# mila-iqia/diffusion_for_multi_scale_molecular_dynamics

Hardware: AMD Instinct MI355X
Metric: sampled structures/sec (1000-step predictor-corrector SDE sampling) (higher is better)
Workload: dtype f32 (per-edge matrix products as split-f16 hi/lo x3 MFMA terms with f32 accumulation: 22-bit products; state, updates, reductions and every other layer in f32)

## Files before the change

diffusion_for_multi_scale_molecular_dynamics_amd/csrc/mdx_egnn.hip:

```cpp
#include <hip/hip_runtime.h>
#include <stdint.h>

#include "../../include/mdx_hip.h"
#include "mdx_launch.hpp"

using mdx::as_stream;
using mdx::kBlock;
using mdx::kWave;
using mdx::launch_status;

namespace {

__device__ __forceinline__ float silu_fast(float a) { return a / (1.0f + __expf(-a)); }

__global__ __launch_bounds__(kBlock) void egnn_message_input_kernel(const float* __restrict__ proj, const int64_t* __restrict__ edges,
                                                                    const float* __restrict__ radial, const float* __restrict__ bias,
                                                                    const float* __restrict__ w_radial, int64_t n_edges, int H,
                                                                    int silu, float* __restrict__ out)
{
    const int quads = H >> 2;
    const int64_t total = n_edges * quads;
    for (int64_t t = blockIdx.x * (int64_t)blockDim.x + threadIdx.x; t < total; t += (int64_t)gridDim.x * blockDim.x) {
        const int64_t e = t / quads;
        const int q = (int)(t - e * quads);
        const int64_t src = edges[2 * e], dst = edges[2 * e + 1];
        const float r = radial[e];
        const float4 a = reinterpret_cast<const float4*>(proj + src * 2 * H)[q];
        const float4 b = reinterpret_cast<const float4*>(proj + dst * 2 * H + H)[q];
        const float4 bi = reinterpret_cast<const float4*>(bias)[q];
        const float4 wr = reinterpret_cast<const float4*>(w_radial)[q];
        float4 o;
        o.x = (a.x + b.x + bi.x) + r * wr.x;
        o.y = (a.y + b.y + bi.y) + r * wr.y;
        o.z = (a.z + b.z + bi.z) + r * wr.z;
        o.w = (a.w + b.w + bi.w) + r * wr.w;
        if (silu) { o.x = silu_fast(o.x); o.y = silu_fast(o.y); o.z = silu_fast(o.z); o.w = silu_fast(o.w); }
        reinterpret_cast<float4*>(out + e * H)[q] = o;
    }
}

__device__ __forceinline__ void uplift(float kr, float& c, float& s)
{
    const double a = (double)kr;
    c = (float)cos(a);
    s = (float)sin(a);
}

__global__ __launch_bounds__(kBlock) void egnn_node_inputs_kernel(const float* __restrict__ x, const float* __restrict__ k_vectors,
                                                                  int n_k, const float* __restrict__ sigma, int atoms_per_structure,
                                                                  const int64_t* __restrict__ atom_types,
                                                                  const float* __restrict__ w, const float* __restrict__ b,
                                                                  int F, int H, int64_t n_nodes, float* __restrict__ z,
                                                                  float* __restrict__ h, const float* __restrict__ w2,
                                                                  const float* __restrict__ b2, int H2, float* __restrict__ h2,
                                                                  const uint32_t* __restrict__ table_key)
{
    if (mdx::table_is_current(table_key, sigma)) return;
    const int64_t stride = (int64_t)gridDim.x * blockDim.x, t0 = blockIdx.x * (int64_t)blockDim.x + threadIdx.x;
    if (h2) {
        for (int64_t t = t0; t < n_nodes * H2; t += stride) {
            const int64_t i = t / H2;
            const int j = (int)(t - i * H2);
            const float s = sigma[i / atoms_per_structure];
            const int64_t a = atom_types[i];
            float v = b2[j] + s * w2[(int64_t)j * F];
            if (a >= 0 && a + 1 < F) v = v + w2[(int64_t)j * F + 1 + a];
            h2[t] = v;
        }
    }
    for (int64_t t = t0; h && t < n_nodes * H; t += stride) {
        const int64_t i = t / H;
        const int j = (int)(t - i * H);
        const float s = sigma[i / atoms_per_structure];
        const int64_t a = atom_types[i];
        float v = b[j] + s * w[(int64_t)j * F];
        if (a >= 0 && a + 1 < F) v = v + w[(int64_t)j * F + 1 + a];
        h[t] = v;
    }
    for (int64_t t = t0; t < n_nodes * n_k; t += stride) {
        const int64_t i = t / n_k;
        const int k = (int)(t - i * n_k);
        float kr = 0.0f;
        for (int d = 0; d < 3; ++d) kr = kr + (6.2831855f * x[3 * i + d]) * k_vectors[3 * k + d];
        uplift(kr, z[2 * t], z[2 * t + 1]);
    }
}

__device__ __forceinline__ float4 embed_quad(const float* __restrict__ t, int H, int q, float s, int64_t a, int F)
{
    const float4 bias = reinterpret_cast<const float4*>(t)[q];
    const float4 w0 = reinterpret_cast<const float4*>(t + H)[q];
    float4 v;
    v.x = bias.x + s * w0.x;
    v.y = bias.y + s * w0.y;
    v.z = bias.z + s * w0.z;
    v.w = bias.w + s * w0.w;
    if (a >= 0 && a + 1 < F) {
        const float4 wa = reinterpret_cast<const float4*>(t + (2 + a) * H)[q];
        v.x = v.x + wa.x;
        v.y = v.y + wa.y;
        v.z = v.z + wa.z;
        v.w = v.w + wa.w;
    }
    return v;
}

__global__ __launch_bounds__(kBlock) void egnn_node_inputs_rows_kernel(const float* __restrict__ x, const float* __restrict__ k_vectors,
                                                                       int n_k, const float* __restrict__ sigma,
                                                                       int atoms_per_structure,
                                                                       const int64_t* __restrict__ atom_types,
                                                                       const float* __restrict__ w, const float* __restrict__ b,
                                                                       int F, int H, int64_t n_nodes, float* __restrict__ z,
                                                                       float* __restrict__ h, const float* __restrict__ w2,
                                                                       const float* __restrict__ b2, int H2,
                                                                       float* __restrict__ h2,
                                                                       const uint32_t* __restrict__ table_key)
{
    if (mdx::table_is_current(table_key, sigma)) return;
    extern __shared__ float tables[];
    float* t1 = tables;
    float* t2 = tables + (1 + F) * H;
    for (int j = threadIdx.x; h && j < H; j += blockDim.x) {
        t1[j] = b[j];
        for (int f = 0; f < F; ++f) t1[(1 + f) * H + j] = w[(int64_t)j * F + f];
    }
    if (h2)
        for (int j = threadIdx.x; j < H2; j += blockDim.x) {
            t2[j] = b2[j];
            for (int f = 0; f < F; ++f) t2[(1 + f) * H2 + j] = w2[(int64_t)j * F + f];
        }
    __syncthreads();
    const int lane = threadIdx.x % 64;
    const int64_t wave = (blockIdx.x * (int64_t)blockDim.x + threadIdx.x) / 64, n_waves = ((int64_t)gridDim.x * blockDim.x) / 64;
    const int per = n_k <= 64 ? min(4, 64 / n_k) : 1;
    for (int64_t i0 = wave * per; i0 < n_nodes; i0 += n_waves * per) {
        if (n_k <= 64) {
            const int g = lane / n_k, k = lane - g * n_k;
            const int64_t i = i0 + g;
            if (g < per && i < n_nodes) {
                float kr = 0.0f;
                for (int d = 0; d < 3; ++d) kr = kr + (6.2831855f * x[3 * i + d]) * k_vectors[3 * k + d];
                uplift(kr, z[2 * (i * n_k + k)], z[2 * (i * n_k + k) + 1]);
            }
        } else {
            for (int k = lane; k < n_k; k += 64) {
                float kr = 0.0f;
                for (int d = 0; d < 3; ++d) kr = kr + (6.2831855f * x[3 * i0 + d]) * k_vectors[3 * k + d];
                uplift(kr, z[2 * (i0 * n_k + k)], z[2 * (i0 * n_k + k) + 1]);
            }
        }
        if (!h && !h2) continue;
        for (int g = 0; g < per && i0 + g < n_nodes; ++g) {
            const int64_t i = i0 + g;
            const float s = sigma[i / atoms_per_structure];
            const int64_t a = atom_types[i];
            if (h2)
                for (int q = lane; q < (H2 >> 2); q += 64) reinterpret_cast<float4*>(h2 + i * H2)[q] = embed_quad(t2, H2, q, s, a, F);
            if (h)
                for (int q = lane; q < (H >> 2); q += 64) reinterpret_cast<float4*>(h + i * H)[q] = embed_quad(t1, H, q, s, a, F);
        }
    }
}

__global__ __launch_bounds__(kBlock) void egnn_scores_kernel(const float* __restrict__ z, const float* __restrict__ x_hat,
                                                             const float* __restrict__ k_vectors, int n_k, int64_t n_nodes,
                                                             float* __restrict__ scores)
{
    for (int64_t t = blockIdx.x * (int64_t)blockDim.x + threadIdx.x; t < n_nodes * 3; t += (int64_t)gridDim.x * blockDim.x) {
        const int64_t i = t / 3;
        const int alpha = (int)(t - 3 * i);
        const float* zi = z + i * 2 * n_k;
        const float* xi = x_hat + i * 2 * n_k;
        float acc = 0.0f;
        for (int k = 0; k < n_k; ++k) {
            const float kk = k_vectors[3 * k + alpha];
            acc = acc + ((zi[2 * k] * -kk) * xi[2 * k + 1] + (zi[2 * k + 1] * kk) * xi[2 * k]);
        }
        scores[t] = acc;
    }
}

__device__ __forceinline__ float wave_sum(float v)
{
    v += __builtin_bit_cast(float, __builtin_amdgcn_update_dpp(0, __builtin_bit_cast(int, v), 0x111, 0xf, 0xf, false));
    v += __builtin_bit_cast(float, __builtin_amdgcn_update_dpp(0, __builtin_bit_cast(int, v), 0x112, 0xf, 0xf, false));
    v += __builtin_bit_cast(float, __builtin_amdgcn_update_dpp(0, __builtin_bit_cast(int, v), 0x114, 0xf, 0xf, false));
    v += __builtin_bit_cast(float, __builtin_amdgcn_update_dpp(0, __builtin_bit_cast(int, v), 0x118, 0xf, 0xf, false));
    v += __builtin_bit_cast(float, __builtin_amdgcn_update_dpp(0, __builtin_bit_cast(int, v), 0x142, 0xa, 0xf, false));
    v += __builtin_bit_cast(float, __builtin_amdgcn_update_dpp(0, __builtin_bit_cast(int, v), 0x143, 0xc, 0xf, false));
    return __builtin_bit_cast(float, __builtin_amdgcn_readlane(__builtin_bit_cast(int, v), 63));
}

constexpr int kMaxClasses = 8;

__global__ __launch_bounds__(kBlock) void egnn_outputs_kernel(const float* __restrict__ z, const float* __restrict__ x_hat,
                                                              const float* __restrict__ k_vectors, int n_k,
                                                              const float* __restrict__ h, const float* __restrict__ cw,
                                                              const float* __restrict__ cb, int H, int C, int mask_class,
                                                              int64_t n_nodes, float* __restrict__ scores,
                                                              float* __restrict__ logits, float* __restrict__ zero_out,
                                                              int64_t n_zero)
{
    const int64_t tid = blockIdx.x * (int64_t)blockDim.x + threadIdx.x, n_threads = (int64_t)gridDim.x * blockDim.x;
    for (int64_t t = tid; t < n_zero; t += n_threads) zero_out[t] = 0.0f;
    const int lane = threadIdx.x % kWave;
    const int quads = H >> 2;
    constexpr int kNodesPerWave = 4;
    const int64_t n_waves = n_threads / kWave;
    for (int64_t node0 = (tid / kWave) * kNodesPerWave; node0 < n_nodes; node0 += n_waves * kNodesPerWave) {
        float acc = 0.0f;
        const int score_node = (lane - (kWave - 3 * kNodesPerWave)) / 3, alpha = (lane - (kWave - 3 * kNodesPerWave)) % 3;
        const bool scores_lane = lane >= kWave - 3 * kNodesPerWave && node0 + score_node < n_nodes;
        if (scores_lane) {
            const float* zi = z + (node0 + score_node) * 2 * n_k;
            const float* xi = x_hat + (node0 + score_node) * 2 * n_k;
            for (int k = 0; k < n_k; ++k) {
                const float kk = k_vectors[3 * k + alpha];
                acc = acc + ((zi[2 * k] * -kk) * xi[2 * k + 1] + (zi[2 * k + 1] * kk) * xi[2 * k]);
            }
        }
        float part[kNodesPerWave][kMaxClasses];
#pragma unroll
        for (int m = 0; m < kNodesPerWave; ++m)
#pragma unroll
            for (int c = 0; c < kMaxClasses; ++c) part[m][c] = 0.0f;
        for (int q = lane; q < quads; q += kWave) {
            float4 hv[kNodesPerWave];
#pragma unroll
            for (int m = 0; m < kNodesPerWave; ++m)
                hv[m] = node0 + m < n_nodes ? reinterpret_cast<const float4*>(h + (node0 + m) * H)[q] : float4{0.0f, 0.0f, 0.0f, 0.0f};
#pragma unroll
            for (int c = 0; c < kMaxClasses; ++c) {
                if (c < C && c != mask_class) {
                    const float4 wv = reinterpret_cast<const float4*>(cw + (int64_t)c * H)[q];
#pragma unroll
                    for (int m = 0; m < kNodesPerWave; ++m)
                        part[m][c] += (hv[m].x * wv.x + hv[m].y * wv.y) + (hv[m].z * wv.z + hv[m].w * wv.w);
                }
            }
        }
#pragma unroll
        for (int c = 0; c < kMaxClasses; ++c) {
            if (c < C) {
#pragma unroll
                for (int m = 0; m < kNodesPerWave; ++m) {
                    float v = part[m][c];
                    if (c != mask_class) v = wave_sum(v);
                    if (lane == 0 && node0 + m < n_nodes) logits[(node0 + m) * C + c] = (c == mask_class) ? -__builtin_inff() : v + cb[c];
                }
            }
// ... 17 lines not shown
        const int64_t e0 = offsets[node], deg = degree[node];
        float acc = 0.0f;
        auto row_dot = [&](int64_t e) {
            float part = 0.0f;
            for (int q = lane; q < quads; q += kWave) {
                const float4 hv = reinterpret_cast<const float4*>(hidden + e * H)[q];
                const float4 wv = reinterpret_cast<const float4*>(w)[q];
                part += (hv.x * wv.x + hv.y * wv.y) + (hv.z * wv.z + hv.w * wv.w);
            }
            return part;
        };
        auto finish = [&](int64_t e, float part) {
            part = mdx::wave_sum(part);
            if (lane < d) acc += coord_diff[e * d + lane] * part;
        };
        int64_t e = e0;
        for (; e + 4 <= e0 + deg; e += 4) {
            const float p0 = row_dot(e), p1 = row_dot(e + 1), p2 = row_dot(e + 2), p3 = row_dot(e + 3);
            finish(e, p0); finish(e + 1, p1); finish(e + 2, p2); finish(e + 3, p3);
        }
        for (; e < e0 + deg; ++e) finish(e, row_dot(e));
        if (lane < d) trans[node * d + lane] = (mean && deg > 0) ? acc / (float)deg : acc;
    }
}

__global__ __launch_bounds__(kBlock) void segment_rows_kernel(const float* __restrict__ data, const int64_t* __restrict__ offsets,
                                                              const int64_t* __restrict__ degree, int64_t n_nodes, int H, int mean,
                                                              float* __restrict__ out)
{
    const int lane = threadIdx.x % kWave;
    const int64_t wave = (blockIdx.x * (int64_t)blockDim.x + threadIdx.x) / kWave;
    const int64_t n_waves = ((int64_t)gridDim.x * blockDim.x) / kWave;
    const int quads = H >> 2;
    for (int64_t node = wave; node < n_nodes; node += n_waves) {
        const int64_t e0 = offsets[node], deg = degree[node];
        const float count = (mean && deg > 0) ? (float)deg : 1.0f;
        for (int q = lane; q < quads; q += kWave) {
            float4 acc = {0.0f, 0.0f, 0.0f, 0.0f};
#pragma unroll 4
            for (int64_t e = e0; e < e0 + deg; ++e) {
                const float4 v = reinterpret_cast<const float4*>(data + e * H)[q];
                acc.x += v.x; acc.y += v.y; acc.z += v.z; acc.w += v.w;
            }
            if (mean) { acc.x /= count; acc.y /= count; acc.z /= count; acc.w /= count; }
            reinterpret_cast<float4*>(out + node * H)[q] = acc;
        }
    }
}

}

extern "C" {

int mdx_egnn_message_input(const float* node_proj, const int64_t* edges, const float* radial, const float* bias,
                           const float* w_radial, int64_t n_edges, int H, int silu, float* out, mdx_stream_t stream)
{
    if (n_edges < 0 || H < 4 || (H & 3)) return H >= 1 && (H & 3) ? MDX_ERR_UNSUPPORTED : MDX_ERR_INVALID_ARG;
    if (n_edges == 0) return MDX_OK;
    if (!node_proj || !edges || !radial || !bias || !w_radial || !out) return MDX_ERR_INVALID_ARG;
    int64_t blocks = (n_edges * (H >> 2) + kBlock - 1) / kBlock;
    if (blocks > 16384) blocks = 16384;
    hipLaunchKernelGGL(egnn_message_input_kernel, dim3((unsigned)blocks), dim3(kBlock), 0, as_stream(stream),
                       node_proj, edges, radial, bias, w_radial, n_edges, H, silu, out);
    return launch_status();
}

static unsigned node_grid(int64_t n_nodes)
{
    int64_t blocks = (n_nodes * kWave + kBlock - 1) / kBlock;
    if (blocks > 16384) blocks = 16384;
    return (unsigned)(blocks < 1 ? 1 : blocks);
}

int mdx_egnn_node_inputs(const float* x, const float* k_vectors, int n_k, const float* sigma, int atoms_per_structure,
                         const int64_t* atom_types, const float* emb_weight, const float* emb_bias, int n_features, int H,
                         int64_t n_nodes, float* z_out, float* h_out, const float* second_weight, const float* second_bias,
                         int second_width, float* second_out, mdx_stream_t stream)
{
    return mdx_egnn_node_inputs_keyed(x, k_vectors, n_k, sigma, atoms_per_structure, atom_types, emb_weight, emb_bias, n_features,
                                      H, n_nodes, z_out, h_out, second_weight, second_bias, second_width, second_out, nullptr,
                                      stream);
}

int mdx_egnn_node_inputs_keyed(const float* x, const float* k_vectors, int n_k, const float* sigma, int atoms_per_structure,
                               const int64_t* atom_types, const float* emb_weight, const float* emb_bias, int n_features, int H,
                               int64_t n_nodes, float* z_out, float* h_out, const float* second_weight, const float* second_bias,
                               int second_width, float* second_out, const uint32_t* table_key, mdx_stream_t stream)
{
    if (n_nodes < 0 || n_k < 1 || atoms_per_structure < 1 || n_features < 2 || H < 1) return MDX_ERR_INVALID_ARG;
    if (n_nodes == 0) return MDX_OK;
    if (!x || !k_vectors || !sigma || !atom_types || !emb_weight || !emb_bias || !z_out) return MDX_ERR_INVALID_ARG;
    if (second_out && (!second_weight || !second_bias || second_width < 1)) return MDX_ERR_INVALID_ARG;
    const size_t table_bytes = sizeof(float) * (size_t)(1 + n_features) * ((size_t)H + (second_out ? (size_t)second_width : 0));
    if ((H & 3) == 0 && (!second_out || (second_width & 3) == 0) && table_bytes <= 48 * 1024) {
        int64_t blocks = (n_nodes + 15) / 16;
        if (blocks > 2048) blocks = 2048;
        hipLaunchKernelGGL(egnn_node_inputs_rows_kernel, dim3((unsigned)blocks), dim3(kBlock), table_bytes,
                           as_stream(stream), x, k_vectors, n_k, sigma, atoms_per_structure, atom_types,
                           emb_weight, emb_bias, n_features, H, n_nodes, z_out, h_out, second_weight, second_bias, second_width,
                           second_out, table_key);
        return launch_status();
    }
    int64_t blocks = (n_nodes * H + kBlock - 1) / kBlock;
    if (blocks > 16384) blocks = 16384;
    hipLaunchKernelGGL(egnn_node_inputs_kernel, dim3((unsigned)blocks), dim3(kBlock), 0, as_stream(stream), x,
                       k_vectors, n_k, sigma, atoms_per_structure, atom_types, emb_weight, emb_bias, n_features, H, n_nodes,
                       z_out, h_out, second_weight, second_bias, second_width, second_out, table_key);
    return launch_status();
}

int mdx_egnn_scores(const float* z, const float* x_hat, const float* k_vectors, int n_k, int64_t n_nodes, float* scores_out,
                    mdx_stream_t stream)
{
    if (n_nodes < 0 || n_k < 1) return MDX_ERR_INVALID_ARG;
    if (n_nodes == 0) return MDX_OK;
    if (!z || !x_hat || !k_vectors || !scores_out) return MDX_ERR_INVALID_ARG;
    int64_t blocks = (n_nodes * 3 + kBlock - 1) / kBlock;
    if (blocks > 16384) blocks = 16384;
    hipLaunchKernelGGL(egnn_scores_kernel, dim3((unsigned)blocks), dim3(kBlock), 0, as_stream(stream), z, x_hat,
                       k_vectors, n_k, n_nodes, scores_out);
    return launch_status();
}

int mdx_egnn_outputs(const float* z, const float* x_hat, const float* k_vectors, int n_k, const float* h,
                     const float* class_weight, const float* class_bias, int H, int num_classes, int mask_class,
                     int64_t n_nodes, float* scores_out, float* logits_out, float* zero_out, int64_t n_zero,
                     mdx_stream_t stream)
{
    if (n_nodes < 0 || n_k < 1 || H < 4 || num_classes < 1 || n_zero < 0 || mask_class >= num_classes) return MDX_ERR_INVALID_ARG;
    if ((H & 3) || num_classes > kMaxClasses) return MDX_ERR_UNSUPPORTED;
    if (n_zero > 0 && !zero_out) return MDX_ERR_INVALID_ARG;
    if (n_nodes == 0 && n_zero == 0) return MDX_OK;
    if (n_nodes > 0 && (!z || !x_hat || !k_vectors || !h || !class_weight || !class_bias || !scores_out || !logits_out))
        return MDX_ERR_INVALID_ARG;
    hipLaunchKernelGGL(egnn_outputs_kernel, dim3(node_grid((n_nodes + 3) / 4)), dim3(kBlock), 0, as_stream(stream), z,
                       x_hat, k_vectors, n_k, h, class_weight, class_bias, H, num_classes, mask_class, n_nodes, scores_out,
                       logits_out, zero_out, n_zero);
    return launch_status();
}

int mdx_egnn_coord_head(const float* hidden, const float* w_out, const float* coord_diff, const int64_t* offsets,
                        const int64_t* degree, int64_t n_nodes, int H, int spatial_dimension, int mean, float* trans,
                        mdx_stream_t stream)
{
    if (n_nodes < 0 || H < 4 || spatial_dimension < 1) return MDX_ERR_INVALID_ARG;
    if ((H & 3) || spatial_dimension > kWave) return MDX_ERR_UNSUPPORTED;
    if (n_nodes == 0) return MDX_OK;
    if (!hidden || !w_out || !coord_diff || !offsets || !degree || !trans) return MDX_ERR_INVALID_ARG;
    hipLaunchKernelGGL(egnn_coord_head_kernel, dim3(node_grid(n_nodes)), dim3(kBlock), 0, as_stream(stream),
                       hidden, w_out, coord_diff, offsets, degree, n_nodes, H, spatial_dimension, mean, trans);
    return launch_status();
}

int mdx_segment_rows(const float* data, const int64_t* offsets, const int64_t* degree, int64_t n_nodes, int H, int mean,
                     float* out, mdx_stream_t stream)
{
    if (n_nodes < 0 || H < 4) return MDX_ERR_INVALID_ARG;
    if (H & 3) return MDX_ERR_UNSUPPORTED;
    if (n_nodes == 0) return MDX_OK;
    if (!data || !offsets || !degree || !out) return MDX_ERR_INVALID_ARG;
    hipLaunchKernelGGL(segment_rows_kernel, dim3(node_grid(n_nodes)), dim3(kBlock), 0, as_stream(stream),
                       data, offsets, degree, n_nodes, H, mean, out);
    return launch_status();
}

}
```

diffusion_for_multi_scale_molecular_dynamics_amd/csrc/mdx_egnn_table.hip:

```cpp
#include <hip/hip_runtime.h>
#include <stdint.h>

#include "../../include/mdx_hip.h"
#include "mdx_launch.hpp"

using namespace mdx;

namespace {

typedef float f32x4 __attribute__((ext_vector_type(4)));

__device__ __forceinline__ void lagrange_weights(float t, float w[4])
{
    const float tp = t + 1.0f, tm = t - 1.0f, t2 = t - 2.0f;
    w[0] = -(t * tm * t2) / 6.0f;
    w[1] = (tp * tm * t2) / 2.0f;
    w[2] = -(tp * t * t2) / 2.0f;
    w[3] = (tp * t * tm) / 6.0f;
}

__device__ __forceinline__ float interpolate(const float w[4], float v0, float v1, float v2, float v3)
{
    return ((w[0] * v0 + w[1] * v1) + w[2] * v2) + w[3] * v3;
}

__device__ __forceinline__ f32x4 interpolate4(const float w[4], f32x4 v0, f32x4 v1, f32x4 v2, f32x4 v3)
{
    return ((w[0] * v0 + w[1] * v1) + w[2] * v2) + w[3] * v3;
}

__device__ __forceinline__ float squared_distance(const float* ci, const float* __restrict__ cj, int D)
{
    float r2 = 0.0f;
    for (int k = 0; k < D; ++k) {
        const float dlt = ci[k] - cj[k];
        r2 += dlt * dlt;
    }
    return r2;
}

__device__ __forceinline__ float coord_head_value(float s, int flags) { return (flags & MDX_EGNN_COORD_TANH) ? tanhf(s) : s; }
__device__ __forceinline__ float normalize_factor(float r2) { return tanhf(r2) / sqrtf(r2 + 1.0e-16f); }

__device__ __forceinline__ unsigned abs_bits(float v) { return __float_as_uint(v) & 0x7fffffffu; }

constexpr int kCheckRows = 32;
__global__ __launch_bounds__(256) void egnn_table_check_kernel(const float* __restrict__ messages, const float* __restrict__ scalar,
                                                               int H, int n_pairs, int n_even, unsigned* __restrict__ workspace,
                                                               const uint32_t* __restrict__ table_key,
                                                               const float* __restrict__ sigma)
{
    if (table_is_current(table_key, sigma)) return;
    const int p = blockIdx.x, K = 2 * n_even - 1;
    const int j0 = blockIdx.y * kCheckRows, j1 = min(j0 + kCheckRows, n_even - 2);
    float w[4];
    lagrange_weights(0.5f, w);
    for (int c = threadIdx.x; c <= H; c += blockDim.x) {
        auto value = [&](int row) { return c < H ? messages[((int64_t)p * K + row) * H + c] : scalar[(int64_t)p * K + row]; };
        unsigned err = 0, big = 0;
        for (int j = j0; j < j1; ++j) {
            const float v0 = value(j > 0 ? j - 1 : 1), v1 = value(j), v2 = value(j + 1), v3 = value(j + 2);
            const float mid = value(n_even + j);
            err = max(err, abs_bits(interpolate(w, v0, v1, v2, v3) - mid));
            big = max(big, max(max(abs_bits(v1), abs_bits(v2)), max(abs_bits(v3), abs_bits(mid))));
        }
        if (j0 < j1) {
            atomicMax(workspace + (int64_t)p * (H + 1) + c, err);
            atomicMax(workspace + (int64_t)n_pairs * (H + 1) + p, big);
        }
    }
}

__global__ __launch_bounds__(256) void egnn_table_verdict_kernel(unsigned* __restrict__ workspace, int n_pairs, int columns,
                                                                 const float* __restrict__ sigma, int64_t n_sigma, float tolerance,
                                                                 float* __restrict__ worst_out, uint32_t* __restrict__ status,
                                                                 uint32_t* __restrict__ table_key)
{
    __shared__ float worst[256];
    __shared__ int bad[256];
    float mine = 0.0f;
    int fail = 0;
    const bool built = !table_is_current(table_key, sigma);
    const int64_t n_entries = built ? (int64_t)n_pairs * columns : 0;
    for (int64_t i = threadIdx.x; i < n_entries; i += blockDim.x) {
        const float err = __uint_as_float(workspace[i]), big = __uint_as_float(workspace[n_entries + i / columns]);
        if (!(err <= tolerance * big)) fail = 1;
        if (big > 0.0f) mine = fmaxf(mine, err / big);
        else if (err > 0.0f || err != err) mine = INFINITY;
    }
    __syncthreads();
    if (built)
        for (int64_t i = threadIdx.x; i < n_entries + n_pairs; i += blockDim.x) workspace[i] = 0u;
    const int table_fail = fail;
    for (int64_t i = 1 + threadIdx.x; i < n_sigma; i += blockDim.x)
        if (!(sigma[i] == sigma[0])) fail = 1;
    worst[threadIdx.x] = mine;
    bad[threadIdx.x] = fail | (table_fail << 1);
    __syncthreads();
    for (int s = 128; s > 0; s >>= 1) {
        if ((int)threadIdx.x < s) {
            worst[threadIdx.x] = fmaxf(worst[threadIdx.x], worst[threadIdx.x + s]);
            bad[threadIdx.x] |= bad[threadIdx.x + s];
        }
        __syncthreads();
    }
    if (threadIdx.x == 0) {
        if (worst_out && built) worst_out[0] = worst[0];
        if (bad[0] && status) atomicOr(status, MDX_STATUS_EGNN_TABLE);
        if (table_key && built) {
            if (bad[0] & 2) {
                table_key[0] = MDX_EGNN_TABLE_NO_KEY;
            } else {
                table_key[0] = __float_as_uint(sigma[0]);
                table_key[1] = table_key[1] + 1u;
            }
        }
    }
}

__global__ __launch_bounds__(256) void egnn_table_gather_kernel(const float* __restrict__ table, const float* __restrict__ table_scalar,
                                                                int H, int n_classes, int n_even, float inv_spacing,
                                                                const int64_t* __restrict__ atom_types,
                                                                const int64_t* __restrict__ offsets, const int64_t* __restrict__ degree,
                                                                int64_t n_nodes, int mean_messages, float* __restrict__ out,
                                                                const float* __restrict__ left, const float* __restrict__ coord,
                                                                const int64_t* __restrict__ edges, int D, int mean_coords,
                                                                int flags, float* __restrict__ coord_out, uint32_t* __restrict__ status)
{
    const int lane = threadIdx.x % kWave;
    const int64_t wave = (blockIdx.x * (int64_t)blockDim.x + threadIdx.x) / kWave;
    const int64_t n_waves = ((int64_t)gridDim.x * blockDim.x) / kWave;
    const int K = 2 * n_even - 1, quads = H >> 2;
    const bool has_quad = lane < quads;
    bool outside = false;
    for (int64_t node = wave; node < n_nodes; node += n_waves) {
        const int64_t e0 = offsets[node], deg = degree[node], e1 = e0 + deg;
        int64_t a = atom_types[node];
        if (a < 0 || a >= n_classes) { outside = true; a = 0; }
        float part[8] = {0, 0, 0, 0, 0, 0, 0, 0}, ci[8];
#pragma unroll
        for (int k = 0; k < 8; ++k) ci[k] = k < D ? coord[node * D + k] : 0.0f;
        f32x4 acc = {0.0f, 0.0f, 0.0f, 0.0f};
        for (int64_t c0 = e0; c0 < e1; c0 += kWave) {
            const int64_t e = c0 + lane;
            int row = 0, row_left = 0;
            float w[4] = {0, 0, 0, 0};
            if (e < e1) {
                const int64_t dst = edges[2 * e + 1];
                int64_t b = atom_types[dst];
                if (b < 0 || b >= n_classes) { outside = true; b = 0; }
                const float r2 = squared_distance(ci, coord + dst * D, D);
                const float u = sqrtf(r2) * inv_spacing;
                int m = 0;
                float t = 0.0f;
                if (u <= (float)(n_even - 2)) {
                    m = min((int)u, n_even - 3);
                    t = u - (float)m;
                } else {
                    outside = true;
                }
                lagrange_weights(t, w);
                row = (int)(a * n_classes + b) * K + m;
                row_left = m > 0 ? row - 1 : row + 1;
                const float s = coord_head_value(interpolate(w, table_scalar[row_left], table_scalar[row], table_scalar[row + 1],
                                                             table_scalar[row + 2]), flags);
                if (flags & MDX_EGNN_COORD_NORMALIZE) {
                    float diff[8], n2 = 0.0f;
#pragma unroll
                    for (int k = 0; k < 8; ++k) {
                        diff[k] = k < D ? ci[k] - coord[dst * D + k] : 0.0f;
                        if (k < D) n2 += diff[k] * diff[k];
                    }
                    const float f = normalize_factor(n2);
#pragma unroll
                    for (int k = 0; k < 8; ++k)
                        if (k < D) part[k] += (f * diff[k]) * s;
                } else {
#pragma unroll
                    for (int k = 0; k < 8; ++k)
                        if (k < D) part[k] += (ci[k] - coord[dst * D + k]) * s;
                }
            }
            const int n = (int)min<int64_t>(kWave, e1 - c0);
            for (int i = 0; i < n; ++i) {
                const int r = __builtin_amdgcn_readlane(row, i), rl = __builtin_amdgcn_readlane(row_left, i);
                float wi[4];
#pragma unroll
                for (int k = 0; k < 4; ++k)
                    wi[k] = __builtin_bit_cast(float, __builtin_amdgcn_readlane(__builtin_bit_cast(int, w[k]), i));
                if (has_quad) {
                    const f32x4* base = reinterpret_cast<const f32x4*>(table + (int64_t)r * H) + lane;
                    const f32x4 v0 = reinterpret_cast<const f32x4*>(table + (int64_t)rl * H)[lane];
                    acc += interpolate4(wi, v0, base[0], base[quads], base[2 * quads]);
                }
            }
        }
        const float count = (mean_messages && deg > 0) ? (float)deg : 1.0f;
        if (has_quad) {
            if (mean_messages) acc = acc / count;
            if (left) {
                reinterpret_cast<f32x4*>(out + node * 2 * H)[lane] = reinterpret_cast<const f32x4*>(left + node * H)[lane];
                reinterpret_cast<f32x4*>(out + node * 2 * H + H)[lane] = acc;
            } else {
                reinterpret_cast<f32x4*>(out + node * H)[lane] = acc;
            }
        }
#pragma unroll
        for (int k = 0; k < 8; ++k) {
            if (k < D) {
                float v = part[k];
                v += __builtin_bit_cast(float, __builtin_amdgcn_update_dpp(0, __builtin_bit_cast(int, v), 0x111, 0xf, 0xf, false));
                v += __builtin_bit_cast(float, __builtin_amdgcn_update_dpp(0, __builtin_bit_cast(int, v), 0x112, 0xf, 0xf, false));
                v += __builtin_bit_cast(float, __builtin_amdgcn_update_dpp(0, __builtin_bit_cast(int, v), 0x114, 0xf, 0xf, false));
                v += __builtin_bit_cast(float, __builtin_amdgcn_update_dpp(0, __builtin_bit_cast(int, v), 0x118, 0xf, 0xf, false));
                v += __builtin_bit_cast(float, __builtin_amdgcn_update_dpp(0, __builtin_bit_cast(int, v), 0x142, 0xa, 0xf, false));
                v += __builtin_bit_cast(float, __builtin_amdgcn_update_dpp(0, __builtin_bit_cast(int, v), 0x143, 0xc, 0xf, false));
                part[k] = __builtin_bit_cast(float, __builtin_amdgcn_readlane(__builtin_bit_cast(int, v), 63));
            }
        }
        if (lane < D) {
            float total = 0.0f, mine = 0.0f;
#pragma unroll
            for (int k = 0; k < 8; ++k) {
                if (k == lane) { total = part[k]; mine = ci[k]; }
            }
            if (mean_coords && deg > 0) total = total / (float)deg;
            coord_out[node * D + lane] = mine + total;
        }
    }
    if (outside && status) atomicOr(status, MDX_STATUS_EGNN_TABLE);
}

}

extern "C" {

int mdx_egnn_table_check(const float* table, const float* table_scalar, int H, int n_classes, int n_even, const float* sigma,
                         int64_t n_sigma, float tolerance, uint32_t* workspace, float* worst_out, uint32_t* status,
                         mdx_stream_t stream)
{
    return mdx_egnn_table_check_keyed(table, table_scalar, H, n_classes, n_even, sigma, n_sigma, tolerance, workspace, worst_out,
                                      status, nullptr, stream);
}

int mdx_egnn_table_check_keyed(const float* table, const float* table_scalar, int H, int n_classes, int n_even, const float* sigma,
                               int64_t n_sigma, float tolerance, uint32_t* workspace, float* worst_out, uint32_t* status,
                               uint32_t* table_key, mdx_stream_t stream)
{
    if (H < 1 || n_classes < 1 || n_even < 4 || n_sigma < 1 || !(tolerance >= 0.0f)) return MDX_ERR_INVALID_ARG;
    if (!table || !table_scalar || !sigma || !workspace) return MDX_ERR_INVALID_ARG;
    const int n_pairs = n_classes * n_classes;
    const hipStream_t s = as_stream(stream);
    hipLaunchKernelGGL(egnn_table_check_kernel, dim3((unsigned)n_pairs, (unsigned)((n_even - 2 + kCheckRows - 1) / kCheckRows)),
                       dim3(256), 0, s, table, table_scalar, H, n_pairs, n_even, reinterpret_cast<unsigned*>(workspace),
                       table_key, sigma);
    hipLaunchKernelGGL(egnn_table_verdict_kernel, dim3(1), dim3(256), 0, s, reinterpret_cast<unsigned*>(workspace), n_pairs,
                       H + 1, sigma, n_sigma, tolerance, worst_out, status, table_key);
    return launch_status();
}

int mdx_egnn_table_gather(const float* table, const float* table_scalar, int H, int n_classes, int n_even, float inv_spacing,
                          const int64_t* atom_types, const int64_t* offsets, const int64_t* degree, int64_t n_nodes,
                          int mean_messages, const float* left, float* out, const float* coord, int coord_dimension,
                          const int64_t* edges, int mean_coords, int coord_flags, float* coord_out, uint32_t* status,
                          mdx_stream_t stream)
{
    if (n_nodes < 0 || H < 4 || n_classes < 1 || n_even < 4 || coord_dimension < 1 || !(inv_spacing > 0.0f))
        return MDX_ERR_INVALID_ARG;
    if (coord_flags & ~(MDX_EGNN_COORD_NORMALIZE | MDX_EGNN_COORD_TANH)) return MDX_ERR_INVALID_ARG;
    if ((H & 3) || H > 4 * kWave || coord_dimension > 8) return MDX_ERR_UNSUPPORTED;
    if ((int64_t)n_classes * n_classes * (2 * (int64_t)n_even - 1) * H >= ((int64_t)1 << 31)) return MDX_ERR_UNSUPPORTED;
    if (n_nodes == 0) return MDX_OK;
    if (!table || !table_scalar || !atom_types || !offsets || !degree || !out || !coord || !edges || !coord_out)
        return MDX_ERR_INVALID_ARG;
    int64_t blocks = (n_nodes * kWave + 255) / 256;
    if (blocks > 16384) blocks = 16384;
    hipLaunchKernelGGL(egnn_table_gather_kernel, dim3((unsigned)blocks), dim3(256), 0, as_stream(stream),
                       table, table_scalar, H, n_classes, n_even, inv_spacing, atom_types, offsets, degree, n_nodes, mean_messages,
                       out, left, coord, edges, coord_dimension, mean_coords, coord_flags, coord_out, status);
    return launch_status();
}

}
```

diffusion_for_multi_scale_molecular_dynamics_amd/csrc/mdx_hip.hip:

```cpp
#include <hip/hip_runtime.h>
#include <stdint.h>

#include <atomic>
#include <cmath>

#include "../../include/mdx_hip.h"
#include "mdx_launch.hpp"
#include "mdx_math.hpp"

using namespace mdx;

namespace {

struct ScheduleArgs {
    int T, type, C;
    double time_delta, sigma_min, sigma_max, corrector_eps;
    float *time, *sigma, *sigma2, *g, *g2, *eps, *sqrt2eps, *beta, *alpha_bar, *q, *qbar, *qbar_tm1;
};

template <int CSPEC>
__device__ __forceinline__ void qbar_chain(const ScheduleArgs& a, int r)
{
    const int T = a.T, C = CSPEC > 0 ? CSPEC : a.C;
#define MDX_SCHED_CLASSES(c) _Pragma("unroll") for (int c = 0; c < MDX_MAX_CLASSES; ++c) if (c < C)
// ... 529 lines not shown
            }
            if (one) {
                const float cand = (prop != a_t) ? v_best : -__builtin_huge_valf();
                if (cand > best_v || (cand == best_v && n < best_n)) { best_v = cand; best_n = n; best_prop = prop; }
                v.a_out[n] = a_t;
            } else {
                v.a_out[n] = prop;
                if (st.last_predictor_step && prop == M && p.status) atomicOr(p.status, MDX_STATUS_MASK_AT_LAST_STEP);
            }
        } else if (v.a_out && v.a_out != v.a) {
            v.a_out[n] = v.a[n];
        }
        if (p.do_coords) {
            float z0 = 0.0f, z1 = 0.0f, z2 = 0.0f, z3 = 0.0f;
            if (!v.z_coord) {
                const u32x4 r = philox4x32_10(item, st.call8, st.draw, MDX_TAG_COORD, st.k0, st.k1);
                box_muller(r.v[0], r.v[1], z0, z1);
                if (d > 2) box_muller(r.v[2], r.v[3], z2, z3);
            }
            float xin[3], sin_[3], out[3];
#pragma unroll
            for (int k = 0; k < 3; ++k)
                if (k < d) {
                    const int e = n * d + k;
                    const float zk = k == 0 ? z0 : (k == 1 ? z1 : z2);
                    xin[k] = v.x[e];
                    sin_[k] = v.score_x[e];
                    out[k] = v.z_coord ? v.z_coord[e] : zk;
                }
#pragma unroll
            for (int k = 0; k < 3; ++k)
                if (k < d) out[k] = coord_update(xin[k], sin_[k], out[k], sc.w, sc.n, sc.sigma);
#pragma unroll
            for (int k = 0; k < 3; ++k)
                if (k < d) v.x_out[n * d + k] = out[k];
        }
    }
    if (update_types && one) {
        group_argmax<G>(best_v, best_n, best_prop);
        if (lane == 0 && best_n < N) v.a_out[best_n] = best_prop;
    }
    if (p.do_lattice) {
        for (int k = lane; k < p.nl; k += G) {
            if (p.fixed_lattice) {
                if (v.l_out != v.l) v.l_out[k] = v.l[k];
            } else {
                float zz;
                if (v.z_lat) zz = v.z_lat[k];
                else {
                    const u32x4 r = philox4x32_10((uint32_t)v.b, st.call8 | (uint32_t)(k >> 2), st.draw, MDX_TAG_LATTICE,
                                                  st.k0, st.k1);
                    float z0, z1, z2, z3;
                    box_muller(r.v[0], r.v[1], z0, z1);
                    box_muller(r.v[2], r.v[3], z2, z3);
                    const int kk = k & 3;
                    zz = kk == 0 ? z0 : (kk == 1 ? z1 : (kk == 2 ? z2 : z3));
                }
                v.l_out[k] = (v.l[k] + (sc.w * v.score_l[k]) / sc.sigma_n) + sc.n * zz;
            }
        }
    }
}

__device__ __forceinline__ const float* off(const float* p, int64_t o) { return p ? p + o : nullptr; }
__device__ __forceinline__ float* off(float* p, int64_t o) { return p ? p + o : nullptr; }

__device__ __forceinline__ PcView structure_view(const PcArgs& p, int64_t b)
{
    const int N = p.N, C = p.C, d = p.d;
    PcView v;
    const int64_t a0 = b * N;
    v.a = p.a ? p.a + a0 : nullptr;
    v.x = off(p.x, a0 * d); v.l = off(p.l, b * p.nl);
    v.logits = off(p.logits, a0 * C); v.score_x = off(p.score_x, a0 * d); v.score_l = off(p.score_l, b * p.nl);
    v.z_coord = off(p.z_coord, a0 * d); v.gumbel = off(p.gumbel, a0 * C); v.u = off(p.u, a0);
    v.z_lat = off(p.z_lat, b * p.nl);
    v.a_out = p.a_out ? p.a_out + a0 : nullptr;
    v.x_out = off(p.x_out, a0 * d); v.l_out = off(p.l_out, b * p.nl); v.p_out = off(p.p_out, a0 * C);
    v.item0 = a0;
    v.b = b;
    return v;
}

template <int G, int CSPEC>
__global__ __launch_bounds__(kBlock) void pc_step_kernel(PcArgs p_in)
{
    PcArgs p = p_in;
    if constexpr (CSPEC > 0) { p.C = CSPEC; p.d = 3; p.nl = 6; }
    const int lane = threadIdx.x & (G - 1);
    const int64_t groups_per_grid = ((int64_t)gridDim.x * blockDim.x) / G;
    const int64_t group0 = ((int64_t)blockIdx.x * blockDim.x + threadIdx.x) / G;
    const PcStep st = make_step(p);
    for (int64_t b = group0; b < p.B; b += groups_per_grid) {
        const PcView v = structure_view(p, b);
        pc_update_structure<G>(p, st, v, lane, p.update_types);
    }
}

inline int lanes_per_structure(int N)
{
    int G = 1;
    while (G < N && G < kWave) G <<= 1;
    return G;
}

inline dim3 structure_grid(int64_t B, int G)
{
    int64_t blocks = cdiv(B * G, kBlock);
    if (blocks > 4096) blocks = 4096;
    if (blocks < 1) blocks = 1;
    return dim3((unsigned)blocks);
}

#define MDX_SWITCH_G(G, LAUNCH)                                                                              \
    switch (G) {                                                                                             \
        case 1: LAUNCH(1) break;                                                                             \
        case 2: LAUNCH(2) break;                                                                             \
        case 4: LAUNCH(4) break;                                                                             \
        case 8: LAUNCH(8) break;                                                                             \
        case 16: LAUNCH(16) break;                                                                           \
        case 32: LAUNCH(32) break;                                                                           \
        default: LAUNCH(64) break;                                                                           \
    }

int launch_pc(const PcArgs& a, hipStream_t st)
{
    const int G = lanes_per_structure(a.N);
    const dim3 grid = structure_grid(a.B, G), block(kBlock);
    const int cspec = (a.d == 3 && (a.C == 2 || a.C == 3)) ? a.C : 0;
#define MDX_LAUNCH_PC(GG)                                                                                   \
    if (cspec == 2) hipLaunchKernelGGL((pc_step_kernel<GG, 2>), grid, block, 0, st, a);                       \
    else if (cspec == 3) hipLaunchKernelGGL((pc_step_kernel<GG, 3>), grid, block, 0, st, a);                  \
    else hipLaunchKernelGGL((pc_step_kernel<GG, 0>), grid, block, 0, st, a);
    MDX_SWITCH_G(G, MDX_LAUNCH_PC)
#undef MDX_LAUNCH_PC
    return launch_status();
}

template <int G, int O = G / 2>
__device__ __forceinline__ float group_sum(float v)
{
    if constexpr (O > 0) {
        v = group_sum<G, O / 2>(v);
        v = v + partner<O>(v);
    }
    return v;
}

struct AdaptiveStatsArgs {
    const float *score_x, *score_l, *z_coord, *z_lat;
    mdx_rng_t rng;
    int index_i;
    const int32_t* d_index;
    int64_t B;
    int N, d, nl, fixed_lattice;
    float* workspace;
};

template <int G>
__global__ __launch_bounds__(kBlock) void adaptive_stats_kernel(AdaptiveStatsArgs p)
{
    const int lane = threadIdx.x & (G - 1);
    const int64_t groups_per_grid = ((int64_t)gridDim.x * blockDim.x) / G;
    const int64_t group0 = ((int64_t)blockIdx.x * blockDim.x + threadIdx.x) / G;
    const int N = p.N, d = p.d;
    const int index = (p.d_index ? *p.d_index : 0) + p.index_i;
    const uint32_t draw = (uint32_t)index * p.rng.draw_stride + p.rng.draw_offset;
    const uint32_t k0 = (uint32_t)p.rng.seed, k1 = (uint32_t)(p.rng.seed >> 32), call8 = rng_call(p.rng) << 8;
    for (int64_t b = group0; b < p.B; b += groups_per_grid) {
        const int64_t a0 = b * N;
        const float* sx = p.score_x + a0 * d;
        const float* zx = p.z_coord ? p.z_coord + a0 * d : nullptr;
        float ss = 0.0f, zn = 0.0f;
        for (int n = lane; n < N; n += G) {
            float z0 = 0.0f, z1 = 0.0f, z2 = 0.0f, z3 = 0.0f;
            if (!zx) {
                const u32x4 r = philox4x32_10((uint32_t)(a0 + n), call8, draw, MDX_TAG_COORD, k0, k1);
                box_muller(r.v[0], r.v[1], z0, z1);
                if (d > 2) box_muller(r.v[2], r.v[3], z2, z3);
            }
            float zz = 0.0f;
#pragma unroll
            for (int k = 0; k < 3; ++k)
                if (k < d) {
                    const int e = n * d + k;
                    const float s = sx[e];
                    const float zk = zx ? zx[e] : (k == 0 ? z0 : (k == 1 ? z1 : z2));
                    ss = ss + s * s;
                    zz = zz + zk * zk;
                }
            zn = zn + __builtin_sqrtf(zz);
        }
        ss = group_sum<G>(ss);
        zn = group_sum<G>(zn);
        float sl = 0.0f, zl = 0.0f;
        if (!p.fixed_lattice) {
            for (int k = lane; k < p.nl; k += G) {
                float zk;
                if (p.z_lat) zk = p.z_lat[b * p.nl + k];
                else {
                    const u32x4 r = philox4x32_10((uint32_t)b, call8 | (uint32_t)(k >> 2), draw, MDX_TAG_LATTICE, k0, k1);
                    float z0, z1, z2, z3;
                    box_muller(r.v[0], r.v[1], z0, z1);
                    box_muller(r.v[2], r.v[3], z2, z3);
                    const int kk = k & 3;
                    zk = kk == 0 ? z0 : (kk == 1 ? z1 : (kk == 2 ? z2 : z3));
                }
                const float s = p.score_l[b * p.nl + k];
                sl = sl + s * s;
                zl = zl + zk * zk;
            }
            sl = group_sum<G>(sl);
            zl = group_sum<G>(zl);
        }
        if (lane == 0) {
            float* w = p.workspace + b * 4;
// ... 1311 lines not shown
    return coordinates_update(x, s, z, score_weight, gaussian_noise_weight, sigma, nullptr, count, out, stream);
}

int mdx_relative_coordinates_update_dev(const float* x, const float* s, const float* z, const float* weights, int64_t count,
                                        float* out, mdx_stream_t stream)
{
    if (!weights) return MDX_ERR_INVALID_ARG;
    return coordinates_update(x, s, z, 0.0f, 0.0f, 1.0f, weights, count, out, stream);
}

static int lattice_update(const float* l, const float* s, const float* z, float score_weight, float gaussian_noise_weight,
                          float sigma_n, const float* weights_dev, int64_t count, float* out, mdx_stream_t stream)
{
    if (count < 0 || (count > 0 && (!l || !s || !z || !out))) return MDX_ERR_INVALID_ARG;
    if (count == 0) return MDX_OK;
    hipLaunchKernelGGL(lattice_update_kernel, dim3(flat_grid(count)), dim3(kBlock), 0, as_stream(stream), l, s, z,
                       score_weight, gaussian_noise_weight, sigma_n, count, out, weights_dev);
    return launch_status();
}

int mdx_lattice_parameters_update(const float* l, const float* s, const float* z, float score_weight,
                                  float gaussian_noise_weight, float sigma_n, int64_t count, float* out,
                                  mdx_stream_t stream)
{
    return lattice_update(l, s, z, score_weight, gaussian_noise_weight, sigma_n, nullptr, count, out, stream);
}

int mdx_lattice_parameters_update_dev(const float* l, const float* s, const float* z, const float* weights, int64_t count,
                                      float* out, mdx_stream_t stream)
{
    if (!weights) return MDX_ERR_INVALID_ARG;
    return lattice_update(l, s, z, 0.0f, 0.0f, 1.0f, weights, count, out, stream);
}

int mdx_atom_types_update(const float* logits, const int64_t* atom_types, const float* q, const float* q_bar,
                          const float* q_bar_tm1, const float* gumbel, const float* u, int64_t batch,
                          int number_of_atoms, int num_classes, float small_epsilon, int greedy, int one_transition,
                          int64_t* atom_types_out, float* probabilities_out, mdx_stream_t stream)
{
    if (batch < 0 || number_of_atoms < 1) return MDX_ERR_INVALID_ARG;
    if (num_classes < 2) return MDX_ERR_INVALID_ARG;
    if (num_classes > MDX_MAX_CLASSES) return MDX_ERR_UNSUPPORTED;
    if (batch == 0) return MDX_OK;
    if (!logits || !atom_types || !q || !q_bar || !q_bar_tm1 || !gumbel || !atom_types_out || (greedy && !u))
        return MDX_ERR_INVALID_ARG;
    PcArgs a{};
    a.use_tables = 0;
    a.q_explicit = q; a.qbar_explicit = q_bar; a.qbar_tm1_explicit = q_bar_tm1;
    a.greedy = greedy; a.one_transition = one_transition; a.update_types = 1;
    a.small_eps = small_epsilon;
    a.a = atom_types; a.logits = logits; a.gumbel = gumbel; a.u = u;
    a.B = batch; a.N = number_of_atoms; a.C = num_classes; a.d = 3;
    a.a_out = atom_types_out; a.p_out = probabilities_out;
    return launch_pc(a, as_stream(stream));
}

static int pc_common_args(const mdx_schedule_t* sched_host, int mode, int index_i, const int32_t* d_index, const mdx_pc_flags_t* f,
                          const int64_t* atom_types, const float* logits, const float* gumbel, const float* u, mdx_rng_t rng,
                          int64_t batch, int number_of_atoms, int spatial_dimension, int64_t* atom_types_out, uint32_t* status,
                          PcArgs& a)
{
    const int rc = check_index(sched_host, mode, index_i, d_index);
    if (rc != MDX_OK) return rc;
    if (!f || batch < 0 || number_of_atoms < 1 || spatial_dimension < 1 || spatial_dimension > 3) return MDX_ERR_INVALID_ARG;
    const int C = sched_host->num_classes;
    if (C < 2) return MDX_ERR_INVALID_ARG;
    if (C > MDX_MAX_CLASSES) return MDX_ERR_UNSUPPORTED;
    a.sched = to_dev(sched_host);
    a.use_tables = 1;
    a.mode = mode; a.index_i = index_i; a.d_index = d_index;
    a.atoms_pow = pow((double)number_of_atoms, 1.0 / (double)spatial_dimension);
    a.greedy = f->atom_type_greedy_sampling; a.one_transition = f->one_atom_type_transition_per_step;
    a.fixed_lattice = f->use_fixed_lattice_parameters;
    a.small_eps = f->small_epsilon;
    a.a = atom_types; a.logits = logits; a.gumbel = gumbel; a.u = u;
    a.rng = rng;
    a.B = batch; a.N = number_of_atoms; a.d = spatial_dimension; a.C = C;
    a.nl = spatial_dimension * (spatial_dimension + 1) / 2;
    a.a_out = atom_types_out; a.p_out = nullptr;
    a.status = status;
    return MDX_OK;
}

int mdx_pc_step_update(const mdx_schedule_t* sched_host, int mode, int index_i, const int32_t* d_index,
                       const mdx_pc_flags_t* f, const int64_t* atom_types, const float* x, const float* l,
                       const float* logits, const float* score_x, const float* score_l, const float* z_coordinates,
                       const float* gumbel, const float* u, const float* z_lattice, mdx_rng_t rng, int64_t batch,
                       int number_of_atoms, int spatial_dimension, int64_t* atom_types_out, float* x_out, float* l_out,
                       uint32_t* status, mdx_stream_t stream)
{
    PcArgs a{};
    const int rc = pc_common_args(sched_host, mode, index_i, d_index, f, atom_types, logits, gumbel, u, rng, batch, number_of_atoms,
                                  spatial_dimension, atom_types_out, status, a);
    if (rc != MDX_OK || batch == 0) return rc;
    if (!x || !score_x || !x_out || !l || !l_out) return MDX_ERR_INVALID_ARG;
    if (f->update_atom_types && (!atom_types || !atom_types_out)) return MDX_ERR_INVALID_ARG;
    if (f->update_atom_types && !logits && (a.C != 2 || a.p_out)) return MDX_ERR_INVALID_ARG;
    if (!f->use_fixed_lattice_parameters && !score_l) return MDX_ERR_INVALID_ARG;
    if ((int64_t)batch * number_of_atoms > 0xffffffffLL) return MDX_ERR_UNSUPPORTED;
    a.update_types = f->update_atom_types;
    a.do_coords = 1; a.do_lattice = 1;
    a.x = x; a.l = l; a.score_x = score_x; a.score_l = score_l; a.z_coord = z_coordinates; a.z_lat = z_lattice;
    a.x_out = x_out; a.l_out = l_out;
    return launch_pc(a, as_stream(stream));
}

static AdaptiveStepArgs adaptive_step_args(const mdx_schedule_t* sched_host, int index_i, const int32_t* d_index,
                                           int number_of_atoms, int spatial_dimension, int fixed_lattice, float corrector_r,
                                           float small_epsilon, const double* totals, float* weights)
{
    AdaptiveStepArgs s{};
    s.sched = to_dev(sched_host);
    s.index_i = index_i; s.d_index = d_index;
    s.atoms_pow = pow((double)number_of_atoms, 1.0 / (double)spatial_dimension);
    s.corrector_r = corrector_r; s.small_eps = small_epsilon;
    s.fixed_lattice = fixed_lattice;
    s.totals = totals; s.weights = weights;
    return s;
}

int mdx_adaptive_corrector_statistics(const mdx_schedule_t* sched_host, int index_i, const int32_t* d_index,
                                      const float* score_x, const float* score_l, const float* z_coordinates,
                                      const float* z_lattice_for_step_size, mdx_rng_t rng, int64_t batch, int number_of_atoms,
                                      int spatial_dimension, int use_fixed_lattice_parameters, float corrector_r,
                                      float small_epsilon, float* workspace, double* totals, float* weights,
                                      mdx_stream_t stream)
{
    const int rc = check_index(sched_host, MDX_CORRECTOR, index_i, d_index);
    if (rc != MDX_OK) return rc;
    if (batch < 1 || number_of_atoms < 1 || spatial_dimension < 1 || spatial_dimension > 3) return MDX_ERR_INVALID_ARG;
    if (!score_x || !workspace || !totals || (!use_fixed_lattice_parameters && !score_l)) return MDX_ERR_INVALID_ARG;
    if ((int64_t)batch * number_of_atoms > 0xffffffffLL) return MDX_ERR_UNSUPPORTED;
    AdaptiveStatsArgs a{};
    a.score_x = score_x; a.score_l = score_l; a.z_coord = z_coordinates; a.z_lat = z_lattice_for_step_size;
    a.rng = rng;
    a.index_i = index_i; a.d_index = d_index;
    a.B = batch; a.N = number_of_atoms; a.d = spatial_dimension;
    a.nl = spatial_dimension * (spatial_dimension + 1) / 2;
    a.fixed_lattice = use_fixed_lattice_parameters;
    a.workspace = workspace;
    const int rs = launch_adaptive_stats(a, as_stream(stream));
    if (rs != MDX_OK) return rs;
    hipLaunchKernelGGL(adaptive_totals_kernel, dim3(1), dim3(kBlock), 0, as_stream(stream), (const float*)workspace, batch,
                       number_of_atoms, totals,
                       adaptive_step_args(sched_host, index_i, d_index, number_of_atoms, spatial_dimension,
                                          use_fixed_lattice_parameters, corrector_r, small_epsilon, totals, weights));
    return launch_status();
}

int mdx_adaptive_corrector_step_size(const mdx_schedule_t* sched_host, int index_i, const int32_t* d_index,
                                     const double* totals, int number_of_atoms, int spatial_dimension,
                                     int use_fixed_lattice_parameters, float corrector_r, float small_epsilon, float* weights,
                                     mdx_stream_t stream)
{
    const int rc = check_index(sched_host, MDX_CORRECTOR, index_i, d_index);
    if (rc != MDX_OK) return rc;
    if (number_of_atoms < 1 || spatial_dimension < 1 || spatial_dimension > 3 || !totals || !weights) return MDX_ERR_INVALID_ARG;
    hipLaunchKernelGGL(adaptive_step_kernel, dim3(1), dim3(1), 0, as_stream(stream),
                       adaptive_step_args(sched_host, index_i, d_index, number_of_atoms, spatial_dimension,
                                          use_fixed_lattice_parameters, corrector_r, small_epsilon, totals, weights));
    return launch_status();
}

int mdx_adaptive_corrector_update(const mdx_schedule_t* sched_host, int mode, int index_i, const int32_t* d_index,
                                  const mdx_pc_flags_t* f, const int64_t* atom_types, const float* x, const float* l,
                                  const float* logits, const float* score_x, const float* score_l, const float* z_coordinates,
                                  const float* gumbel, const float* u, const float* z_lattice, const float* weights,
                                  mdx_rng_t rng, int64_t batch, int number_of_atoms, int spatial_dimension,
                                  int64_t* atom_types_out, float* x_out, float* l_out, uint32_t* status, mdx_stream_t stream)
{
    PcArgs a{};
    const int rc = pc_common_args(sched_host, mode, index_i, d_index, f, atom_types, logits, gumbel, u, rng, batch, number_of_atoms,
                                  spatial_dimension, atom_types_out, status, a);
    if (rc != MDX_OK || batch == 0) return rc;
    const int types = mode == MDX_PREDICTOR ? 1 : f->update_atom_types;
    if (types && (!atom_types || !logits || !atom_types_out)) return MDX_ERR_INVALID_ARG;
    if (mode == MDX_CORRECTOR) {
        if (!weights || !x || !score_x || !x_out || !l || !l_out) return MDX_ERR_INVALID_ARG;
        if (!f->use_fixed_lattice_parameters && !score_l) return MDX_ERR_INVALID_ARG;
    }
    if ((int64_t)batch * number_of_atoms > 0xffffffffLL) return MDX_ERR_UNSUPPORTED;
    a.update_types = types;
    if (mode == MDX_CORRECTOR) {
        a.x = x; a.l = l; a.score_x = score_x; a.score_l = score_l; a.z_coord = z_coordinates; a.z_lat = z_lattice;
        a.x_out = x_out; a.l_out = l_out;
    }
    return launch_adaptive_update(a, weights, as_stream(stream));
// ... 376 lines not shown
```

diffusion_for_multi_scale_molecular_dynamics_amd/generators/langevin_generator.py:

```python
import contextlib
import dataclasses
import gc
import warnings
import weakref
from typing import Optional

import torch

from .. import kernels
from .._hip import (MDX_CORRECTOR, MDX_PREDICTOR, STATUS_EGNN_F16_RANGE, STATUS_EGNN_TABLE, STATUS_MASK_AT_LAST_STEP,
                    MdxError, PcFlags, Rng)
from ..models.score_networks.score_network import ScoreNetwork
from ..namespace import AXL, CARTESIAN_FORCES, NOISE, NOISY_AXL_COMPOSITION, TIME
from ..noise_schedulers.noise_parameters import NoiseParameters
from ..noise_schedulers.noise_scheduler import NoiseScheduler
from ..utils.sample_trajectory import PinnedStaging, SampleTrajectory
from . import network_hooks as hooks
from .noise_sources import DevicePhiloxNoise, RecordingNoise, ReferenceOrderNoise, one_host_thread, upload
from .predictor_corrector_axl_generator import PredictorCorrectorAXLGenerator, PredictorCorrectorSamplingParameters
from .trajectory_initializer import TrajectoryInitializer


class LangevinGenerator(PredictorCorrectorAXLGenerator):
    def __init__(self, noise_parameters: NoiseParameters, sampling_parameters: PredictorCorrectorSamplingParameters,
                 axl_network: ScoreNetwork, trajectory_initializer: Optional[TrajectoryInitializer] = None):
        sp = sampling_parameters
        super().__init__(number_of_discretization_steps=noise_parameters.total_time_steps,
                         number_of_corrector_steps=sp.number_of_corrector_steps,
                         spatial_dimension=sp.spatial_dimension, num_atom_types=sp.num_atom_types,
                         number_of_atoms=sp.number_of_atoms,
                         use_fixed_lattice_parameters=sp.use_fixed_lattice_parameters,
                         fixed_lattice_parameters=sp.fixed_lattice_parameters,
                         trajectory_initializer=trajectory_initializer)
        self.noise_parameters = noise_parameters
        self.sampling_parameters = sp
        self.number_of_atoms = sp.number_of_atoms
        self.masked_atom_type_index = self.num_classes - 1
        self.axl_network = axl_network
        self.small_epsilon = sp.small_epsilon
        self.one_atom_type_transition_per_step = sp.one_atom_type_transition_per_step
        self.atom_type_greedy_sampling = sp.atom_type_greedy_sampling
        self.atom_type_transition_in_corrector = sp.atom_type_transition_in_corrector
        self.use_fixed_lattice_parameters = sp.use_fixed_lattice_parameters
        self.fixed_lattice_parameters = sp.fixed_lattice_parameters

        self.record = sp.record_samples
        self.record_corrector = sp.record_samples_corrector_steps
        self.record_atom_type_update = sp.record_atom_type_update
        if self.record_corrector or self.record_atom_type_update:
            assert self.record, "Corrector steps or atom_type_update can only be recorded if record_samples is True."

        rng_mode = getattr(sp, "rng_mode", "reference")
        assert rng_mode in ("reference", "device"), f"unknown rng_mode {rng_mode}"
        self.rng_mode = rng_mode
        self.use_hip_graph = bool(getattr(sp, "use_hip_graph", False))
        self.fused_score_network = bool(getattr(sp, "fused_score_network", False))
        self._mlp_pack = None
        self._noise_workspace = kernels.NoiseWorkspace()
        self.fused_sampler_options = 0
        self.fused_predrawn_noise = True
        self._seed = getattr(sp, "seed", None)
        self._call_counter = 0
        self.noise_source = ReferenceOrderNoise() if rng_mode == "reference" else None
        self.f16_range_fallbacks = 0
        self.table_fallbacks = 0
        self.resampling_steps = 0
        self._visit = 0
        self._warned_not_capturable = False

        self._scheduler = None
        self._status = None
        self._call_word = None
        self._buffers = {}
        if self.record:
            self.sample_trajectory_recorder = SampleTrajectory()
            self._staging = PinnedStaging()
            self.sample_trajectory_recorder.record(key="noise_parameters", entry=dataclasses.asdict(noise_parameters))
            self.sample_trajectory_recorder.record(key="sampling_parameters",
                                                   entry={k: v for k, v in dataclasses.asdict(sp).items()})

    @property
    def _device_rng(self) -> bool:
        return getattr(self.noise_source, "device_rng", False)

    @staticmethod
    def _device(device) -> torch.device:
        device = torch.device(device)
        if device.type == "cuda" and device.index is None:
            device = torch.device("cuda", torch.cuda.current_device())
        return device

    def _prepare(self, device: torch.device):
        device = self._device(device)
        if device.type != "cuda":
            raise MdxError(f"LangevinGenerator runs on the GPU hot path only; got device '{device}' "
                           "(there is no CPU fallback -- use the reference implementation on CPU)")
        if self._scheduler is None or self._scheduler.tables.device != device:
            self._scheduler = NoiseScheduler(self.noise_parameters, num_classes=self.num_classes, device=device)
            self.noise, self.langevin_dynamics = self._scheduler.get_all_sampling_parameters()
            self._status = torch.zeros(1, dtype=torch.int32, device=device)
            self._buffers = {}
            if self.record:
                self.sample_trajectory_recorder.record(
                    key="noise", entry=type(self.noise)(*[t.detach().cpu() for t in self.noise]))
        return self._scheduler.tables

    def _time_sigma(self, batch: int, device):
        key = ("ts", batch)
        if key not in self._buffers:
            self._buffers[key] = (torch.empty(batch, 1, dtype=torch.float32, device=device),
                                  torch.empty(batch, 1, dtype=torch.float32, device=device))
        return self._buffers[key]

    def _flags(self, update_atom_types: bool) -> PcFlags:
        return PcFlags(int(self.atom_type_greedy_sampling), int(self.one_atom_type_transition_per_step),
                       int(self.use_fixed_lattice_parameters), int(update_atom_types), float(self.small_epsilon))

    def _draw_stride(self) -> int:
        return (self.number_of_corrector_steps + 1) * (self.resampling_steps + 1)

    def _rng(self, draw_offset: int) -> Rng:
        src = self.noise_source
        seed, call = (src.seed, src.call) if self._device_rng else (0, 0)
        word = self._call_word.data_ptr() if self._device_rng and self._call_word is not None else None
        return Rng(seed, call, self._draw_stride(),
                   self._visit * (self.number_of_corrector_steps + 1) + draw_offset, 0, word)

    def _begin_call(self, device):
        if self.rng_mode == "device":
            seed = self._seed if self._seed is not None else torch.initial_seed()
            rank = torch.distributed.get_rank() if torch.distributed.is_available() and \
                torch.distributed.is_initialized() else 0
            self.noise_source = DevicePhiloxNoise(seed + rank, self._call_counter)
            device = self._device(device)
            if self._call_word is None or self._call_word.device != device:
                self._buffers.pop("graph_loop", None)
                self._call_word = torch.zeros(1, dtype=torch.int32, device=device)
            kernels.index_set(self._call_word, self._call_counter)
            self._call_counter += 1
        if hasattr(self.trajectory_initializer, "noise_source"):
            self.trajectory_initializer.noise_source = self.noise_source

    def _draw_coordinates_gaussian_sample(self, number_of_samples):
        return self.noise_source.randn(number_of_samples, self.number_of_atoms, self.spatial_dimension)

    def _draw_lattice_gaussian_sample(self, number_of_samples):
        return self.noise_source.randn(number_of_samples, self.num_lattice_parameters)

# ... 39 lines not shown
        lat = lattice_parameters
        if z is None:
            z = self._draw_lattice_gaussian_sample(lat.shape[0])
        weights = self._three_scalars(score_weight, gaussian_noise_weight, sigma_n_i, lat)
        return kernels.lattice_parameters_update(lat.contiguous(), sigma_normalized_scores.to(lat).contiguous(),
                                                 z.to(lat).contiguous(), weights=weights)

    _lattice_parameters_update_predictor_step = _lattice_parameters_update
    _lattice_parameters_update_corrector_step = _lattice_parameters_update

    @staticmethod
    def _shared_matrix(m: torch.Tensor, name: str) -> torch.Tensor:
        from ..utils.d3pm_utils import _one_matrix
        one = _one_matrix(m)
        if one is None:
            flat = m.reshape(-1, m.shape[-2], m.shape[-1])
            one = flat[0]
            if not bool((flat == one).all()):
                raise MdxError(f"{name}: the transition matrices differ between samples / atoms; the sampler's atom-type update "
                               "takes ONE time index per call (use utils.d3pm_utils.get_probability_at_previous_time_step for "
                               "per-atom matrices)")
        return one

    def _atom_types_update(self, predicted_logits: torch.Tensor, atom_types_i: torch.LongTensor, q_matrices_i: torch.Tensor,
                           q_bar_matrices_i: torch.Tensor, q_bar_tm1_matrices_i: torch.Tensor,
                           atom_type_greedy_sampling: bool, one_atom_type_transition_per_step: bool) -> torch.LongTensor:
        logits = predicted_logits
        batch = logits.shape[0]
        gumbel = self._draw_gumbel_sample(batch).to(device=logits.device, dtype=torch.float32).contiguous()
        u = None
        if atom_type_greedy_sampling:
            u = self._draw_binary_sample(batch).to(device=logits.device, dtype=torch.float32).contiguous()
        q, q_bar, q_bar_tm1 = [self._shared_matrix(m, name).to(logits).contiguous()
                               for m, name in ((q_matrices_i, "q_matrices_i"), (q_bar_matrices_i, "q_bar_matrices_i"),
                                               (q_bar_tm1_matrices_i, "q_bar_tm1_matrices_i"))]
        a_in = atom_types_i.to(logits.device).contiguous()
        a_out, probs = kernels.atom_types_update(logits.contiguous(), a_in, q, q_bar, q_bar_tm1, gumbel, u, self.small_epsilon,
                                                 atom_type_greedy_sampling, one_atom_type_transition_per_step,
                                                 return_probabilities=True)
        if self.record_atom_type_update:
            if atom_type_greedy_sampling:
                all_masked = (a_in == self.masked_atom_type_index).all(dim=-1)
                gumbel = torch.where(all_masked.view(-1, 1, 1), gumbel, torch.zeros_like(gumbel))
            self.sample_trajectory_recorder.record(key="atom_type_update", entry=dict(
                predicted_logits=logits.detach().cpu(), one_step_transition_probabilities=probs.cpu(),
                gumbel_sample=gumbel.cpu(), a_i=a_in.cpu(), a_im1=a_out.cpu()))
        return a_out

    def _get_coordinates_corrector_step_size(self, index_i: int, sigma_i: torch.Tensor, model_predictions_i: torch.Tensor,
                                             z: torch.Tensor) -> torch.Tensor:
        self._prepare(model_predictions_i.device)
        return self.langevin_dynamics.epsilon[index_i].to(model_predictions_i)

    def _get_lattice_parameters_corrector_step_size(self, index_i: int, sigma_n_i: torch.Tensor,
                                                    model_predictions_i: torch.Tensor, z: torch.Tensor) -> torch.Tensor:
        self._prepare(model_predictions_i.device)
        return self.langevin_dynamics.epsilon[index_i].to(model_predictions_i)

    def _get_model_predictions(self, composition: AXL, time, sigma_noise, cartesian_forces: torch.Tensor) -> AXL:
        if not isinstance(time, torch.Tensor) or time.dim() == 0:
            time = torch.full((composition.X.shape[0], 1), float(time), dtype=torch.float32, device=composition.X.device)
        if not isinstance(sigma_noise, torch.Tensor) or sigma_noise.dim() == 0:
            sigma_noise = torch.full((composition.X.shape[0], 1), float(sigma_noise), dtype=torch.float32, device=composition.X.device)
        batch = {NOISY_AXL_COMPOSITION: composition, TIME: time, NOISE: sigma_noise, CARTESIAN_FORCES: cartesian_forces}
        with hooks.uniform_sigma(self.axl_network):
            return self.axl_network(batch, conditional=False)

    def _lattice_score(self, predictions: AXL, composition: AXL) -> Optional[torch.Tensor]:
        if self.use_fixed_lattice_parameters:
            return None
        if predictions.L.shape != composition.L.shape:
            raise MdxError(f"the score network's lattice output has shape {tuple(predictions.L.shape)}, the lattice parameters "
                           f"{tuple(composition.L.shape)}: this network can only sample with use_fixed_lattice_parameters=True")
        return predictions.L.contiguous()

    def _logits_unread(self, update_types: bool, predictions_unread: bool) -> bool:
        constant_logits = self.num_classes == 2
        return bool(predictions_unread and (not update_types or constant_logits) and not self.record
                    and not self.record_atom_type_update and "_get_model_predictions" not in self.__dict__
                    and type(self)._get_model_predictions is _OWN_GET_MODEL_PREDICTIONS
                    and not hooks.outputs_watched(self.axl_network))

    def _step(self, mode: int, composition: AXL, index_i: int, cartesian_forces: torch.Tensor, draw_offset: int,
              d_index: Optional[torch.Tensor] = None, in_place: bool = False, predictions_unread: bool = False):
        x = composition.X
        device = x.device
        sched = self._prepare(device)
        batch = x.shape[0]
        time_t, sigma_t = self._time_sigma(batch, device)
        kernels.fill_time_sigma(sched, mode, index_i, d_index, time_t, sigma_t)
        update_types = mode == MDX_PREDICTOR or self.atom_type_transition_in_corrector
        unread = self._logits_unread(update_types, predictions_unread)
        with hooks.logits_unread(self.axl_network) if unread else contextlib.nullcontext():
            predictions = self._get_model_predictions(composition, time_t, sigma_t, cartesian_forces)

        z = gumbel = u = z_lattice = None
        if not self._device_rng:
            if mode == MDX_PREDICTOR:
                gumbel = self._draw_gumbel_sample(batch)
                if self.atom_type_greedy_sampling:
                    u = self._draw_binary_sample(batch)
                z = self._draw_coordinates_gaussian_sample(batch)
                z_lattice = self._draw_lattice_gaussian_sample(batch)
            else:
                z = self._draw_coordinates_gaussian_sample(batch)
                self._draw_lattice_gaussian_sample(batch)
                if not self.use_fixed_lattice_parameters:
                    z_lattice = self._draw_lattice_gaussian_sample(batch)
                if update_types:
                    gumbel = self._draw_gumbel_sample(batch)
                    if self.atom_type_greedy_sampling:
                        u = self._draw_binary_sample(batch)
            if self.use_fixed_lattice_parameters:
                z_lattice = None
            z, gumbel, u, z_lattice = [upload(t, device) for t in (z, gumbel, u, z_lattice)]
            if not self.use_fixed_lattice_parameters and z_lattice is None:
                raise MdxError("internal error: lattice noise missing")

        a_in = composition.A
        if update_types:
            a_out = a_in if in_place else torch.empty_like(a_in)
        else:
            a_out = a_in
        x_out = x if in_place else torch.empty_like(x)
        if self.use_fixed_lattice_parameters or in_place:
            l_out = composition.L
        else:
            l_out = torch.empty_like(composition.L)
        logits = predictions.A.contiguous() if update_types and predictions.A is not None else None
        if update_types and logits is None and not unread:
            raise MdxError("the score network returned no atom-type logits for a step that reads them")
        kernels.pc_step_update(sched, mode, index_i, d_index, self._flags(update_types),
                               a_in if update_types else None, x, composition.L, logits,
                               predictions.X.contiguous(),
                               self._lattice_score(predictions, composition),
                               z, gumbel, u, z_lattice, self._rng(draw_offset),
                               a_out if update_types else None, x_out, l_out, self._status)
        if self.record_atom_type_update and update_types:
            self._record_atom_type_update(sched, mode, index_i, logits, a_in, gumbel, u, a_out, batch)
        return AXL(A=a_out, X=x_out, L=l_out), predictions

    def _record_atom_type_update(self, sched, mode, index_i, logits, a_in, gumbel, u, a_out, batch):
        idx = index_i - 1 if (mode == MDX_PREDICTOR or index_i > 0) else 0
        src = self.noise_source
        if gumbel is None:
            from .._hip import TAG_BINARY, TAG_GUMBEL
            draw = index_i * self._draw_stride() + self._visit * (self.number_of_corrector_steps + 1) + \
                (0 if mode == MDX_PREDICTOR else 1)
            n = batch * self.number_of_atoms
            gumbel = kernels.rng_fill(kernels.RNG_GUMBEL, src.seed, src.call, draw, TAG_GUMBEL, n, self.num_classes,
                                      logits.device).view(batch, self.number_of_atoms, self.num_classes)
            u = kernels.rng_fill(kernels.RNG_UNIFORM, src.seed, src.call, draw, TAG_BINARY, n, 1,
                                 logits.device).view(batch, self.number_of_atoms)
        one = self.one_atom_type_transition_per_step and not (mode == MDX_PREDICTOR and idx == 0)
        a_check, probs = kernels.atom_types_update(logits, a_in, sched.q_matrix[idx], sched.q_bar_matrix[idx],
                                                   sched.q_bar_tm1_matrix[idx], gumbel, u, self.small_epsilon,
                                                   self.atom_type_greedy_sampling, one, return_probabilities=True)
        assert torch.equal(a_check, a_out), "stand-alone and fused atom-type updates disagree"
        if self.atom_type_greedy_sampling:
            all_masked = (a_in == self.masked_atom_type_index).all(dim=-1)
            gumbel = torch.where(all_masked.view(-1, 1, 1), gumbel, torch.zeros_like(gumbel))
        self.sample_trajectory_recorder.record(key="atom_type_update", entry=dict(
            predicted_logits=self._staging.to_host(logits), one_step_transition_probabilities=self._staging.to_host(probs),
            gumbel_sample=self._staging.to_host(gumbel), a_i=self._staging.to_host(a_in),
            a_im1=self._staging.to_host(a_out)))

    def predictor_step(self, composition_i: AXL, index_i: int, cartesian_forces: torch.Tensor) -> AXL:
        assert 1 <= index_i <= self.number_of_discretization_steps, \
            "The predictor step can only be invoked for index_i between 1 and the total number of discretization steps."
        composition_im1, predictions = self._step(MDX_PREDICTOR, composition_i, index_i, cartesian_forces, 0)
        if self.record:
            self._record_step("predictor_step", ["composition_i", "composition_im1", "model_predictions_i"],
                              [composition_i, composition_im1, predictions], index_i)
        return composition_im1

    def corrector_step(self, composition_i: AXL, index_i: int, cartesian_forces: torch.Tensor,
                       corrector_number: int = 0) -> AXL:
        assert 0 <= index_i <= self.number_of_discretization_steps - 1, \
            "The corrector step can only be invoked for index_i between 0 and the total number of " \
            "discretization steps minus 1."
        corrected, predictions = self._step(MDX_CORRECTOR, composition_i, index_i, cartesian_forces,
                                            1 + corrector_number)
        if self.record_corrector:
            self._record_step("corrector_step", ["composition_i", "corrected_composition_i", "model_predictions_i"],
                              [composition_i, corrected, predictions], index_i)
        return corrected

    def _record_step(self, key, names, axls, index_i):
        entry = dict(time_step_index=index_i)
        for name, axl in zip(names, axls):
            host = self._staging.to_host
            entry[name] = AXL(A=host(axl.A), X=host(axl.X), L=host(axl.L))
        self.sample_trajectory_recorder.record(key=key, entry=entry)

    def _after_predictor(self, composition: AXL, index_i: int, d_index=None) -> AXL:
        return composition

    def sample_from_noisy_composition(self, starting_noisy_composition: AXL, starting_step_index: int,
                                      ending_step_index: int) -> AXL:
        self._check_index_range(starting_step_index, ending_step_index)
        self._prepare(starting_noisy_composition.X.device)
        if self.noise_source is None:
            self._begin_call(starting_noisy_composition.X.device)
        self._share_noise_source()
        out = self._run_loop(starting_noisy_composition, starting_step_index, ending_step_index)
        self.check_status()
        return out

    def _recover(self, report: int, index_i: int, run):
        self._status.zero_()
        if report & STATUS_EGNN_F16_RANGE:
            self.f16_range_fallbacks += 1
            warnings.warn(f"EGNN edge chain: a value beyond the f16 range at time index {index_i}; this iteration is recomputed "
                          "with edge_chain_precision='f32' on the same draws (the network's setting is restored afterwards)")
        if report & STATUS_EGNN_TABLE:
            self.table_fallbacks += 1
            hooks.table_off(self.axl_network)
            warnings.warn(f"EGNN first layer: the distance table failed its check at time index {index_i}; this iteration is "
                          "recomputed on the per-edge chain, and the network's first_layer_table is now 'off'")
        if not report & STATUS_EGNN_F16_RANGE:
# ... 1 lines not shown
        with hooks.exact_f32(self.axl_network):
            return run()

    def _iteration(self, composition: AXL, i: int, forces: torch.Tensor) -> AXL:
        visits = self._visits_at(i)
        for self._visit in range(visits):
            composition = self.predictor_step(composition, i + 1, forces)
            for m in range(self.number_of_corrector_steps):
                composition = self.corrector_step(composition, i, forces, m)
            if self._visit < visits - 1:
                composition = self._forward_step(composition, i)
        self._visit = 0
        return composition

    def _guarded_iteration(self, composition: AXL, i: int, forces: torch.Tensor) -> AXL:
        if not hooks.reports_watched(self.axl_network):
            return self._iteration(composition, i, forces)
        source, keeps = self.noise_source, not self._device_rng
        if keeps:
            self.noise_source = RecordingNoise(source)
            self._share_noise_source()
        marks = self._recorder_marks() if self.record else None

        def again():
            if marks is not None:
                self._recorder_truncate(marks)
            if keeps:
                self.noise_source = self.noise_source.replay()
                self._share_noise_source()
            return self._iteration(composition, i, forces)

        try:
            out = self._iteration(composition, i, forces)
            report = hooks.take_reports(self.axl_network)
            return self._recover(report, i, again) if report else out
        finally:
            if keeps:
                self.noise_source = source
                self._share_noise_source()

    def _share_noise_source(self):
        if hasattr(self.trajectory_initializer, "noise_source"):
            self.trajectory_initializer.noise_source = self.noise_source

    def _recorder_marks(self):
        data = self.sample_trajectory_recorder._internal_data
        return {key: len(data[key]) for key in ("predictor_step", "corrector_step", "atom_type_update") if key in data}

    def _recorder_truncate(self, marks):
        data = self.sample_trajectory_recorder._internal_data
        for key in ("predictor_step", "corrector_step", "atom_type_update"):
            if key in data:
                del data[key][marks.get(key, 0):]

    def _run_loop(self, starting_noisy_composition: AXL, starting_step_index: int, ending_step_index: int) -> AXL:
        if self.fused_score_network:
            return self._sample_fused(starting_noisy_composition, starting_step_index, ending_step_index)
        if self.use_hip_graph and self._device_rng and not self.record and self._capture_safe(starting_noisy_composition):
            return self._sample_with_graph(starting_noisy_composition, starting_step_index, ending_step_index)
        composition = starting_noisy_composition
        forces = torch.zeros_like(composition.X)
        hooks.clear_reports(self.axl_network)
        for i in range(starting_step_index - 1, max(ending_step_index, 0) - 1, -1):
            composition = self._guarded_iteration(composition, i, forces)
        return composition

    def _capture_safe(self, composition: AXL) -> bool:
        safe = hooks.capture_safe(self.axl_network, *composition.X.shape[:2], composition.X.device)
        if not safe and not self._warned_not_capturable:
            warnings.warn("use_hip_graph=True, but the score network's forward on this batch shape needs a host "
                          "synchronisation: the sampler iteration is launched eagerly")
            self._warned_not_capturable = True
        return safe

    def _visits_at(self, index_i: int) -> int:
        return 1 + self.resampling_steps if index_i > 0 else 1

    def _forward_step(self, composition: AXL, index_i: int, d_index=None) -> AXL:
        raise MdxError("resampling needs the repaint generator")

    def _iteration_on_device_index(self, comp: AXL, forces: torch.Tensor, d_index: torch.Tensor,
                                   visits: Optional[int] = None):
        visits = 1 + self.resampling_steps if visits is None else visits
        for self._visit in range(visits):
            comp, _ = self._step(MDX_PREDICTOR, comp, 1, forces, 0, d_index=d_index, in_place=True, predictions_unread=True)
            comp = self._after_predictor(comp, 0, d_index=d_index)
            for m in range(self.number_of_corrector_steps):
                comp, _ = self._step(MDX_CORRECTOR, comp, 0, forces, 1 + m, d_index=d_index, in_place=True,
                                     predictions_unread=True)
            if self._visit < visits - 1:
                comp = self._forward_step(comp, 0, d_index=d_index)
        self._visit = 0
        kernels.index_add(d_index, -1)
        return comp

    def fused_pack(self, device):
        from ..models.score_networks.mlp_score_network import MLPScoreNetwork
        if not isinstance(self.axl_network, MLPScoreNetwork):
            raise MdxError("fused_score_network=True needs an MLPScoreNetwork; other networks use the per-step kernels")
        if not self._device_rng or self.record or type(self)._after_predictor is not LangevinGenerator._after_predictor:
            raise MdxError("fused_score_network=True needs rng_mode='device', no recording and no repaint constraint")
        if self._mlp_pack is None or self._mlp_pack.device != torch.device(device):
            self._mlp_pack = kernels.MlpPack(self.axl_network, device)
        return self._mlp_pack

    def _sample_fused(self, start: AXL, starting_step_index: int, ending_step_index: int) -> AXL:
        device = start.X.device
        sched = self._prepare(device)
        pack = self.fused_pack(device)
        comp = AXL(A=start.A.clone(), X=start.X.clone(), L=start.L.clone())
        kernels.mlp_pc_sample(sched, pack, self._flags(True), self.number_of_corrector_steps,
                              self.atom_type_transition_in_corrector, starting_step_index,
                              starting_step_index - max(ending_step_index, 0), self._rng(0), comp.A, comp.X, comp.L,
                              self._status, workspace=self._noise_workspace if self.fused_predrawn_noise else None,
                              options=self.fused_sampler_options)
        return comp

    def _graph_key(self, start: AXL):
        settings = (self.number_of_corrector_steps, self.resampling_steps, self.atom_type_greedy_sampling,
                    self.one_atom_type_transition_per_step, self.atom_type_transition_in_corrector,
                    self.use_fixed_lattice_parameters, self.small_epsilon, self.num_classes)
        words = tuple(None if w is None else w.data_ptr() for w in (self._call_word, self._status))
        net = self.axl_network
        return (tuple(start.X.shape), tuple(start.L.shape), str(start.X.device), hooks.capture_key(net), settings, words,
                kernels.parameter_stamp(*net.parameters()))

    def _sample_with_graph(self, start: AXL, starting_step_index: int, ending_step_index: int) -> AXL:
        key = self._graph_key(start)
        kept = self._buffers.get("graph_loop")
        if kept is not None and kept.key == key:
            loop = kept
            loop.reset(start, starting_step_index)
        else:
            loop = IterationLoop(self, start, starting_step_index, use_graph=True)
            loop.key = key
            self._buffers["graph_loop"] = loop
        loop.advance(starting_step_index - max(ending_step_index, 0))
        comp = loop.composition
        return AXL(A=comp.A.clone(), X=comp.X.clone(), L=comp.L.clone())

    def check_status(self):
        if self._status is None:
            return
        word = int(self._status.item())
        self._status.zero_()
        net_status = hooks.status_word(self.axl_network)
        if net_status is not None:
            from ..utils.neighbors import _raise_if_cutoff_too_large
            held = net_status.clone()
            net_status.zero_()
            _raise_if_cutoff_too_large(held)
        if word & STATUS_MASK_AT_LAST_STEP:
            raise AssertionError("There remains MASKED atoms at the last time step: review code, there must be a "
                                 "bug or invalid input.")

    def sample(self, number_of_samples: int, device: torch.device) -> AXL:
        device = self._device(device)
        self._prepare(device)
        self._begin_call(device)
        composition = super().sample(number_of_samples, device)
        if self.rng_mode == "device":
            self.noise_source = None
        return composition


_OWN_GET_MODEL_PREDICTIONS = LangevinGenerator._get_model_predictions


class IterationLoop:

    def __init__(self, generator: LangevinGenerator, start: AXL, starting_step_index: int, use_graph: bool):
        gen = generator
        self.generator = weakref.proxy(generator)
        device = start.X.device
        gen._prepare(device)
        assert gen._device_rng, "the device-resident loop needs rng_mode='device'"
        self.composition = AXL(A=start.A.clone(), X=start.X.clone(), L=start.L.clone())
        self.forces = torch.zeros_like(self.composition.X)
        self.d_index = torch.zeros(1, dtype=torch.int32, device=device)
        self.remaining = starting_step_index
        self.graph = None
        self.key = None
        self._watch = None
        if use_graph:
            comp = self.composition
            saved = AXL(A=comp.A.clone(), X=comp.X.clone(), L=comp.L.clone())
            side = torch.cuda.Stream(device=device)
            side.wait_stream(torch.cuda.current_stream(device))
            with torch.cuda.stream(side):
                kernels.index_set(self.d_index, starting_step_index - 1)
                for _ in range(2):
                    gen._iteration_on_device_index(comp, self.forces, self.d_index)
            torch.cuda.current_stream(device).wait_stream(side)
            comp.A.copy_(saved.A)
            comp.X.copy_(saved.X)
            comp.L.copy_(saved.L)
            gen._status.zero_()
            hooks.clear_reports(gen.axl_network)
            self.graph = torch.cuda.CUDAGraph()
            previous = gen._buffers.pop("graph_loop", None)
            if previous is not None:
                previous.graph = None
            del previous
            gc.collect()
# ... 85 lines not shown
```

diffusion_for_multi_scale_molecular_dynamics_amd/kernels.py:

```python
import ctypes as C
import inspect
from collections import namedtuple
from dataclasses import dataclass
from functools import lru_cache
from typing import Optional

import torch

from . import _hip
from ._hip import Mlp, PcFlags, Rng, Schedule, call, lib

F32, F64, I64, I32 = torch.float32, torch.float64, torch.int64, torch.int32


@dataclass
class DeviceSchedule:

    total_time_steps: int
    num_classes: int
    sigma_min: float
    time: torch.Tensor
    sigma: torch.Tensor
    sigma_squared: torch.Tensor
    g: torch.Tensor
# ... 6 lines not shown
    q_bar_matrix: torch.Tensor
    q_bar_tm1_matrix: torch.Tensor

    def __post_init__(self):
        self.c_struct = Schedule(self.total_time_steps, self.num_classes, float(self.sigma_min),
                                 self.time.data_ptr(), self.sigma.data_ptr(), self.g.data_ptr(),
                                 self.g_squared.data_ptr(), self.epsilon.data_ptr(), self.q_matrix.data_ptr(),
                                 self.q_bar_matrix.data_ptr(), self.q_bar_tm1_matrix.data_ptr())

    @property
    def device(self):
        return self.time.device


def noise_schedule_build(total_time_steps: int, schedule_type: str, time_delta: float, sigma_min: float,
                         sigma_max: float, corrector_step_epsilon: float, num_classes: int,
                         device: torch.device) -> DeviceSchedule:
    device = torch.device(device)
    if device.type != "cuda":
        raise _hip.MdxError(f"schedule tables are built on the GPU; got device {device}")
    T, Cn = int(total_time_steps), int(num_classes)
    st = {"exponential": 0, "linear": 1}[schedule_type]
    with torch.cuda.device(device):
        vec = [torch.empty(T, dtype=F32, device=device) for _ in range(9)]
        mats = [torch.empty(T, Cn, Cn, dtype=F32, device=device) for _ in range(3)]
        call("mdx_noise_schedule_build", T, st, float(time_delta), float(sigma_min), float(sigma_max),
             float(corrector_step_epsilon), Cn, *vec, *mats)
    time, sigma, sigma2, g, g2, eps, s2e, beta, ab = vec
    q, qb, qbm = mats
    return DeviceSchedule(T, Cn, float(sigma_min), time, sigma, sigma2, g, g2, eps, s2e, beta, ab, q, qb, qbm)


def index_set(d_index: torch.Tensor, value: int):
    call("mdx_index_set", d_index, int(value))


def index_add(d_index: torch.Tensor, delta: int):
    call("mdx_index_add", d_index, int(delta))


def fill_time_sigma(sched: DeviceSchedule, mode: int, index_i: int, d_index: Optional[torch.Tensor],
                    time_out: torch.Tensor, sigma_out: torch.Tensor):
    batch = time_out.numel()
    assert sigma_out.numel() == batch
    call("mdx_fill_time_sigma", C.byref(sched.c_struct), mode, int(index_i), d_index, time_out, sigma_out, batch)


def relative_coordinates_update(x, s, z, score_weight=None, gaussian_noise_weight=None, sigma=None, out=None, weights=None):
    assert x.shape == s.shape == z.shape
    out = torch.empty_like(x) if out is None else out
    if weights is not None:
        assert weights.numel() == 3
        call("mdx_relative_coordinates_update_dev", x, s, z, weights, x.numel(), out)
        return out
    call("mdx_relative_coordinates_update", x, s, z, float(score_weight), float(gaussian_noise_weight), float(sigma), x.numel(), out)
    return out


def lattice_parameters_update(l, s, z, score_weight=None, gaussian_noise_weight=None, sigma_n=None, out=None, weights=None):
    assert l.shape == s.shape == z.shape
    out = torch.empty_like(l) if out is None else out
    if weights is not None:
        assert weights.numel() == 3
        call("mdx_lattice_parameters_update_dev", l, s, z, weights, l.numel(), out)
        return out
    call("mdx_lattice_parameters_update", l, s, z, float(score_weight), float(gaussian_noise_weight), float(sigma_n), l.numel(), out)
    return out


def atom_types_update(logits, atom_types, q, q_bar, q_bar_tm1, gumbel, u, small_epsilon: float, greedy: bool,
                      one_transition: bool, return_probabilities: bool = False):
    B, N, Cn = logits.shape
    assert atom_types.shape == (B, N) and gumbel.shape == (B, N, Cn)
    assert q.shape == q_bar.shape == q_bar_tm1.shape == (Cn, Cn)
    out = torch.empty_like(atom_types)
    p_out = torch.empty_like(logits) if return_probabilities else None
    call("mdx_atom_types_update", logits, atom_types, q, q_bar, q_bar_tm1, gumbel, u, B, N, Cn, float(small_epsilon),
         int(bool(greedy)), int(bool(one_transition)), out, p_out)
    return (out, p_out) if return_probabilities else out


def pc_step_update(sched: DeviceSchedule, mode: int, index_i: int, d_index: Optional[torch.Tensor], flags: PcFlags,
                   atom_types, x, l, logits, score_x, score_l, z_coordinates, gumbel, u, z_lattice, rng: Rng,
                   atom_types_out, x_out, l_out, status: Optional[torch.Tensor]):
    B, N, d = x.shape
    call("mdx_pc_step_update", C.byref(sched.c_struct), int(mode), int(index_i), d_index, C.byref(flags), atom_types, x, l,
         logits, score_x, score_l, z_coordinates, gumbel, u, z_lattice, rng, B, N, d, atom_types_out, x_out, l_out, status)


def adaptive_corrector_statistics(sched: DeviceSchedule, index_i: int, d_index: Optional[torch.Tensor], score_x, score_l,
                                  z_coordinates, z_lattice_for_step_size, rng: Rng, use_fixed_lattice_parameters: bool,
                                  corrector_r: float, small_epsilon: float, workspace, totals, weights=None):
    B, N, d = score_x.shape
    assert workspace.numel() == 4 * B and totals.numel() == 8 and (weights is None or weights.numel() == 6)
    call("mdx_adaptive_corrector_statistics", C.byref(sched.c_struct), int(index_i), d_index, score_x, score_l, z_coordinates,
         z_lattice_for_step_size, rng, B, N, d, int(bool(use_fixed_lattice_parameters)), float(corrector_r),
         float(small_epsilon), workspace, totals, weights)


def adaptive_corrector_step_size(sched: DeviceSchedule, index_i: int, d_index: Optional[torch.Tensor], totals,
                                 number_of_atoms: int, spatial_dimension: int, use_fixed_lattice_parameters: bool,
                                 corrector_r: float, small_epsilon: float, weights):
    assert totals.numel() == 8 and weights.numel() == 6
    call("mdx_adaptive_corrector_step_size", C.byref(sched.c_struct), int(index_i), d_index, totals, int(number_of_atoms),
         int(spatial_dimension), int(bool(use_fixed_lattice_parameters)), float(corrector_r), float(small_epsilon), weights)


def adaptive_corrector_update(sched: DeviceSchedule, mode: int, index_i: int, d_index: Optional[torch.Tensor], flags: PcFlags,
                              atom_types, x, l, logits, score_x, score_l, z_coordinates, gumbel, u, z_lattice, weights,
                              rng: Rng, atom_types_out, x_out, l_out, status: Optional[torch.Tensor]):
    B, N, d = x.shape
    call("mdx_adaptive_corrector_update", C.byref(sched.c_struct), int(mode), int(index_i), d_index, C.byref(flags), atom_types,
         x, l, logits, score_x, score_l, z_coordinates, gumbel, u, z_lattice, weights, rng, B, N, d, atom_types_out, x_out, l_out,
         status)


def noise_relative_coordinates(x0, z, sigma, out=None):
    assert x0.shape == z.shape
    out = torch.empty_like(x0) if out is None else out
    if isinstance(sigma, torch.Tensor):
        assert sigma.shape == x0.shape, "sigmas array is expected to be of the same shape as the real_relative_coordinates array"
        call("mdx_noise_relative_coordinates_sigmas", x0, z, sigma, x0.numel(), out)
        return out
    call("mdx_noise_relative_coordinates", x0, z, float(sigma), x0.numel(), out)
    return out


def noise_lattice_parameters(l0, z, sigmas_n):
    assert l0.shape == z.shape == sigmas_n.shape
    out = torch.empty_like(l0)
    call("mdx_noise_lattice_parameters", l0, z, sigmas_n, l0.numel(), out)
    return out


def noise_atom_types(a0, q_bar, u):
    Cn = u.shape[-1]
    assert u.shape[:-1] == a0.shape
    out = torch.empty_like(a0)
    if q_bar.dim() > 2:
        assert q_bar.shape == tuple(a0.shape) + (Cn, Cn), "q_bar array first dimensions should match real_atom_types array"
        call("mdx_noise_atom_types_per_atom", a0, q_bar, u, a0.numel(), Cn, out)
        return out
    assert q_bar.shape == (Cn, Cn)
    call("mdx_noise_atom_types", a0, q_bar, u, a0.numel(), Cn, out)
    return out


def repaint_constrained_rows(sched: DeviceSchedule, index_i: int, d_index, constrained_x, constrained_a,
                             constrained_indices, z, u, rng: Rng, x_inout, a_inout):
    B, N, d = x_inout.shape
    K = constrained_x.shape[0]
    call("mdx_repaint_constrained_rows", C.byref(sched.c_struct), int(index_i), d_index, constrained_x, constrained_a,
         constrained_indices, K, z, u, rng, B, N, d, x_inout, a_inout)


def forward_diffusion_step(sched: DeviceSchedule, index_i: int, d_index, z, u, rng: Rng, x_inout, a_inout):
    B, N, d = x_inout.shape
    call("mdx_forward_diffusion_step", C.byref(sched.c_struct), int(index_i), d_index, z, u, rng, B, N, d, x_inout, a_inout)


def repaint_rows_per_sample(sched: DeviceSchedule, index_i: int, d_index, constrained_x, constrained_a, constrained_indices,
                            counts, sample_environment, z, u, rng: Rng, x_inout, a_inout):
    B, N, d = x_inout.shape
    E, K = constrained_a.shape
    assert constrained_x.shape == (E, K, d) and constrained_indices.shape == (E, K) and counts.shape == (E,)
    assert sample_environment.shape == (B,) and a_inout.shape == (B, N)
    call("mdx_repaint_rows_per_sample", C.byref(sched.c_struct), int(index_i), d_index, constrained_x, constrained_a,
         constrained_indices, counts, E, K, sample_environment, z, u, rng, B, N, d, x_inout, a_inout)
# ... 1258 lines not shown
        assert W == pack.hidden and agg.shape == node_in.shape
        call("mdx_node_mlp_rows_split", C.byref(pack.c_struct), node_in, agg, int(bool(add_residual)), M, None, out, proj, status)
        return (out, proj) if pack.projects else out
    assert W == 2 * pack.hidden
    call("mdx_node_mlp_rows", C.byref(pack.c_struct), node_in, int(bool(add_residual)), M, None, out, proj, status)
    return (out, proj) if pack.projects else out


def mlp_chain_rows(pack: RowChainPack, x, residual=None, status=None) -> torch.Tensor:
    M, H = x.shape
    assert H == pack.hidden and (residual is None or residual.shape == x.shape)
    out = torch.empty_like(x)
    call("mdx_mlp_chain_rows", C.byref(pack.c_struct), x, residual, M, None, out, status)
    return out


def egnn_edge_chain(pack: EdgeChainPack, node_proj, coord, edges, status=None, n_edges_dev=None, piece_sums: bool = False,
                    memo: Optional["EgnnTableMemo"] = None, sigma=None):
    E, H = edges.shape[0], pack.hidden
    pack.c_struct.message_mode = 1 if piece_sums else 0
    assert node_proj.shape[1] == 2 * H and coord.shape[0] == node_proj.shape[0]
    if memo is not None:
        assert not piece_sums and sigma is not None and tuple(memo.values.shape) == (E, H)
        call("mdx_egnn_edge_chain_keyed", C.byref(pack.c_struct), node_proj, coord, coord.shape[1], edges, E, n_edges_dev,
             memo.values, memo.scalars, status, memo.key, sigma)
        return memo.values, memo.scalars
    rows = lib().mdx_egnn_piece_rows(E, node_proj.shape[0]) if piece_sums else E
    messages = torch.empty(rows, H, dtype=F32, device=edges.device)
    scalar = torch.empty(E, dtype=F32, device=edges.device)
    call("mdx_egnn_edge_chain", C.byref(pack.c_struct), node_proj, coord, coord.shape[1], edges, E, n_edges_dev, messages, scalar,
         status)
    return messages, scalar


def segment_combine(pieces, n_edges: int, offsets, degree, mean: bool, left=None) -> torch.Tensor:
    n_nodes, H = degree.shape[0], pieces.shape[1]
    assert left is None or tuple(left.shape) == (n_nodes, H)
    assert pieces.shape[0] == lib().mdx_egnn_piece_rows(n_edges, n_nodes), "pieces: not the compact layout of n_edges, n_nodes"
    out = torch.empty(n_nodes, H if left is None else 2 * H, dtype=F32, device=pieces.device)
    call("mdx_segment_combine", pieces, n_edges, offsets, degree, n_nodes, H, int(bool(mean)), left, out)
    return out


def coord_flags(normalize: bool, tanh: bool) -> int:
    return (_hip.EGNN_COORD_NORMALIZE if normalize else 0) | (_hip.EGNN_COORD_TANH if tanh else 0)


def egnn_node_gather(pieces, n_edges: int, offsets, degree, mean_messages: bool, left, edge_scalar, coord, edges,
                     mean_coords: bool, flags: int = 0):
    if pieces is None:
        assert left is None
        coord_out = torch.empty_like(coord)
        call("mdx_egnn_node_gather", None, n_edges, offsets, degree, degree.shape[0], 4, int(bool(mean_messages)), None, None,
             edge_scalar, coord, coord.shape[1], edges, int(bool(mean_coords)), int(flags), coord_out)
        return None, coord_out
    n_nodes, H = degree.shape[0], pieces.shape[1]
    assert left is None or tuple(left.shape) == (n_nodes, H)
    assert pieces.shape[0] == lib().mdx_egnn_piece_rows(n_edges, n_nodes), "pieces: not the compact layout of n_edges, n_nodes"
    out = torch.empty(n_nodes, H if left is None else 2 * H, dtype=F32, device=pieces.device)
    coord_out = torch.empty_like(coord)
    call("mdx_egnn_node_gather", pieces, n_edges, offsets, degree, n_nodes, H, int(bool(mean_messages)), left, out, edge_scalar,
         coord, coord.shape[1], edges, int(bool(mean_coords)), int(flags), coord_out)
    return out, coord_out


TABLE_INV_SPACING = 256.0
TABLE_TOLERANCE = 2.0 ** -16


TABLE_NO_KEY = _hip.EGNN_TABLE_NO_KEY


class EgnnTableMemo:

    def __init__(self, n_classes: int, n_even: int, hidden: int, embedding_width: int, coord_dimension: int, device):
        K = 2 * n_even - 1
        rows, G = n_classes * n_classes * K, n_classes * (K + 1)
        self.n_classes, self.n_even = n_classes, n_even
        self.values = torch.zeros(rows, hidden, dtype=F32, device=device)
        self.scalars = torch.zeros(rows, dtype=F32, device=device)
        self.grid_z = torch.zeros(G, coord_dimension, dtype=F32, device=device)
        self.grid_h = torch.zeros(G, embedding_width, dtype=F32, device=device)
        self.grid_proj = torch.zeros(G, 2 * hidden, dtype=F32, device=device)
        self.workspace = torch.zeros(n_classes ** 2 * (hidden + 2), dtype=I32, device=device)
        self.worst = torch.zeros(1, dtype=F32, device=device)
        self.key = torch.tensor([TABLE_NO_KEY, 0], dtype=I32, device=device)
        self.stamp = None

    def reset(self):
        self.key[:1].fill_(TABLE_NO_KEY)

    def builds(self) -> int:
        return int(self.key[1].item())


@dataclass
class EgnnTable:
    grid_proj: torch.Tensor
    sigma: torch.Tensor
    atom_types: torch.Tensor
    n_classes: int
    n_even: int
    memo: EgnnTableMemo


def egnn_table_points(coord_dimension: int) -> int:
    import math
    return int(math.ceil(math.sqrt(2.0 * coord_dimension) * TABLE_INV_SPACING)) + 3


_TABLE_GRIDS = {}


def egnn_table_grid(n_classes: int, n_even: int, coord_dimension: int, device):
    key = (n_classes, n_even, coord_dimension, str(device))
    if key not in _TABLE_GRIDS:
        K = 2 * n_even - 1
        r = torch.arange(K, dtype=torch.float64)
        rho = torch.where(r < n_even, r, r - n_even + 0.5) / TABLE_INV_SPACING
        classes = torch.cat([torch.arange(n_classes), torch.arange(n_classes).repeat_interleave(K)])
        coord = torch.zeros(n_classes * (K + 1), coord_dimension, dtype=F32)
        coord[n_classes:, 0] = rho.to(F32).repeat(n_classes)
        a = torch.arange(n_classes).repeat_interleave(n_classes * K)
        dst = n_classes + torch.arange(n_classes * K).repeat(n_classes)
        edges = torch.stack([a, dst], dim=1)
        _TABLE_GRIDS[key] = (classes.to(device), coord.to(device), edges.contiguous().to(device))
    return _TABLE_GRIDS[key]


def egnn_table_check(table, table_scalar, n_classes: int, n_even: int, sigma, workspace, worst=None, status=None, key=None):
    H = table.shape[1]
    assert table.shape[0] == n_classes * n_classes * (2 * n_even - 1) and workspace.numel() >= n_classes ** 2 * (H + 2)
    call("mdx_egnn_table_check_keyed", table, table_scalar, H, n_classes, n_even, sigma, sigma.numel(), TABLE_TOLERANCE, workspace,
         worst, status, key)


def egnn_table_gather(table, table_scalar, n_classes: int, n_even: int, atom_types, offsets, degree, mean_messages: bool, left,
                      coord, edges, mean_coords: bool, flags: int = 0, status=None):
    n_nodes, H = degree.shape[0], table.shape[1]
    assert left is None or tuple(left.shape) == (n_nodes, H)
    assert atom_types.shape[0] == n_nodes and table.shape[0] == n_classes * n_classes * (2 * n_even - 1)
    out = torch.empty(n_nodes, H if left is None else 2 * H, dtype=F32, device=table.device)
    coord_out = torch.empty_like(coord)
    call("mdx_egnn_table_gather", table, table_scalar, H, n_classes, n_even, TABLE_INV_SPACING, atom_types, offsets, degree,
         n_nodes, int(bool(mean_messages)), left, out, coord, coord.shape[1], edges, int(bool(mean_coords)), int(flags), coord_out,
         status)
    return out, coord_out


def egnn_node_inputs(x, k_vectors, sigma, atom_types, emb_weight, emb_bias, second=None, memo: Optional[EgnnTableMemo] = None,
                     with_h: bool = True):
    B, N, d = x.shape
    assert d == 3 and k_vectors.shape[1] == 3
    n_nodes, n_k, (H, F) = B * N, k_vectors.shape[0], emb_weight.shape
    w2, b2 = second if second is not None else (None, None)
    assert second is None or (w2.shape[1] == F and b2.shape[0] == w2.shape[0])
    H2 = w2.shape[0] if second is not None else 0
    if memo is not None:
        z, h, h2 = memo.grid_z, memo.grid_h, memo.grid_proj
        assert second is not None and tuple(z.shape) == (n_nodes, 2 * n_k) and tuple(h.shape) == (n_nodes, H) and \
            tuple(h2.shape) == (n_nodes, H2)
    else:
        z = torch.empty(n_nodes, 2 * n_k, dtype=F32, device=x.device)
        h = torch.empty(n_nodes, H, dtype=F32, device=x.device) if with_h else None
        h2 = torch.empty(n_nodes, H2, dtype=F32, device=x.device) if second is not None else None
    call("mdx_egnn_node_inputs_keyed", x, k_vectors, n_k, sigma, N, atom_types, emb_weight, emb_bias, F, H, n_nodes, z, h, w2, b2,
         H2, h2, memo.key if memo is not None else None)
    return (z, h) if second is None else (z, h, h2)


def egnn_scores(z, x_hat, k_vectors):
    n_nodes, n_k = z.shape[0], k_vectors.shape[0]
    assert z.shape == x_hat.shape == (n_nodes, 2 * n_k)
    out = torch.empty(n_nodes, 3, dtype=F32, device=z.device)
    call("mdx_egnn_scores", z, x_hat, k_vectors, n_k, n_nodes, out)
    return out


def egnn_outputs(z, x_hat, k_vectors, h, class_weight, class_bias, mask_class: int, n_zero: int):
    n_nodes, n_k = z.shape[0], k_vectors.shape[0]
    C, H = class_weight.shape
    assert z.shape == x_hat.shape == (n_nodes, 2 * n_k) and h.shape == (n_nodes, H) and class_bias.shape == (C,)
    scores = torch.empty(n_nodes, 3, dtype=F32, device=z.device)
    logits = torch.empty(n_nodes, C, dtype=F32, device=z.device)
    zeros = torch.empty(int(n_zero), dtype=F32, device=z.device)
    call("mdx_egnn_outputs", z, x_hat, k_vectors, n_k, h, class_weight, class_bias, H, C, int(mask_class), n_nodes, scores, logits,
         zeros if n_zero else None, int(n_zero))
    return scores, logits, zeros


def egnn_coord_aggregate(edge_scalar, coord, edges, offsets, degree, mean: bool, flags: int = 0) -> torch.Tensor:
    out = torch.empty_like(coord)
    call("mdx_egnn_coord_aggregate", edge_scalar, coord, coord.shape[1], edges, offsets, degree, coord.shape[0], int(bool(mean)),
         int(flags), out)
    return out


RNG_UNIFORM, RNG_NORMAL, RNG_GUMBEL = 0, 1, 2


def rng_fill(kind: int, seed: int, call: int, draw: int, tag: int, n_items: int, width: int, device) -> torch.Tensor:
    out = torch.empty(n_items, width, dtype=F32, device=device)
    _hip.call("mdx_rng_fill", kind, int(seed) & 0xFFFFFFFFFFFFFFFF, int(call), int(draw), int(tag), n_items, width, out)
    return out


def math_probe(fn: int, x: torch.Tensor) -> torch.Tensor:
    y = torch.empty_like(x)
    call("mdx_math_probe", fn, x, x.numel(), y)
    return y
```

diffusion_for_multi_scale_molecular_dynamics_amd/models/egnn.py:

```python
from typing import Callable, List, NamedTuple, Optional, Tuple

import torch
from torch import nn

from .. import kernels
from ..namespace import AXL


def run_mlp(layers, x: torch.Tensor) -> torch.Tensor:
    for layer in layers:
        x = layer(x)
    return x


class RoutePath(NamedTuple):
    edge: str
    sums: str
    reduce: str
    sliced: bool = False
    node: str = "torch"
    coords_only: bool = False
    class_rows: bool = False
    projects_next: bool = False
    message_input: bool = False
# ... 237 lines not shown

    def _node_chain_pack(self):
        linears = self._node_linears()
        if linears is None:
            return None
        rest = linears[1:]
        if linears[0].out_features != rest[0].in_features or not kernels.RowChainPack.supported(rest):
            return None
        precision = self.edge_chain_precision
        stamp = (precision,) + kernels.parameter_stamp(*(t for lin in rest for t in (lin.weight, lin.bias)))
        return self.device_state.pack("rows", precision, stamp, lambda: kernels.RowChainPack(
            rest, precision, scales=self._scales("rows", len(rest), rest[0].weight.device)))

    def _node_mlp_pack(self, next_layer=None):
        linears = self._node_linears()
        if linears is None or not kernels.NodeMlpPack.supported(linears):
            return None
        next_pack = next_layer._edge_chain_pack() if next_layer is not None and next_layer.use_fused_ops else None
        projection = None
        if next_pack is not None and tuple(next_pack.proj_weight.shape) == (2 * linears[0].out_features, linears[0].out_features) \
                and next_pack.hidden == linears[0].out_features and next_pack.message_width == next_pack.hidden:
            projection = next_pack.proj_weight
        first_next = next_layer.message_mlp[0].weight if projection is not None else None
        precision = self.edge_chain_precision
        stamp = (precision,) + kernels.parameter_stamp(*(t for lin in linears for t in (lin.weight, lin.bias)), first_next)
        return self.device_state.pack("node", precision, stamp, lambda: kernels.NodeMlpPack(
            linears, precision, next_projection=projection,
            scales=self._scales("node", kernels.NodeMlpPack.n_chain_layers(linears), linears[0].weight.device)))

    def _coord_head_is_plain(self) -> bool:
        last = self.coord_mlp[-1]
        return isinstance(last, nn.Linear) and last.out_features == 1 and last.bias is None and \
            last.in_features % 4 == 0 and len(self.coord_mlp) >= 2 and isinstance(self.coord_mlp[-2], nn.SiLU)

    def forward(self, h: torch.Tensor, edge_index: torch.Tensor, coord: torch.Tensor,
                degree: Optional[torch.Tensor] = None, offsets: Optional[torch.Tensor] = None,
                n_edges: Optional[torch.Tensor] = None, node_proj: Optional[torch.Tensor] = None,
                next_layer: Optional["E_GCL"] = None, table=None, coords_only: bool = False,
                row_class: Optional[torch.Tensor] = None) -> Tuple[torch.Tensor, torch.Tensor]:
        if degree is None:
            degree = torch.bincount(edge_index[:, 0], minlength=h.shape[0])
        needs_grad = torch.is_grad_enabled() and (h.requires_grad or coord.requires_grad or
                                                  any(t.requires_grad for t in self.parameters()))
        route = self.route(degree.shape[0], h.shape[1], coord.shape[1], edge_index.shape[0], h.is_cuda and not needs_grad,
                           offsets is not None, next_layer, table is not None, coords_only, row_class is not None)
        out, coord, _ = self.run(route, h, edge_index, coord, degree, offsets, n_edges, node_proj, table, row_class)
        return out, coord

    def route(self, n_nodes: int, width: int, coord_dimension: int, n_edge_rows: int, fused: bool, has_offsets: bool,
              next_layer: Optional["E_GCL"] = None, table: bool = False, coords_only: bool = False,
              class_rows: bool = False) -> Route:
        fused = fused and self.use_fused_ops
        pack = self._edge_chain_pack() if fused and has_offsets and n_edge_rows > 0 else None
        if pack is None:
            linears = [m for m in self.message_mlp if isinstance(m, nn.Linear)]
            message_input = fused and linears[0].out_features % 4 == 0 and isinstance(self.message_mlp[1], nn.SiLU)
            segments = fused and has_offsets and linears[-1].out_features % 4 == 0
            return Route(RoutePath("torch", "rows" if segments else "torch",
                              "coord_head" if segments and self._coord_head_is_plain() else "torch", message_input=message_input))
        pieces = pack.piece_sums_ok and n_nodes < (1 << 31)
        full = pack.message_width == pack.hidden
        gather_covers = pieces and full and width == pack.hidden and coord_dimension <= 8
        on_table = table and gather_covers and not self.attention and pack.hidden <= 256 and self.status_word is not None
        edge, sums = ("table", "table") if on_table else ("chain", "pieces" if pieces else "rows")
        if gather_covers and coords_only and not on_table and not self.attention:
            return Route(RoutePath(edge, sums, "gather", node="none", coords_only=True), pack)
        whole = self._node_mlp_pack(next_layer) if gather_covers else None
        if whole is not None and whole.hidden == width:
            return Route(RoutePath(edge, sums, "gather", node="pack", class_rows=class_rows and on_table,
                              projects_next=whole.projects), pack, whole)
        rows = self._node_chain_pack()
        if rows is not None and self.residual and width != rows.hidden:
            rows = None
        return Route(RoutePath(edge, sums, "gather" if gather_covers else "aggregate", not full,
                          node="torch" if rows is None else "rows"), pack, rows)

    def _table_gather(self, pack, table, left, coord, edge_index, offsets, degree):
        _, grid_coord, grid_edges = kernels.egnn_table_grid(table.n_classes, table.n_even, coord.shape[1], coord.device)
        memo = table.memo
        values, scalars = kernels.egnn_edge_chain(pack, memo.grid_proj, grid_coord, grid_edges, status=self.status_word,
                                                  memo=memo, sigma=table.sigma)
        self.device_state.table_worst = memo.worst
        kernels.egnn_table_check(values, scalars, table.n_classes, table.n_even, table.sigma, memo.workspace,
                                 worst=memo.worst, status=self.status_word, key=memo.key)
        return kernels.egnn_table_gather(values, scalars, table.n_classes, table.n_even, table.atom_types, offsets, degree,
                                         self.message_mean, left, coord, edge_index, self.coords_mean,
                                         flags=self._coord_flags(), status=self.status_word)

    def run(self, route: Route, h, edge_index, coord, degree, offsets=None, n_edges=None, node_proj=None, table=None,
            row_class=None):
        path, pack = route.path, route.edge_pack
        assert (row_class is not None) == path.class_rows, "class rows go to a layer whose route reads them, and only there"
        if pack is None:
            return self._run_torch(path, h, edge_index, coord, degree, offsets, n_edges) + (None,)
        coord = coord.contiguous()
        n_rows, flags = edge_index.shape[0], self._coord_flags()
        if path.edge == "table":
            def gather(left):
                return self._table_gather(pack, table, left, coord, edge_index, offsets, degree)
        else:
            proj = node_proj if node_proj is not None else torch.nn.functional.linear(h, pack.proj_weight)
            pieces = path.sums == "pieces"
            messages, edge_scalar = kernels.egnn_edge_chain(pack, proj.contiguous(), coord, edge_index, status=self.status_word,
                                                            n_edges_dev=n_edges, piece_sums=pieces)
            if path.coords_only:
                return kernels.egnn_node_gather(None, n_rows, offsets, degree, self.message_mean, None, edge_scalar, coord,
                                                edge_index, self.coords_mean, flags=flags) + (None,)

            def gather(left):
                if path.reduce == "gather":
                    return kernels.egnn_node_gather(messages, n_rows, offsets, degree, self.message_mean, left, edge_scalar,
                                                    coord, edge_index, self.coords_mean, flags=flags)
                coord_out = kernels.egnn_coord_aggregate(edge_scalar, coord, edge_index, offsets, degree, self.coords_mean,
                                                         flags=flags)
                agg = (kernels.segment_combine(messages, n_rows, offsets, degree, self.message_mean) if pieces
                       else kernels.segment_rows(messages, offsets, degree, self.message_mean))
                if path.sliced:
                    agg = agg[:, :pack.message_width]
                return torch.cat([left, agg], dim=1), coord_out
        if path.node == "pack":
            h = h.contiguous()
            agg, coord_out = gather(None)
            out = kernels.node_mlp_rows(route.node_pack, h, self.residual, status=self.status_word, agg=agg, row_class=row_class)
            out, next_proj = out if path.projects_next else (out, None)
            return out, coord_out, next_proj
        node_in, coord_out = gather(h.contiguous())
        if path.node == "rows":
            first = self.node_mlp[0]
            hidden = torch.nn.functional.silu(torch.nn.functional.linear(node_in, first.weight, first.bias))
            out = kernels.mlp_chain_rows(route.node_pack, hidden, residual=h.contiguous() if self.residual else None,
                                         status=self.status_word)
            return out, coord_out, None
        out = run_mlp(self.node_mlp, node_in)
        return (h + out if self.residual else out), coord_out, None

    def _run_torch(self, path: RoutePath, h, edge_index, coord, degree, offsets, n_edges):
        assert n_edges is None, "a capacity-sized edge list needs the fused edge chain in every layer"
        row, col = edge_index[:, 0], edge_index[:, 1]
        count = degree.clamp(min=1).to(h.dtype).unsqueeze(1)

        coord_diff = coord.index_select(0, row) - coord.index_select(0, col)
        radial = (coord_diff ** 2).sum(dim=1, keepdim=True)
        if self.normalize:
            coord_diff = torch.tanh(radial) / torch.sqrt(radial + self.epsilon ** 2) * coord_diff

        messages = self._messages(h, edge_index, radial, path.message_input)

        if path.reduce == "coord_head":
            hidden = run_mlp(list(self.coord_mlp)[:-1], messages)
            coord = coord + kernels.egnn_coord_head(hidden.contiguous(), self.coord_mlp[-1].weight.reshape(-1),
                                                    coord_diff.contiguous(), offsets, degree, self.coords_mean)
        else:
            trans = segment_sum_sorted(coord_diff * run_mlp(self.coord_mlp, messages), degree)
            coord = coord + (trans / count if self.coords_mean else trans)

        if path.sums == "rows":
            agg = kernels.segment_rows(messages.contiguous(), offsets, degree, self.message_mean)
        else:
            agg = segment_sum_sorted(messages, degree)
            if self.message_mean:
                agg = agg / count
        out = run_mlp(self.node_mlp, torch.cat([h, agg], dim=1))
        return (h + out if self.residual else out), coord


class EGNN(nn.Module):

# ... 73 lines not shown
```

diffusion_for_multi_scale_molecular_dynamics_amd/models/score_networks/egnn_score_network.py:

```python
import itertools
import math
from dataclasses import dataclass
from typing import AnyStr, Callable, Dict, Optional, Union

import torch

from ...namespace import AXL, NOISE, NOISY_AXL_COMPOSITION
from ...utils import neighbors
from ..egnn import EGNN
from .score_network import ScoreNetwork, ScoreNetworkParameters


@dataclass(kw_only=True)
class EGNNScoreNetworkParameters(ScoreNetworkParameters):

    architecture: str = "egnn"
    number_of_bloch_wave_shells: int = 1
    message_n_hidden_dimensions: int = 1
    message_hidden_dimensions_size: int = 16
    node_n_hidden_dimensions: int = 1
    node_hidden_dimensions_size: int = 32
    coordinate_n_hidden_dimensions: int = 1
    coordinate_hidden_dimensions_size: int = 32
    residual: bool = True
    attention: bool = False
    normalize: bool = False
    tanh: bool = False
    coords_agg: str = "mean"
    message_agg: str = "mean"
    n_layers: int = 4
    edges: str = "fully_connected"
    radial_cutoff: Union[float, None] = None
    drop_duplicate_edges: bool = True


def complete_lattice_shells(number_of_complete_shells: int, spatial_dimension: int):
    n = 2 * number_of_complete_shells
    vectors = [v for v in itertools.product(range(-n, n + 1), repeat=spatial_dimension) if any(v)]
    vectors.sort(key=lambda v: (sum(c * c for c in v), tuple(-c for c in v)))
    seen, shells, previous_norm = set(), [], 0
    for v in vectors:
        if v in seen:
            continue
        orbit = set()
        for perm in itertools.permutations(range(spatial_dimension)):
            for signs in itertools.product((-1, 1), repeat=spatial_dimension):
                orbit.add(tuple(signs[k] * v[perm[k]] for k in range(spatial_dimension)))
        seen |= orbit
        shells.append(sorted(orbit, reverse=True))
        norm = sum(c * c for c in v)
        if len(shells) >= number_of_complete_shells and norm > previous_norm:
            break
        previous_norm = norm
    return shells


def positive_bloch_wave_vectors(number_of_complete_shells: int, spatial_dimension: int) -> torch.Tensor:
    half = []
    for shell in complete_lattice_shells(number_of_complete_shells, spatial_dimension):
        known = set()
        for v in shell:
            if v in known:
                continue
            half.append(v)
            known |= {v, tuple(-c for c in v)}
    return torch.tensor(half, dtype=torch.float32)


class EGNNScoreNetwork(ScoreNetwork):

    def __init__(self, hyper_params: EGNNScoreNetworkParameters, edge_builder: Optional[Callable] = None):
        super().__init__(hyper_params)
        hp = hyper_params
        self.number_of_features_per_node = self.num_atom_types + 2
        self.number_of_bloch_wave_shells = hp.number_of_bloch_wave_shells
        k_vectors = positive_bloch_wave_vectors(hp.number_of_bloch_wave_shells, self.spatial_dimension)
        self.register_parameter("bloch_wave_reciprocal_lattice_vectors",
                                torch.nn.Parameter(k_vectors, requires_grad=False))
        self.register_parameter("projection_matrices",
                                torch.nn.Parameter(self._projection_matrices(k_vectors), requires_grad=False))
        assert hp.edges in ("fully_connected", "radial_cutoff"), \
            f"Edges type should be fully_connected or radial_cutoff. Got {hp.edges}"
        self.edges = hp.edges
        self.radial_cutoff = hp.radial_cutoff
        if self.edges == "fully_connected":
            assert self.radial_cutoff is None, "Specifying a radial cutoff is inconsistent with edges=fully_connected."
        else:
            assert type(self.radial_cutoff) is float, \
                "A floating point value for the radial cutoff is needed for edges=radial_cutoff."
        self.drop_duplicate_edges = hp.drop_duplicate_edges
        self.edge_builder = edge_builder
        self.graph_status = None
        self.static_edge_list_max_fraction = 0.5
        self._logged_two_call_switch = False
        self.first_layer_table = "auto"
        self.sigma_uniform_hint = False
        self.first_layer_table_reuse = True
        self.skip_unread_logits = True
        self.logits_unread_hint = False
        self.first_layer_class_rows = True
        self.egnn = self._make_egnn(hp)

    def __getstate__(self):
        state = dict(self.__dict__)
        state.pop("_fully_connected_edges", None)
        state.pop("_table_grid_x", None)
        return state

    @property
    def edge_chain_precision(self):
        return self.egnn.graph_layers[0].edge_chain_precision if len(self.egnn.graph_layers) else None

    @edge_chain_precision.setter
    def edge_chain_precision(self, value):
        for layer in self.egnn.graph_layers:
            layer.edge_chain_precision = value

    def adapt_f16_range(self):
        for layer in self.egnn.graph_layers:
            layer.adapt_f16_range()

    def begin_f16_range_fallback(self):
        for layer in self.egnn.graph_layers:
            layer.begin_f16_range_fallback()

    def reset_f16_range(self):
        for layer in self.egnn.graph_layers:
            layer.reset_f16_range()

    def table_builds(self) -> int:
        return self.egnn.graph_layers[0].table_builds() if len(self.egnn.graph_layers) else 0

    def check_status(self):
        if self.graph_status is not None:
            try:
                neighbors._raise_if_cutoff_too_large(self.graph_status)
            finally:
                self.graph_status.zero_()

    def _impose_non_mask_atomic_type_prediction(self, output: AXL):
        if output.A is not None and not getattr(output.A, "_mdx_mask_imposed", False):
            super()._impose_non_mask_atomic_type_prediction(output)

    def _routes(self, n_nodes: int, coord_dimension: int, n_edge_rows: int, **wishes):
        return self.egnn.routes(n_nodes, coord_dimension, n_edge_rows, True, True, **wishes)

    def _first_projection_of_inputs(self, pack=None):
        from ... import kernels
        layers = self.egnn.graph_layers
        if len(layers) == 0 or not layers[0].use_fused_ops:
            return None
        if pack is None:
            pack = layers[0]._edge_chain_pack()
        emb = self.egnn.embedding_in
        if pack is None or pack.proj_weight.shape[1] != emb.out_features:
            return None
        first = layers[0].message_mlp[0].weight
        stamp = kernels.parameter_stamp(first, emb.weight, emb.bias) + (layers[0].edge_chain_precision,)
        if getattr(self, "_first_projection", (None, None))[0] != stamp:
            with torch.no_grad():
                w2 = (pack.proj_weight.double() @ emb.weight.double()).float().contiguous()
                b2 = (pack.proj_weight.double() @ emb.bias.double()).float().contiguous()
            self._first_projection = (stamp, (w2, b2))
        return self._first_projection[1]

    def _table_serves_first_layer(self, n_edge_rows: int, coord_dimension: int) -> bool:
        from ... import kernels
        mode = self.first_layer_table
        if mode not in ("auto", "on", "off"):
            raise ValueError(f"first_layer_table should be auto, on or off. Got {mode}")
        if mode != self.__dict__.get("_table_mode_seen", mode) and len(self.egnn.graph_layers):
            self.egnn.graph_layers[0].reset_table_memos()
        self._table_mode_seen = mode
        if mode == "off" or (mode == "auto" and not self.sigma_uniform_hint):
            return False
        n_classes = self.num_atom_types + 1
        n_even = kernels.egnn_table_points(coord_dimension)
        return not (mode == "auto" and n_classes ** 2 * (2 * n_even - 1) * 8 > n_edge_rows)

    def _class_rows_serve_first_layer(self) -> bool:
        return self.first_layer_class_rows and self.sigma_uniform_hint

    def _first_layer_table(self, edges, z, h, sigma, atom_types, k_vectors, second, route=None):
        from ... import kernels
        if route is None:
            route = self._routes(z.shape[0], z.shape[1], edges.shape[0],
                                 table=self._table_serves_first_layer(edges.shape[0], z.shape[1]))[0]
        if route.path.edge != "table":
            return None
        layer = self.egnn.graph_layers[0]
        n_classes = self.num_atom_types + 1
        n_even = kernels.egnn_table_points(z.shape[1])
        classes, _, _ = kernels.egnn_table_grid(n_classes, n_even, z.shape[1], z.device)
        G = classes.shape[0]
        grid_x = self.__dict__.get("_table_grid_x")
        if grid_x is None or grid_x.shape[1] != G or grid_x.device != z.device:
            grid_x = self._table_grid_x = torch.zeros(1, G, 3, dtype=torch.float32, device=z.device)
        sigma = sigma.to(device=z.device, dtype=torch.float32).reshape(-1).contiguous()
        emb = self.egnn.embedding_in
        stamp = kernels.parameter_stamp(emb.weight, emb.bias, *second)
        memo = layer.table_memo(route.edge_pack, n_classes, n_even, emb.out_features, z.shape[1], z.device, stamp)
        if not self.first_layer_table_reuse:
            memo.reset()
        _, _, grid_proj = kernels.egnn_node_inputs(grid_x, k_vectors.contiguous(), sigma, classes.reshape(1, G),
                                                   emb.weight.detach().contiguous(), emb.bias.detach().contiguous(), second=second,
                                                   memo=memo)
        return kernels.EgnnTable(grid_proj=grid_proj, sigma=sigma, atom_types=atom_types.reshape(-1).long().contiguous(),
                                 n_classes=n_classes, n_even=n_even, memo=memo)

    def _make_egnn(self, hp):
        return EGNN(
            input_size=self.number_of_features_per_node, num_classes=self.num_atom_types + 1,
            message_n_hidden_dimensions=hp.message_n_hidden_dimensions,
            message_hidden_dimensions_size=hp.message_hidden_dimensions_size,
            node_n_hidden_dimensions=hp.node_n_hidden_dimensions,
            node_hidden_dimensions_size=hp.node_hidden_dimensions_size,
            coordinate_n_hidden_dimensions=hp.coordinate_n_hidden_dimensions,
            coordinate_hidden_dimensions_size=hp.coordinate_hidden_dimensions_size,
            residual=hp.residual, attention=hp.attention, normalize=hp.normalize, tanh=hp.tanh,
            coords_agg=hp.coords_agg, message_agg=hp.message_agg, n_layers=hp.n_layers)

    @staticmethod
    def _projection_matrices(k_vectors: torch.Tensor) -> torch.Tensor:
        n_k, d = k_vectors.shape
        gamma = torch.zeros(d, 2 * n_k, 2 * n_k)
        for k in range(n_k):
            gamma[:, 2 * k, 2 * k + 1] = -k_vectors[k]
            gamma[:, 2 * k + 1, 2 * k] = k_vectors[k]
        return gamma

    def _build_edges(self, relative_coordinates: torch.Tensor, lattice_parameters: torch.Tensor, routes=None):
        bsz, n, d = relative_coordinates.shape
        if self.edges == "fully_connected":
            key = (n, bsz, str(relative_coordinates.device))
            cache = self.__dict__.setdefault("_fully_connected_edges", {})
            if key not in cache:
                if len(cache) >= 8:
                    cache.clear()
                cache[key] = (neighbors.get_edges_batch(n, bsz, device=relative_coordinates.device),
                              torch.full((bsz * n,), n - 1, dtype=torch.int64, device=relative_coordinates.device))
            return cache[key]
        if self.edge_builder is not None:
            lengths = lattice_parameters[:, :d].clip(min=2.2 * self.radial_cutoff)
            return self.edge_builder(relative_coordinates, torch.diag_embed(lengths), self.radial_cutoff)
        if self.graph_status is None or self.graph_status.device != relative_coordinates.device:
            self.graph_status = torch.zeros(1, dtype=torch.int32, device=relative_coordinates.device)
        capacity = bsz * n * (n - 1)
        if relative_coordinates.is_cuda and not torch.is_grad_enabled() and self._static_edge_list_fits(bsz, n, relative_coordinates.device, routes):
            edges, degree, offsets, n_edges = neighbors.get_edges_static_clipped(
                relative_coordinates, lattice_parameters.to(torch.float32), 2.2 * self.radial_cutoff, self.radial_cutoff,
                capacity, status=self.graph_status)
            return edges, (degree, offsets, n_edges)
        lengths = lattice_parameters[:, :d].clip(min=2.2 * self.radial_cutoff)
        return neighbors.get_edges_with_radial_cutoff(relative_coordinates, torch.diag_embed(lengths), self.radial_cutoff,
                                                      status=self.graph_status, return_degree=True)

    def _static_edge_list_fits(self, bsz: int, n: int, device, routes=None) -> bool:
        capacity = bsz * n * (n - 1)
        if self.spatial_dimension != 3:
            return False
        if capacity <= 0:
            return False
        if routes is None:
            routes = self._routes(bsz * n, 2 * self.bloch_wave_reciprocal_lattice_vectors.shape[0], capacity)
        if not all(route.edge_pack is not None for route in routes):
            return False
        width = max((route.edge_pack.hidden for route in routes), default=0)
        needed = capacity * 20 + (capacity // 16 + bsz * n) * width * 4
        key = (str(device), capacity, width, self.static_edge_list_max_fraction)
        decisions = self.__dict__.setdefault("_static_decisions", {})
        if key not in decisions and not torch.cuda.is_current_stream_capturing():
            free = torch.cuda.mem_get_info(device)[0] + torch.cuda.memory_reserved(device) - torch.cuda.memory_allocated(device)
            decisions[key] = (needed <= self.static_edge_list_max_fraction * free, free)
        fits, free = decisions.get(key, (True, 0))
        if not fits and not self._logged_two_call_switch:
            import logging
            logging.getLogger(__name__).warning(
                "EGNN radius graph: a capacity-sized edge list would take %.1f GB of the %.1f GB free on the device; using "
                "the two-call protocol (one host read per forward, the sampler iteration is not captured in a hipGraph)",
                needed / 2 ** 30, free / 2 ** 30)
            self._logged_two_call_switch = True
        return fits

    def capture_safe(self, batch_size: int, number_of_atoms: int, device) -> bool:
        if self.edges == "fully_connected":
            return True
        if self.edge_builder is not None:
            return False
        return self._static_edge_list_fits(batch_size, number_of_atoms, torch.device(device))

    def _forward_unchecked(self, batch: Dict[AnyStr, torch.Tensor], conditional: bool = False) -> AXL:
        comp = batch[NOISY_AXL_COMPOSITION]
        x = comp.X
        bsz, n, d = x.shape
        if x.is_cuda and (self.graph_status is None or self.graph_status.device != x.device):
            self.graph_status = torch.zeros(1, dtype=torch.int32, device=x.device)
        for layer in self.egnn.graph_layers:
            layer.status_word = self.graph_status if x.is_cuda else None
        emb = self.egnn.embedding_in
        sigma_in = batch[NOISE]
        fused = (x.is_cuda and not torch.is_grad_enabled() and d == 3 and x.dtype == torch.float32 and
                 emb.in_features == self.num_atom_types + 2 and sigma_in.numel() == bsz)
        head = self.egnn.node_classification_layer
        one_launch_head = head.out_features <= 8 and head.in_features % 4 == 0 and comp.L.dtype == torch.float32
        coord_dimension = 2 * self.bloch_wave_reciprocal_lattice_vectors.shape[0]

        def forward_routes(n_edge_rows):
            return self._routes(bsz * n, coord_dimension, n_edge_rows,
                                table=self._table_serves_first_layer(n_edge_rows, coord_dimension),
                                class_rows=self._class_rows_serve_first_layer(),
                                coords_only=one_launch_head and self.skip_unread_logits and self.logits_unread_hint)

        capacity = bsz * n * (n - 1)
        routes = forward_routes(capacity) if fused and self.edges == "radial_cutoff" and self.edge_builder is None and \
            capacity > 0 else None
        edges, degree = self._build_edges(x, comp.L, routes)
        if fused:
            from ... import kernels
            k_vectors = self.bloch_wave_reciprocal_lattice_vectors.to(x)
            if routes is None or edges.shape[0] != capacity:
                routes = forward_routes(edges.shape[0])
            first = routes[0] if routes else None
            second = self._first_projection_of_inputs(first.edge_pack) if first is not None else None
            class_rows = first is not None and first.path.class_rows
            inputs = kernels.egnn_node_inputs(x.contiguous(), k_vectors.contiguous(),
                                              sigma_in.to(device=x.device, dtype=torch.float32).reshape(-1).contiguous(),
                                              comp.A.reshape(bsz, n).long().contiguous(), emb.weight.detach().contiguous(),
                                              emb.bias.detach().contiguous(), second=None if class_rows else second,
                                              with_h=not class_rows)
            z, h = inputs[:2]
            first_proj = inputs[2] if second is not None and not class_rows else None
            table = row_class = None
            if first is not None and first.path.edge == "table":
                table = self._first_layer_table(edges, z, h, sigma_in, comp.A, k_vectors, second, route=first)
            if class_rows:
                h, row_class = table.memo.grid_h[:table.n_classes], table.atom_types
            out = self.egnn(h, edges, z, degree, routes=routes, first_proj=first_proj, first_table=table,
                            first_row_class=row_class)
            h, x_hat = out.A, out.X
            if routes and routes[-1].path.coords_only:
                scores = kernels.egnn_scores(z, x_hat.contiguous(), k_vectors.contiguous())
                return AXL(A=None, X=scores.reshape(bsz, n, d), L=torch.zeros_like(comp.L))
            if one_launch_head:
                scores, logits, zeros = kernels.egnn_outputs(
                    z, x_hat.contiguous(), k_vectors.contiguous(), h.contiguous(), head.weight.detach().contiguous(),
                    head.bias.detach().contiguous(), self.num_atom_types, comp.L.numel())
                logits = logits.reshape(bsz, n, -1)
                logits._mdx_mask_imposed = True
                return AXL(A=logits, X=scores.reshape(bsz, n, d), L=zeros.reshape(comp.L.shape))
            logits = head(h)
            scores = kernels.egnn_scores(z, x_hat.contiguous(), k_vectors.contiguous())
            return AXL(A=logits.reshape(bsz, n, -1), X=scores.reshape(bsz, n, d), L=torch.zeros_like(comp.L))

        flat = x.reshape(bsz * n, d)
        k_vectors = self.bloch_wave_reciprocal_lattice_vectors.to(flat)
        if flat.is_cuda:
            kr = ((2.0 * math.pi * flat)[:, None, :] * k_vectors[None, :, :]).sum(dim=-1)
        else:
            kr = (2.0 * math.pi * flat) @ k_vectors.t()
        if flat.is_cuda:
            kr64 = kr.double()
            z = torch.stack([kr64.cos().to(kr.dtype), kr64.sin().to(kr.dtype)], dim=2).reshape(bsz * n, -1)
        else:
            z = torch.stack([kr.cos(), kr.sin()], dim=2).reshape(bsz * n, -1)

        sigmas = batch[NOISE].to(x.device).repeat_interleave(n, dim=0)
        one_hot = torch.nn.functional.one_hot(comp.A.reshape(-1).long(), self.num_atom_types + 1).to(x.dtype)
        h = torch.cat([sigmas, one_hot], dim=1)

        out = self.egnn(h=h, edges=edges, x=z, degree=degree)
        gamma = self.projection_matrices.to(z)
        if z.is_cuda:
            scores = ((z[:, None, :, None] * gamma[None]) * out.X[:, None, None, :]).sum(dim=(2, 3))
        else:
            scores = torch.einsum("ni,aij,nj->na", z, gamma, out.X)
        return AXL(A=out.A.reshape(bsz, n, -1), X=scores.reshape(bsz, n, d), L=torch.zeros_like(comp.L))
```

include/mdx_hip.h:

```cpp
#ifndef MDX_HIP_H
#define MDX_HIP_H

#include <stdint.h>

#ifdef __cplusplus
extern "C" {
#endif

#define MDX_ABI_VERSION 14

#define MDX_OK 0
#define MDX_ERR_INVALID_ARG (-1)
#define MDX_ERR_UNSUPPORTED (-2)
#define MDX_ERR_HIP (-3)

#define MDX_STATUS_CUTOFF_TOO_LARGE 1u
#define MDX_STATUS_MASK_AT_LAST_STEP 2u
#define MDX_STATUS_EGNN_F16_RANGE 4u
#define MDX_STATUS_GRAPH_CAPACITY 8u
#define MDX_STATUS_EGNN_TABLE 16u
#define MDX_STATUS_SW_NEIGHBOURS 32u
#define MDX_STATUS_SW_ATOM_TYPE 64u
#define MDX_STATUS_ANALYTICAL_SIGMA 128u
#define MDX_STATUS_ANALYTICAL_COORDINATES 256u
// ... 29 lines not shown
#define MDX_TAG_FILL_UNIFORM 11
#define MDX_TAG_FILL_TYPE 12
#define MDX_TAG_FILL_VOXEL 13

#if defined(__GNUC__)
#define MDX_API __attribute__((visibility("default")))
#else
#define MDX_API
#endif

typedef void* mdx_stream_t;

typedef struct mdx_schedule {
    int32_t total_time_steps;
    int32_t num_classes;
    double sigma_min;
    const float* time;
    const float* sigma;
    const float* g;
    const float* g_squared;
    const float* epsilon;
    const float* q_matrix;
    const float* q_bar_matrix;
    const float* q_bar_tm1_matrix;
} mdx_schedule_t;

typedef struct mdx_rng {
    uint64_t seed;
    uint32_t call;
    uint32_t draw_stride;
    uint32_t draw_offset;
    uint32_t reserved;
    const uint32_t* call_dev;
} mdx_rng_t;

typedef struct mdx_pc_flags {
    int32_t atom_type_greedy_sampling;
    int32_t one_atom_type_transition_per_step;
    int32_t use_fixed_lattice_parameters;
    int32_t update_atom_types;
    float small_epsilon;
} mdx_pc_flags_t;

MDX_API int mdx_abi_version(void);
MDX_API const char* mdx_status_string(int status);

MDX_API int mdx_noise_schedule_build(int total_time_steps, int schedule_type, double time_delta, double sigma_min,
                             double sigma_max, double corrector_step_epsilon, int num_classes, float* time,
                             float* sigma, float* sigma_squared, float* g, float* g_squared, float* epsilon,
                             float* sqrt_2_epsilon, float* beta, float* alpha_bar, float* q_matrix,
                             float* q_bar_matrix, float* q_bar_tm1_matrix, mdx_stream_t stream);

MDX_API int mdx_index_set(int32_t* d_index, int32_t value, mdx_stream_t stream);
MDX_API int mdx_index_add(int32_t* d_index, int32_t delta, mdx_stream_t stream);

MDX_API int mdx_fill_time_sigma(const mdx_schedule_t* sched_host, int mode, int index_i, const int32_t* d_index,
                        float* time_out, float* sigma_out, int64_t batch, mdx_stream_t stream);

MDX_API int mdx_relative_coordinates_update(const float* x, const float* sigma_normalized_scores, const float* z,
                                    float score_weight, float gaussian_noise_weight, float sigma, int64_t count,
                                    float* out, mdx_stream_t stream);

MDX_API int mdx_lattice_parameters_update(const float* l, const float* sigma_normalized_scores, const float* z,
                                  float score_weight, float gaussian_noise_weight, float sigma_n, int64_t count,
                                  float* out, mdx_stream_t stream);

MDX_API int mdx_relative_coordinates_update_dev(const float* x, const float* sigma_normalized_scores, const float* z,
                                        const float* weights, int64_t count, float* out, mdx_stream_t stream);
MDX_API int mdx_lattice_parameters_update_dev(const float* l, const float* sigma_normalized_scores, const float* z,
                                      const float* weights, int64_t count, float* out, mdx_stream_t stream);

MDX_API int mdx_atom_types_update(const float* logits, const int64_t* atom_types, const float* q, const float* q_bar,
                          const float* q_bar_tm1, const float* gumbel, const float* u, int64_t batch,
                          int number_of_atoms, int num_classes, float small_epsilon, int greedy,
                          int one_transition, int64_t* atom_types_out, float* probabilities_out,
                          mdx_stream_t stream);

MDX_API int mdx_pc_step_update(const mdx_schedule_t* sched_host, int mode, int index_i, const int32_t* d_index,
                       const mdx_pc_flags_t* flags_host, const int64_t* atom_types, const float* x, const float* l,
                       const float* logits, const float* score_x, const float* score_l, const float* z_coordinates,
                       const float* gumbel, const float* u, const float* z_lattice, mdx_rng_t rng, int64_t batch,
                       int number_of_atoms, int spatial_dimension, int64_t* atom_types_out, float* x_out,
                       float* l_out, uint32_t* status, mdx_stream_t stream);

MDX_API int mdx_adaptive_corrector_statistics(const mdx_schedule_t* sched_host, int index_i, const int32_t* d_index,
                                      const float* score_x, const float* score_l, const float* z_coordinates,
                                      const float* z_lattice_for_step_size, mdx_rng_t rng, int64_t batch,
                                      int number_of_atoms, int spatial_dimension, int use_fixed_lattice_parameters,
                                      float corrector_r, float small_epsilon, float* workspace, double* totals,
                                      float* weights, mdx_stream_t stream);
MDX_API int mdx_adaptive_corrector_step_size(const mdx_schedule_t* sched_host, int index_i, const int32_t* d_index,
                                     const double* totals, int number_of_atoms, int spatial_dimension,
                                     int use_fixed_lattice_parameters, float corrector_r, float small_epsilon,
                                     float* weights, mdx_stream_t stream);
MDX_API int mdx_adaptive_corrector_update(const mdx_schedule_t* sched_host, int mode, int index_i, const int32_t* d_index,
                                  const mdx_pc_flags_t* flags_host, const int64_t* atom_types, const float* x,
                                  const float* l, const float* logits, const float* score_x, const float* score_l,
                                  const float* z_coordinates, const float* gumbel, const float* u, const float* z_lattice,
                                  const float* weights, mdx_rng_t rng, int64_t batch, int number_of_atoms,
                                  int spatial_dimension, int64_t* atom_types_out, float* x_out, float* l_out,
                                  uint32_t* status, mdx_stream_t stream);

MDX_API int mdx_noise_relative_coordinates(const float* x0, const float* z, float sigma, int64_t count, float* out,
                                   mdx_stream_t stream);

MDX_API int mdx_noise_atom_types(const int64_t* a0, const float* q_bar, const float* u, int64_t n_atoms, int num_classes,
                         int64_t* out, mdx_stream_t stream);

MDX_API int mdx_noise_relative_coordinates_sigmas(const float* x0, const float* z, const float* sigmas, int64_t count,
                                                  float* out, mdx_stream_t stream);
MDX_API int mdx_noise_atom_types_per_atom(const int64_t* a0, const float* q_bar, const float* u, int64_t n_atoms,
                                          int num_classes, int64_t* out, mdx_stream_t stream);
MDX_API int mdx_noise_lattice_parameters(const float* l0, const float* z, const float* sigmas_n, int64_t count, float* out,
                                         mdx_stream_t stream);

MDX_API int mdx_repaint_constrained_rows(const mdx_schedule_t* sched_host, int index_i, const int32_t* d_index,
                                 const float* constrained_x, const int64_t* constrained_a,
                                 const int64_t* constrained_indices, int number_of_constraints, const float* z,
                                 const float* u, mdx_rng_t rng, int64_t batch, int number_of_atoms,
                                 int spatial_dimension, float* x_inout, int64_t* a_inout, mdx_stream_t stream);

MDX_API int mdx_repaint_rows_per_sample(const mdx_schedule_t* sched_host, int index_i, const int32_t* d_index,
                                        const float* constrained_x, const int64_t* constrained_a,
                                        const int64_t* constrained_indices, const int32_t* counts,
                                        int number_of_environments, int capacity, const int32_t* sample_environment,
                                        const float* z, const float* u, mdx_rng_t rng, int64_t batch, int number_of_atoms,
                                        int spatial_dimension, float* x_inout, int64_t* a_inout, mdx_stream_t stream);

#define MDX_EXCISE_RADIUS 0
#define MDX_EXCISE_NEIGHBOURS 1
#define MDX_EXCISE_MAX_ATOMS 4096
MDX_API int mdx_excise_environments(const double* relative_coordinates, const double* box_sides, int number_of_atoms,
                                    int spatial_dimension, const int64_t* central_atoms, int number_of_environments, int mode,
                                    double radial_cutoff, int number_of_neighbors, int center_atoms, const double* new_box_sides,
                                    int capacity, int64_t* source_indices, float* constrained_x, int32_t* counts,
                                    uint32_t* status, mdx_stream_t stream);

MDX_API int mdx_edit_keep_mask(const float* relative_coordinates, const float* lattice_parameters, int lattice_stride,
                               const int32_t* sample_environment, const int32_t* active_atoms, const int32_t* counts,
                               int number_of_environments, double radius, int64_t batch, int number_of_atoms, int spatial_dimension, uint8_t* keep,
                               mdx_stream_t stream);

#define MDX_RANDOM_FILL_MAX_ATOMS 1024
#define MDX_RANDOM_FILL_MAX_VOXELS 4096
MDX_API int mdx_random_fill_proposals(uint64_t seed, uint32_t call, int64_t first_sample, int64_t batch, int max_attempts,
                                      int number_of_atoms, int spatial_dimension, int num_atom_types, int number_of_voxels,
                                      double* uniforms, int32_t* types, int32_t* voxels, mdx_stream_t stream);
MDX_API int mdx_random_fill_environments(const double* uniforms, const int32_t* types, const int32_t* voxels,
                                         const int32_t* partition, const double* constrained_x, const int64_t* constrained_a,
                                         const int32_t* counts, const int32_t* active, int number_of_environments,
                                         int constrained_capacity, const int32_t* sample_environment, const double* box_sides,
                                         int max_attempts, double minimal_interatomic_distance, int64_t batch,
                                         int number_of_atoms, int spatial_dimension, double* x, int64_t* a, int32_t* active_out,
                                         int32_t* attempts, uint8_t* accepted, double* min_distance, uint32_t* status,
                                         mdx_stream_t stream);

MDX_API int mdx_forward_diffusion_step(const mdx_schedule_t* sched_host, int index_i, const int32_t* d_index,
                                       const float* z, const float* u, mdx_rng_t rng, int64_t batch,
                                       int number_of_atoms, int spatial_dimension, float* x_inout, int64_t* a_inout,
                                       mdx_stream_t stream);

MDX_API int mdx_radius_graph_count(const float* cartesian_positions, const float* basis_vectors, float radial_cutoff,
                           int64_t batch, int number_of_atoms, int unique, int64_t* counts, uint32_t* status,
                           mdx_stream_t stream);
MDX_API int mdx_radius_graph_fill(const float* cartesian_positions, const float* basis_vectors, float radial_cutoff,
                          int64_t batch, int number_of_atoms, int unique, const int64_t* offsets,
// ... 151 lines not shown
                            float* score_x_out, float* score_l_out, mdx_stream_t stream);

#define MDX_MLP_SAMPLE_GENERIC_KERNEL 1u
#define MDX_MLP_SAMPLE_UNFOLDED 2u
#define MDX_MLP_SAMPLE_CALLER_NOISE 4u
#define MDX_MLP_SAMPLE_NO_FIXED_SOFTMAX 8u
#define MDX_MLP_SAMPLE_NO_P2_TABLE 16u
#define MDX_MLP_SAMPLE_PADDED_FAMILY 128u
#define MDX_MLP_SAMPLE_DIAG_NO_FORWARD 256u
#define MDX_MLP_SAMPLE_DIAG_NO_UPDATE 512u
MDX_API int64_t mdx_mlp_pc_sample_workspace_floats(const mdx_mlp_t* mlp_host, int number_of_corrector_steps,
                                                   int atom_type_transition_in_corrector, int n_iterations,
                                                   int64_t batch);
MDX_API int mdx_mlp_pc_sample_variant(const mdx_mlp_t* mlp_host, uint32_t options);
MDX_API int mdx_mlp_pc_sample(const mdx_schedule_t* sched_host, const mdx_mlp_t* mlp_host,
                              const mdx_pc_flags_t* flags_host, int number_of_corrector_steps,
                              int atom_type_transition_in_corrector, int start_index, int n_iterations, mdx_rng_t rng,
                              int64_t batch, int64_t* atom_types, float* x, float* l, float* noise_workspace,
                              int64_t workspace_floats, uint32_t options, uint32_t* status, mdx_stream_t stream);


MDX_API int mdx_egnn_message_input(const float* node_proj, const int64_t* edges, const float* radial, const float* bias,
                                   const float* w_radial, int64_t n_edges, int H, int silu, float* out,
                                   mdx_stream_t stream);

MDX_API int mdx_egnn_coord_head(const float* hidden, const float* w_out, const float* coord_diff, const int64_t* offsets,
                                const int64_t* degree, int64_t n_nodes, int H, int spatial_dimension, int mean,
                                float* trans, mdx_stream_t stream);
MDX_API int mdx_segment_rows(const float* data, const int64_t* offsets, const int64_t* degree, int64_t n_nodes, int H,
                             int mean, float* out, mdx_stream_t stream);

#define MDX_EGNN_CHAIN_MAX_LAYERS 16
#define MDX_EGNN_MESSAGES_ROWS 0
#define MDX_EGNN_MESSAGES_PIECE_SUMS 1
#define MDX_EGNN_F16_ACTIVATION_EXPONENT 6
typedef struct mdx_egnn_chain {
    int32_t hidden, n_message_layers, n_coord_layers, precision;
    int32_t message_mode, reserved;
    const void* weight_image;
    const float* biases;
    const float* bias_in;
    const float* w_radial;
    const int32_t* weight_exponents;
    const int32_t* activation_exponents;
    uint32_t* activation_maxima;
    const float* attention_weight;
    const float* attention_bias;
} mdx_egnn_chain_t;
#define MDX_EGNN_COORD_NORMALIZE 1
#define MDX_EGNN_COORD_TANH 2
MDX_API int mdx_egnn_chain_adapt_activation_exponents(uint32_t* maxima_inout, int count, int32_t* exponents_inout,
                                                      mdx_stream_t stream);
MDX_API int64_t mdx_egnn_chain_image_bytes(int hidden, int n_layers);
MDX_API int mdx_egnn_chain_pack(const float* const* weights_host, int n_layers, const float* w_out, int hidden,
                                int precision, uint32_t tied_layers, void* image_out, int32_t* exponents_out,
                                mdx_stream_t stream);
MDX_API int mdx_egnn_edge_chain(const mdx_egnn_chain_t* chain_host, const float* node_proj, const float* coord,
                                int coord_dimension, const int64_t* edges, int64_t n_edges, const int64_t* n_edges_dev,
                                float* messages_out, float* edge_scalar_out, uint32_t* status, mdx_stream_t stream);
MDX_API int64_t mdx_egnn_piece_rows(int64_t n_edges, int64_t n_nodes);
MDX_API int mdx_segment_combine(const float* pieces, int64_t n_edges, const int64_t* offsets, const int64_t* degree,
                                int64_t n_nodes, int H, int mean, const float* left, float* out, mdx_stream_t stream);
MDX_API int mdx_egnn_node_gather(const float* pieces, int64_t n_edges, const int64_t* offsets, const int64_t* degree,
                                 int64_t n_nodes, int H, int mean_messages, const float* left, float* out,
                                 const float* edge_scalar, const float* coord, int coord_dimension, const int64_t* edges,
                                 int mean_coords, int coord_flags, float* coord_out, mdx_stream_t stream);

MDX_API int mdx_egnn_table_check(const float* table, const float* table_scalar, int H, int n_classes, int n_even,
                                 const float* sigma, int64_t n_sigma, float tolerance, uint32_t* workspace, float* worst_out,
                                 uint32_t* status, mdx_stream_t stream);
#define MDX_EGNN_TABLE_NO_KEY 0x7fc00000u
MDX_API int mdx_egnn_node_inputs_keyed(const float* x, const float* k_vectors, int n_k, const float* sigma,
                                       int atoms_per_structure, const int64_t* atom_types, const float* emb_weight,
                                       const float* emb_bias, int n_features, int H, int64_t n_nodes, float* z_out, float* h_out,
                                       const float* second_weight, const float* second_bias, int second_width, float* second_out,
                                       const uint32_t* table_key, mdx_stream_t stream);
MDX_API int mdx_egnn_edge_chain_keyed(const mdx_egnn_chain_t* chain_host, const float* node_proj, const float* coord,
                                      int coord_dimension, const int64_t* edges, int64_t n_edges, const int64_t* n_edges_dev,
                                      float* messages_out, float* edge_scalar_out, uint32_t* status, const uint32_t* table_key,
                                      const float* sigma, mdx_stream_t stream);
MDX_API int mdx_egnn_table_check_keyed(const float* table, const float* table_scalar, int H, int n_classes, int n_even,
                                       const float* sigma, int64_t n_sigma, float tolerance, uint32_t* workspace,
                                       float* worst_out, uint32_t* status, uint32_t* table_key, mdx_stream_t stream);
MDX_API int mdx_egnn_table_gather(const float* table, const float* table_scalar, int H, int n_classes, int n_even,
                                  float inv_spacing, const int64_t* atom_types, const int64_t* offsets, const int64_t* degree,
                                  int64_t n_nodes, int mean_messages, const float* left, float* out, const float* coord,
                                  int coord_dimension, const int64_t* edges, int mean_coords, int coord_flags, float* coord_out,
                                  uint32_t* status, mdx_stream_t stream);

MDX_API int mdx_egnn_node_inputs(const float* x, const float* k_vectors, int n_k, const float* sigma, int atoms_per_structure,
                                 const int64_t* atom_types, const float* emb_weight, const float* emb_bias, int n_features,
                                 int H, int64_t n_nodes, float* z_out, float* h_out, const float* second_weight,
                                 const float* second_bias, int second_width, float* second_out, mdx_stream_t stream);
MDX_API int mdx_egnn_scores(const float* z, const float* x_hat, const float* k_vectors, int n_k, int64_t n_nodes,
                            float* scores_out, mdx_stream_t stream);

MDX_API int mdx_egnn_outputs(const float* z, const float* x_hat, const float* k_vectors, int n_k, const float* h,
                             const float* class_weight, const float* class_bias, int H, int num_classes, int mask_class,
                             int64_t n_nodes, float* scores_out, float* logits_out, float* zero_out, int64_t n_zero,
                             mdx_stream_t stream);

MDX_API int mdx_mlp_chain_rows(const mdx_egnn_chain_t* chain_host, const float* x, const float* residual, int64_t n_rows,
                               const int64_t* n_rows_dev, float* out, uint32_t* status, mdx_stream_t stream);
MDX_API int mdx_node_mlp_rows(const mdx_egnn_chain_t* chain_host, const float* node_in, int add_residual, int64_t n_rows,
                              const int64_t* n_rows_dev, float* out, float* proj_out, uint32_t* status, mdx_stream_t stream);
MDX_API int mdx_node_mlp_rows_split(const mdx_egnn_chain_t* chain_host, const float* h, const float* agg, int add_residual,
                                    int64_t n_rows, const int64_t* n_rows_dev, float* out, float* proj_out, uint32_t* status,
                                    mdx_stream_t stream);
MDX_API int mdx_node_mlp_rows_indexed(const mdx_egnn_chain_t* chain_host, const float* class_rows, int n_classes,
                                      const int64_t* row_class, const float* agg, int add_residual, int64_t n_rows,
                                      const int64_t* n_rows_dev, float* out, float* proj_out, uint32_t* status,
                                      mdx_stream_t stream);
MDX_API int mdx_egnn_coord_aggregate(const float* edge_scalar, const float* coord, int coord_dimension, const int64_t* edges,
                                     const int64_t* offsets, const int64_t* degree, int64_t n_nodes, int mean,
                                     int coord_flags, float* coord_out, mdx_stream_t stream);

MDX_API int mdx_rng_fill(int kind, uint64_t seed, uint32_t call, uint32_t draw, uint32_t tag, int64_t n_items, int width,
                 float* out, mdx_stream_t stream);

MDX_API int mdx_math_probe(int fn, const float* x, int64_t count, float* y, mdx_stream_t stream);

#ifdef __cplusplus
}
#endif
#endif
```

Measured before the change: 22.01.

## Merge glue kernels into single launches for node inputs, table check, scores, step update

Batch and grid node-input embedding now run in one paired kernel that splits blocks between the two problems. The table check and verdict kernels are combined, the zero-fill of the lattice output moves into the scores kernel, and a step-update variant also writes the next time and sigma. The aim is to cut kernel-launch overhead across the 1000-step sampling loop, at the cost of more branching inside kernels and new code paths gated on a uniform-sigma hint.

```diff
diff --git a/diffusion_for_multi_scale_molecular_dynamics_amd/csrc/mdx_egnn.hip b/diffusion_for_multi_scale_molecular_dynamics_amd/csrc/mdx_egnn.hip
--- a/diffusion_for_multi_scale_molecular_dynamics_amd/csrc/mdx_egnn.hip
+++ b/diffusion_for_multi_scale_molecular_dynamics_amd/csrc/mdx_egnn.hip
@@ -105,6 +105,58 @@
     return v;
 }
 
+__device__ __forceinline__ void node_inputs_rows(const float* __restrict__ x, const float* __restrict__ k_vectors, int n_k,
+                                                 const float* __restrict__ sigma, int atoms_per_structure,
+                                                 const int64_t* __restrict__ atom_types, const float* __restrict__ w,
+                                                 const float* __restrict__ b, int F, int H, int64_t n_nodes, float* __restrict__ z,
+                                                 float* __restrict__ h, const float* __restrict__ w2, const float* __restrict__ b2,
+                                                 int H2, float* __restrict__ h2, int block, int n_blocks)
+{
+    extern __shared__ float tables[];
+    float* t1 = tables;
+    float* t2 = tables + (1 + F) * H;
+    for (int j = threadIdx.x; h && j < H; j += blockDim.x) {
+        t1[j] = b[j];
+        for (int f = 0; f < F; ++f) t1[(1 + f) * H + j] = w[(int64_t)j * F + f];
+    }
+    if (h2)
+        for (int j = threadIdx.x; j < H2; j += blockDim.x) {
+            t2[j] = b2[j];
+            for (int f = 0; f < F; ++f) t2[(1 + f) * H2 + j] = w2[(int64_t)j * F + f];
+        }
+    __syncthreads();
+    const int lane = threadIdx.x % 64;
+    const int64_t wave = (block * (int64_t)blockDim.x + threadIdx.x) / 64, n_waves = ((int64_t)n_blocks * blockDim.x) / 64;
+    const int per = n_k <= 64 ? min(4, 64 / n_k) : 1;
+    for (int64_t i0 = wave * per; i0 < n_nodes; i0 += n_waves * per) {
+        if (n_k <= 64) {
+            const int g = lane / n_k, k = lane - g * n_k;
+            const int64_t i = i0 + g;
+            if (g < per && i < n_nodes) {
+                float kr = 0.0f;
+                for (int d = 0; d < 3; ++d) kr = kr + (6.2831855f * x[3 * i + d]) * k_vectors[3 * k + d];
+                uplift(kr, z[2 * (i * n_k + k)], z[2 * (i * n_k + k) + 1]);
+            }
+        } else {
+            for (int k = lane; k < n_k; k += 64) {
+                float kr = 0.0f;
+                for (int d = 0; d < 3; ++d) kr = kr + (6.2831855f * x[3 * i0 + d]) * k_vectors[3 * k + d];
+                uplift(kr, z[2 * (i0 * n_k + k)], z[2 * (i0 * n_k + k) + 1]);
+            }
+        }
+        if (!h && !h2) continue;
+        for (int g = 0; g < per && i0 + g < n_nodes; ++g) {
+            const int64_t i = i0 + g;
+            const float s = sigma[i / atoms_per_structure];
+            const int64_t a = atom_types[i];
+            if (h2)
+                for (int q = lane; q < (H2 >> 2); q += 64) reinterpret_cast<float4*>(h2 + i * H2)[q] = embed_quad(t2, H2, q, s, a, F);
+            if (h)
+                for (int q = lane; q < (H >> 2); q += 64) reinterpret_cast<float4*>(h + i * H)[q] = embed_quad(t1, H, q, s, a, F);
+        }
+    }
+}
+
 __global__ __launch_bounds__(kBlock) void egnn_node_inputs_rows_kernel(const float* __restrict__ x, const float* __restrict__ k_vectors,
                                                                        int n_k, const float* __restrict__ sigma,
                                                                        int atoms_per_structure,
@@ -117,55 +169,40 @@
                                                                        const uint32_t* __restrict__ table_key)
 {
     if (mdx::table_is_current(table_key, sigma)) return;
-    extern __shared__ float tables[];
-    float* t1 = tables;
-    float* t2 = tables + (1 + F) * H;
-    for (int j = threadIdx.x; h && j < H; j += blockDim.x) {
-        t1[j] = b[j];
-        for (int f = 0; f < F; ++f) t1[(1 + f) * H + j] = w[(int64_t)j * F + f];
-    }
-    if (h2)
-        for (int j = threadIdx.x; j < H2; j += blockDim.x) {
-            t2[j] = b2[j];
-            for (int f = 0; f < F; ++f) t2[(1 + f) * H2 + j] = w2[(int64_t)j * F + f];
-        }
-    __syncthreads();
-    const int lane = threadIdx.x % 64;
-    const int64_t wave = (blockIdx.x * (int64_t)blockDim.x + threadIdx.x) / 64, n_waves = ((int64_t)gridDim.x * blockDim.x) / 64;
-    const int per = n_k <= 64 ? min(4, 64 / n_k) : 1;
-    for (int64_t i0 = wave * per; i0 < n_nodes; i0 += n_waves * per) {
-        if (n_k <= 64) {
-            const int g = lane / n_k, k = lane - g * n_k;
-            const int64_t i = i0 + g;
-            if (g < per && i < n_nodes) {
-                float kr = 0.0f;
-                for (int d = 0; d < 3; ++d) kr = kr + (6.2831855f * x[3 * i + d]) * k_vectors[3 * k + d];
-                uplift(kr, z[2 * (i * n_k + k)], z[2 * (i * n_k + k) + 1]);
-            }
-        } else {
-            for (int k = lane; k < n_k; k += 64) {
-                float kr = 0.0f;
-                for (int d = 0; d < 3; ++d) kr = kr + (6.2831855f * x[3 * i0 + d]) * k_vectors[3 * k + d];
-                uplift(kr, z[2 * (i0 * n_k + k)], z[2 * (i0 * n_k + k) + 1]);
-            }
-        }
-        if (!h && !h2) continue;
-        for (int g = 0; g < per && i0 + g < n_nodes; ++g) {
-            const int64_t i = i0 + g;
-            const float s = sigma[i / atoms_per_structure];
-            const int64_t a = atom_types[i];
-            if (h2)
-                for (int q = lane; q < (H2 >> 2); q += 64) reinterpret_cast<float4*>(h2 + i * H2)[q] = embed_quad(t2, H2, q, s, a, F);
-            if (h)
-                for (int q = lane; q < (H >> 2); q += 64) reinterpret_cast<float4*>(h + i * H)[q] = embed_quad(t1, H, q, s, a, F);
-        }
-    }
+    node_inputs_rows(x, k_vectors, n_k, sigma, atoms_per_structure, atom_types, w, b, F, H, n_nodes, z, h, w2, b2, H2, h2,
+                     (int)blockIdx.x, (int)gridDim.x);
+}
+
+struct NodeInputsProblem {
+    const float* x;
+    const float* sigma;
+    int atoms_per_structure;
+    const int64_t* atom_types;
+    int64_t n_nodes;
+    float *z, *h, *h2;
+};
+
+__global__ __launch_bounds__(kBlock) void egnn_node_inputs_pair_kernel(NodeInputsProblem batch, NodeInputsProblem grid, int batch_blocks,
+                                                                       const float* __restrict__ k_vectors, int n_k,
+                                                                       const float* __restrict__ w, const float* __restrict__ b,
+                                                                       int F, int H, const float* __restrict__ w2,
+                                                                       const float* __restrict__ b2, int H2,
+                                                                       const uint32_t* __restrict__ table_key)
+{
+    const bool of_grid = (int)blockIdx.x >= batch_blocks;
+    if (of_grid && mdx::table_is_current(table_key, grid.sigma)) return;
+    const NodeInputsProblem& q = of_grid ? grid : batch;
+    node_inputs_rows(q.x, k_vectors, n_k, q.sigma, q.atoms_per_structure, q.atom_types, w, b, F, H, q.n_nodes, q.z, q.h, w2, b2, H2,
+                     q.h2, of_grid ? (int)blockIdx.x - batch_blocks : (int)blockIdx.x,
+                     of_grid ? (int)gridDim.x - batch_blocks : batch_blocks);
 }
 
 __global__ __launch_bounds__(kBlock) void egnn_scores_kernel(const float* __restrict__ z, const float* __restrict__ x_hat,
                                                              const float* __restrict__ k_vectors, int n_k, int64_t n_nodes,
-                                                             float* __restrict__ scores)
-{
+                                                             float* __restrict__ scores, float* __restrict__ zero_out,
+                                                             int64_t n_zero)
+{
+    for (int64_t t = blockIdx.x * (int64_t)blockDim.x + threadIdx.x; t < n_zero; t += (int64_t)gridDim.x * blockDim.x) zero_out[t] = 0.0f;
     for (int64_t t = blockIdx.x * (int64_t)blockDim.x + threadIdx.x; t < n_nodes * 3; t += (int64_t)gridDim.x * blockDim.x) {
         const int64_t i = t / 3;
         const int alpha = (int)(t - 3 * i);
@@ -349,6 +386,18 @@
                                       stream);
 }
 
+static int64_t rows_blocks(int64_t n_nodes)
+{
+    const int64_t blocks = (n_nodes + 15) / 16;
+    return blocks > 2048 ? 2048 : blocks;
+}
+
+static bool rows_kernel_covers(int n_features, int H, bool second, int second_width, size_t& table_bytes)
+{
+    table_bytes = sizeof(float) * (size_t)(1 + n_features) * ((size_t)H + (second ? (size_t)second_width : 0));
+    return (H & 3) == 0 && (!second || (second_width & 3) == 0) && table_bytes <= 48 * 1024;
+}
+
 int mdx_egnn_node_inputs_keyed(const float* x, const float* k_vectors, int n_k, const float* sigma, int atoms_per_structure,
                                const int64_t* atom_types, const float* emb_weight, const float* emb_bias, int n_features, int H,
                                int64_t n_nodes, float* z_out, float* h_out, const float* second_weight, const float* second_bias,
@@ -358,10 +407,9 @@
     if (n_nodes == 0) return MDX_OK;
     if (!x || !k_vectors || !sigma || !atom_types || !emb_weight || !emb_bias || !z_out) return MDX_ERR_INVALID_ARG;
     if (second_out && (!second_weight || !second_bias || second_width < 1)) return MDX_ERR_INVALID_ARG;
-    const size_t table_bytes = sizeof(float) * (size_t)(1 + n_features) * ((size_t)H + (second_out ? (size_t)second_width : 0));
-    if ((H & 3) == 0 && (!second_out || (second_width & 3) == 0) && table_bytes <= 48 * 1024) {
-        int64_t blocks = (n_nodes + 15) / 16;
-        if (blocks > 2048) blocks = 2048;
+    size_t table_bytes = 0;
+    if (rows_kernel_covers(n_features, H, second_out != nullptr, second_width, table_bytes)) {
+        const int64_t blocks = rows_blocks(n_nodes);
         hipLaunchKernelGGL(egnn_node_inputs_rows_kernel, dim3((unsigned)blocks), dim3(kBlock), table_bytes,
                            as_stream(stream), x, k_vectors, n_k, sigma, atoms_per_structure, atom_types,
                            emb_weight, emb_bias, n_features, H, n_nodes, z_out, h_out, second_weight, second_bias, second_width,
@@ -376,17 +424,57 @@
     return launch_status();
 }
 
+int mdx_egnn_node_inputs_pair(const float* k_vectors, int n_k, const float* emb_weight, const float* emb_bias, int n_features,
+                              int H, const float* second_weight, const float* second_bias, int second_width, const float* x,
+                              const float* sigma, int atoms_per_structure, const int64_t* atom_types, int64_t n_nodes,
+                              float* z_out, float* h_out, float* second_out, const float* grid_x, const float* grid_sigma,
+                              int grid_atoms_per_structure, const int64_t* grid_atom_types, int64_t grid_nodes, float* grid_z_out,
+                              float* grid_h_out, float* grid_second_out, const uint32_t* table_key, mdx_stream_t stream)
+{
+    if (n_nodes < 1 || grid_nodes < 1 || n_k < 1 || atoms_per_structure < 1 || grid_atoms_per_structure < 1 || n_features < 2 ||
+        H < 1)
+        return MDX_ERR_INVALID_ARG;
+    if (!k_vectors || !emb_weight || !emb_bias || !x || !sigma || !atom_types || !z_out || !grid_x || !grid_sigma ||
+        !grid_atom_types || !grid_z_out)
+        return MDX_ERR_INVALID_ARG;
+    const bool second = second_out || grid_second_out;
+    if (second && (!second_weight || !second_bias || second_width < 1)) return MDX_ERR_INVALID_ARG;
+    size_t table_bytes = 0;
+    if (!rows_kernel_covers(n_features, H, second, second_width, table_bytes)) return MDX_ERR_UNSUPPORTED;
+    const int64_t batch_blocks = rows_blocks(n_nodes), grid_blocks = rows_blocks(grid_nodes);
+    const NodeInputsProblem batch{x, sigma, atoms_per_structure, atom_types, n_nodes, z_out, h_out, second_out};
+    const NodeInputsProblem grid{grid_x, grid_sigma, grid_atoms_per_structure, grid_atom_types, grid_nodes, grid_z_out, grid_h_out,
+                                 grid_second_out};
+    hipLaunchKernelGGL(egnn_node_inputs_pair_kernel, dim3((unsigned)(batch_blocks + grid_blocks)), dim3(kBlock), table_bytes,
+                       as_stream(stream), batch, grid, (int)batch_blocks, k_vectors, n_k, emb_weight, emb_bias, n_features, H,
+                       second_weight, second_bias, second_width, table_key);
+    return launch_status();
+}
+
+static int egnn_scores(const float* z, const float* x_hat, const float* k_vectors, int n_k, int64_t n_nodes, float* scores_out,
+                       float* zero_out, int64_t n_zero, mdx_stream_t stream)
+{
+    if (n_nodes < 0 || n_k < 1 || n_zero < 0 || (n_zero > 0 && !zero_out)) return MDX_ERR_INVALID_ARG;
+    if (n_nodes == 0 && n_zero == 0) return MDX_OK;
+    if (n_nodes > 0 && (!z || !x_hat || !k_vectors || !scores_out)) return MDX_ERR_INVALID_ARG;
+    int64_t blocks = (n_nodes * 3 + kBlock - 1) / kBlock;
+    if (blocks > 16384) blocks = 16384;
+    if (blocks < 1) blocks = 1;
+    hipLaunchKernelGGL(egnn_scores_kernel, dim3((unsigned)blocks), dim3(kBlock), 0, as_stream(stream), z, x_hat,
+                       k_vectors, n_k, n_nodes, scores_out, zero_out, n_zero);
+    return launch_status();
+}
+
 int mdx_egnn_scores(const float* z, const float* x_hat, const float* k_vectors, int n_k, int64_t n_nodes, float* scores_out,
                     mdx_stream_t stream)
 {
-    if (n_nodes < 0 || n_k < 1) return MDX_ERR_INVALID_ARG;
-    if (n_nodes == 0) return MDX_OK;
-    if (!z || !x_hat || !k_vectors || !scores_out) return MDX_ERR_INVALID_ARG;
-    int64_t blocks = (n_nodes * 3 + kBlock - 1) / kBlock;
-    if (blocks > 16384) blocks = 16384;
-    hipLaunchKernelGGL(egnn_scores_kernel, dim3((unsigned)blocks), dim3(kBlock), 0, as_stream(stream), z, x_hat,
-                       k_vectors, n_k, n_nodes, scores_out);
-    return launch_status();
+    return egnn_scores(z, x_hat, k_vectors, n_k, n_nodes, scores_out, nullptr, 0, stream);
+}
+
+int mdx_egnn_scores_zeros(const float* z, const float* x_hat, const float* k_vectors, int n_k, int64_t n_nodes, float* scores_out,
+                          float* zero_out, int64_t n_zero, mdx_stream_t stream)
+{
+    return egnn_scores(z, x_hat, k_vectors, n_k, n_nodes, scores_out, zero_out, n_zero, stream);
 }
 
 int mdx_egnn_outputs(const float* z, const float* x_hat, const float* k_vectors, int n_k, const float* h,
diff --git a/diffusion_for_multi_scale_molecular_dynamics_amd/csrc/mdx_egnn_table.hip b/diffusion_for_multi_scale_molecular_dynamics_amd/csrc/mdx_egnn_table.hip
--- a/diffusion_for_multi_scale_molecular_dynamics_amd/csrc/mdx_egnn_table.hip
+++ b/diffusion_for_multi_scale_molecular_dynamics_amd/csrc/mdx_egnn_table.hip
@@ -45,12 +45,9 @@
 __device__ __forceinline__ unsigned abs_bits(float v) { return __float_as_uint(v) & 0x7fffffffu; }
 
 constexpr int kCheckRows = 32;
-__global__ __launch_bounds__(256) void egnn_table_check_kernel(const float* __restrict__ messages, const float* __restrict__ scalar,
-                                                               int H, int n_pairs, int n_even, unsigned* __restrict__ workspace,
-                                                               const uint32_t* __restrict__ table_key,
-                                                               const float* __restrict__ sigma)
-{
-    if (table_is_current(table_key, sigma)) return;
+__device__ __forceinline__ void table_check_block(const float* __restrict__ messages, const float* __restrict__ scalar, int H,
+                                                  int n_pairs, int n_even, unsigned* __restrict__ workspace)
+{
     const int p = blockIdx.x, K = 2 * n_even - 1;
     const int j0 = blockIdx.y * kCheckRows, j1 = min(j0 + kCheckRows, n_even - 2);
     float w[4];
@@ -71,19 +68,32 @@
     }
 }
 
-__global__ __launch_bounds__(256) void egnn_table_verdict_kernel(unsigned* __restrict__ workspace, int n_pairs, int columns,
-                                                                 const float* __restrict__ sigma, int64_t n_sigma, float tolerance,
-                                                                 float* __restrict__ worst_out, uint32_t* __restrict__ status,
-                                                                 uint32_t* __restrict__ table_key)
+__global__ __launch_bounds__(256) void egnn_table_check_kernel(const float* __restrict__ messages, const float* __restrict__ scalar,
+                                                               int H, int n_pairs, int n_even, unsigned* __restrict__ workspace,
+                                                               const uint32_t* __restrict__ table_key,
+                                                               const float* __restrict__ sigma)
+{
+    if (table_is_current(table_key, sigma)) return;
+    table_check_block(messages, scalar, H, n_pairs, n_even, workspace);
+}
+
+template <bool ACROSS>
+__device__ __forceinline__ void table_verdict_block(unsigned* __restrict__ workspace, int n_pairs, int columns,
+                                                    const float* __restrict__ sigma, int64_t n_sigma, float tolerance,
+                                                    float* __restrict__ worst_out, uint32_t* __restrict__ status,
+                                                    uint32_t* __restrict__ table_key, bool built)
 {
     __shared__ float worst[256];
     __shared__ int bad[256];
     float mine = 0.0f;
     int fail = 0;
-    const bool built = !table_is_current(table_key, sigma);
     const int64_t n_entries = built ? (int64_t)n_pairs * columns : 0;
+    auto word = [&](int64_t i) -> unsigned {
+        if constexpr (ACROSS) return __hip_atomic_load(workspace + i, __ATOMIC_RELAXED, __HIP_MEMORY_SCOPE_AGENT);
+        else return workspace[i];
+    };
     for (int64_t i = threadIdx.x; i < n_entries; i += blockDim.x) {
-        const float err = __uint_as_float(workspace[i]), big = __uint_as_float(workspace[n_entries + i / columns]);
+        const float err = __uint_as_float(word(i)), big = __uint_as_float(word(n_entries + i / columns));
         if (!(err <= tolerance * big)) fail = 1;
         if (big > 0.0f) mine = fmaxf(mine, err / big);
         else if (err > 0.0f || err != err) mine = INFINITY;
@@ -116,6 +126,49 @@
             }
         }
     }
+}
+
+__global__ __launch_bounds__(256) void egnn_table_verdict_kernel(unsigned* __restrict__ workspace, int n_pairs, int columns,
+                                                                 const float* __restrict__ sigma, int64_t n_sigma, float tolerance,
+                                                                 float* __restrict__ worst_out, uint32_t* __restrict__ status,
+                                                                 uint32_t* __restrict__ table_key)
+{
+    table_verdict_block<false>(workspace, n_pairs, columns, sigma, n_sigma, tolerance, worst_out, status, table_key,
+                               !table_is_current(table_key, sigma));
+}
+
+__global__ __launch_bounds__(256) void egnn_table_check_verdict_kernel(const float* __restrict__ messages,
+                                                                       const float* __restrict__ scalar, int H, int n_pairs,
+                                                                       int n_even, unsigned* __restrict__ workspace,
+                                                                       const float* __restrict__ sigma, int64_t n_sigma,
+                                                                       float tolerance, float* __restrict__ worst_out,
+                                                                       uint32_t* __restrict__ status,
+                                                                       uint32_t* __restrict__ table_key)
+{
+    __shared__ int last;
+    const bool built = !table_is_current(table_key, sigma);
+    if (built) {
+        table_check_block(messages, scalar, H, n_pairs, n_even, workspace);
+        asm volatile("s_waitcnt vmcnt(0)" ::: "memory");
+    }
+    __syncthreads();
+    if (threadIdx.x == 0) {
+        unsigned* ticket = workspace + (int64_t)n_pairs * (H + 2);
+        if (built) {
+            __builtin_amdgcn_fence(__ATOMIC_RELEASE, "agent");
+            asm volatile("s_waitcnt vmcnt(0)" ::: "memory");
+        }
+        const unsigned drawn = atomicAdd(ticket, 1u);
+        last = drawn + 1u == gridDim.x * gridDim.y;
+        if (last) {
+            __builtin_amdgcn_fence(__ATOMIC_ACQUIRE, "agent");
+            asm volatile("s_waitcnt vmcnt(0)" ::: "memory");
+            *ticket = 0u;
+        }
+    }
+    __syncthreads();
+    if (!last) return;
+    table_verdict_block<true>(workspace, n_pairs, H + 1, sigma, n_sigma, tolerance, worst_out, status, table_key, built);
 }
 
 __global__ __launch_bounds__(256) void egnn_table_gather_kernel(const float* __restrict__ table, const float* __restrict__ table_scalar,
@@ -259,6 +312,20 @@
     return launch_status();
 }
 
+int mdx_egnn_table_check_verdict(const float* table, const float* table_scalar, int H, int n_classes, int n_even,
+                                 const float* sigma, int64_t n_sigma, float tolerance, uint32_t* workspace, float* worst_out,
+                                 uint32_t* status, uint32_t* table_key, mdx_stream_t stream)
+{
+    if (H < 1 || n_classes < 1 || n_even < 4 || n_sigma < 1 || !(tolerance >= 0.0f)) return MDX_ERR_INVALID_ARG;
+    if (!table || !table_scalar || !sigma || !workspace) return MDX_ERR_INVALID_ARG;
+    const int n_pairs = n_classes * n_classes;
+    hipLaunchKernelGGL(egnn_table_check_verdict_kernel,
+                       dim3((unsigned)n_pairs, (unsigned)((n_even - 2 + kCheckRows - 1) / kCheckRows)), dim3(256), 0,
+                       as_stream(stream), table, table_scalar, H, n_pairs, n_even, reinterpret_cast<unsigned*>(workspace), sigma,
+                       n_sigma, tolerance, worst_out, status, table_key);
+    return launch_status();
+}
+
 int mdx_egnn_table_gather(const float* table, const float* table_scalar, int H, int n_classes, int n_even, float inv_spacing,
                           const int64_t* atom_types, const int64_t* offsets, const int64_t* degree, int64_t n_nodes,
                           int mean_messages, const float* left, float* out, const float* coord, int coord_dimension,
diff --git a/diffusion_for_multi_scale_molecular_dynamics_amd/csrc/mdx_hip.hip b/diffusion_for_multi_scale_molecular_dynamics_amd/csrc/mdx_hip.hip
--- a/diffusion_for_multi_scale_molecular_dynamics_amd/csrc/mdx_hip.hip
+++ b/diffusion_for_multi_scale_molecular_dynamics_amd/csrc/mdx_hip.hip
@@ -635,8 +635,13 @@
     return v;
 }
 
+struct NextFill {
+    float *time, *sigma;
+    int mode, index_i;
+};
+
 template <int G, int CSPEC>
-__global__ __launch_bounds__(kBlock) void pc_step_kernel(PcArgs p_in)
+__global__ __launch_bounds__(kBlock) void pc_step_kernel(PcArgs p_in, NextFill next)
 {
     PcArgs p = p_in;
     if constexpr (CSPEC > 0) { p.C = CSPEC; p.d = 3; p.nl = 6; }
@@ -648,6 +653,13 @@
         const PcView v = structure_view(p, b);
         pc_update_structure<G>(p, st, v, lane, p.update_types);
     }
+    if (next.time && blockIdx.x == 0) {
+        const StepScalars sc = step_scalars(p.sched, next.mode, (p.d_index ? *p.d_index : 0) + next.index_i, 1.0);
+        for (int64_t i = threadIdx.x; i < p.B; i += blockDim.x) {
+            next.time[i] = sc.time;
+            next.sigma[i] = sc.sigma;
+        }
+    }
 }
 
 inline int lanes_per_structure(int N)
@@ -676,15 +688,15 @@
         default: LAUNCH(64) break;                                                                           \
     }
 
-int launch_pc(const PcArgs& a, hipStream_t st)
+int launch_pc(const PcArgs& a, hipStream_t st, NextFill next = NextFill{nullptr, nullptr, 0, 0})
 {
     const int G = lanes_per_structure(a.N);
     const dim3 grid = structure_grid(a.B, G), block(kBlock);
     const int cspec = (a.d == 3 && (a.C == 2 || a.C == 3)) ? a.C : 0;
 #define MDX_LAUNCH_PC(GG)                                                                                   \
-    if (cspec == 2) hipLaunchKernelGGL((pc_step_kernel<GG, 2>), grid, block, 0, st, a);                       \
-    else if (cspec == 3) hipLaunchKernelGGL((pc_step_kernel<GG, 3>), grid, block, 0, st, a);                  \
-    else hipLaunchKernelGGL((pc_step_kernel<GG, 0>), grid, block, 0, st, a);
+    if (cspec == 2) hipLaunchKernelGGL((pc_step_kernel<GG, 2>), grid, block, 0, st, a, next);                       \
+    else if (cspec == 3) hipLaunchKernelGGL((pc_step_kernel<GG, 3>), grid, block, 0, st, a, next);                  \
+    else hipLaunchKernelGGL((pc_step_kernel<GG, 0>), grid, block, 0, st, a, next);
     MDX_SWITCH_G(G, MDX_LAUNCH_PC)
 #undef MDX_LAUNCH_PC
     return launch_status();
@@ -2162,12 +2174,12 @@
     return MDX_OK;
 }
 
-int mdx_pc_step_update(const mdx_schedule_t* sched_host, int mode, int index_i, const int32_t* d_index,
-                       const mdx_pc_flags_t* f, const int64_t* atom_types, const float* x, const float* l,
-                       const float* logits, const float* score_x, const float* score_l, const float* z_coordinates,
-                       const float* gumbel, const float* u, const float* z_lattice, mdx_rng_t rng, int64_t batch,
-                       int number_of_atoms, int spatial_dimension, int64_t* atom_types_out, float* x_out, float* l_out,
-                       uint32_t* status, mdx_stream_t stream)
+static int pc_step_update(const mdx_schedule_t* sched_host, int mode, int index_i, const int32_t* d_index,
+                          const mdx_pc_flags_t* f, const int64_t* atom_types, const float* x, const float* l,
+                          const float* logits, const float* score_x, const float* score_l, const float* z_coordinates,
+                          const float* gumbel, const float* u, const float* z_lattice, mdx_rng_t rng, int64_t batch,
+                          int number_of_atoms, int spatial_dimension, int64_t* atom_types_out, float* x_out, float* l_out,
+                          uint32_t* status, NextFill next, mdx_stream_t stream)
 {
     PcArgs a{};
     const int rc = pc_common_args(sched_host, mode, index_i, d_index, f, atom_types, logits, gumbel, u, rng, batch, number_of_atoms,
@@ -2182,7 +2194,37 @@
     a.do_coords = 1; a.do_lattice = 1;
     a.x = x; a.l = l; a.score_x = score_x; a.score_l = score_l; a.z_coord = z_coordinates; a.z_lat = z_lattice;
     a.x_out = x_out; a.l_out = l_out;
-    return launch_pc(a, as_stream(stream));
+    return launch_pc(a, as_stream(stream), next);
+}
+
+int mdx_pc_step_update(const mdx_schedule_t* sched_host, int mode, int index_i, const int32_t* d_index,
+                       const mdx_pc_flags_t* f, const int64_t* atom_types, const float* x, const float* l,
+                       const float* logits, const float* score_x, const float* score_l, const float* z_coordinates,
+                       const float* gumbel, const float* u, const float* z_lattice, mdx_rng_t rng, int64_t batch,
+                       int number_of_atoms, int spatial_dimension, int64_t* atom_types_out, float* x_out, float* l_out,
+                       uint32_t* status, mdx_stream_t stream)
+{
+    return pc_step_update(sched_host, mode, index_i, d_index, f, atom_types, x, l, logits, score_x, score_l, z_coordinates, gumbel,
+                          u, z_lattice, rng, batch, number_of_atoms, spatial_dimension, atom_types_out, x_out, l_out, status,
+                          NextFill{nullptr, nullptr, 0, 0}, stream);
+}
+
+int mdx_pc_step_update_fill(const mdx_schedule_t* sched_host, int mode, int index_i, const int32_t* d_index,
+                            const mdx_pc_flags_t* f, const int64_t* atom_types, const float* x, const float* l,
+                            const float* logits, const float* score_x, const float* score_l, const float* z_coordinates,
+                            const float* gumbel, const float* u, const float* z_lattice, mdx_rng_t rng, int64_t batch,
+                            int number_of_atoms, int spatial_dimension, int64_t* atom_types_out, float* x_out, float* l_out,
+                            uint32_t* status, int next_mode, int next_index_i, float* next_time_out, float* next_sigma_out,
+                            mdx_stream_t stream)
+{
+    if (!next_time_out != !next_sigma_out) return MDX_ERR_INVALID_ARG;
+    if (next_time_out) {
+        const int rc = check_index(sched_host, next_mode, next_index_i, d_index);
+        if (rc != MDX_OK) return rc;
+    }
+    return pc_step_update(sched_host, mode, index_i, d_index, f, atom_types, x, l, logits, score_x, score_l, z_coordinates, gumbel,
+                          u, z_lattice, rng, batch, number_of_atoms, spatial_dimension, atom_types_out, x_out, l_out, status,
+                          NextFill{next_time_out, next_sigma_out, next_mode, next_index_i}, stream);
 }
 
 static AdaptiveStepArgs adaptive_step_args(const mdx_schedule_t* sched_host, int index_i, const int32_t* d_index,
diff --git a/diffusion_for_multi_scale_molecular_dynamics_amd/generators/langevin_generator.py b/diffusion_for_multi_scale_molecular_dynamics_amd/generators/langevin_generator.py
--- a/diffusion_for_multi_scale_molecular_dynamics_amd/generators/langevin_generator.py
+++ b/diffusion_for_multi_scale_molecular_dynamics_amd/generators/langevin_generator.py
@@ -3,7 +3,7 @@
 import gc
 import warnings
 import weakref
-from typing import Optional
+from typing import Optional, Tuple
 
 import torch
 
@@ -64,6 +64,7 @@
         self.noise_source = ReferenceOrderNoise() if rng_mode == "reference" else None
         self.f16_range_fallbacks = 0
         self.table_fallbacks = 0
+        self.fused_next_fill = True
         self.resampling_steps = 0
         self._visit = 0
         self._warned_not_capturable = False
@@ -269,13 +270,15 @@
                     and not hooks.outputs_watched(self.axl_network))
 
     def _step(self, mode: int, composition: AXL, index_i: int, cartesian_forces: torch.Tensor, draw_offset: int,
-              d_index: Optional[torch.Tensor] = None, in_place: bool = False, predictions_unread: bool = False):
+              d_index: Optional[torch.Tensor] = None, in_place: bool = False, predictions_unread: bool = False,
+              filled: bool = False, then: Optional[Tuple[int, int]] = None):
         x = composition.X
         device = x.device
         sched = self._prepare(device)
         batch = x.shape[0]
         time_t, sigma_t = self._time_sigma(batch, device)
-        kernels.fill_time_sigma(sched, mode, index_i, d_index, time_t, sigma_t)
+        if not filled:
+            kernels.fill_time_sigma(sched, mode, index_i, d_index, time_t, sigma_t)
         update_types = mode == MDX_PREDICTOR or self.atom_type_transition_in_corrector
         unread = self._logits_unread(update_types, predictions_unread)
         with hooks.logits_unread(self.axl_network) if unread else contextlib.nullcontext():
@@ -322,7 +325,8 @@
                                predictions.X.contiguous(),
                                self._lattice_score(predictions, composition),
                                z, gumbel, u, z_lattice, self._rng(draw_offset),
-                               a_out if update_types else None, x_out, l_out, self._status)
+                               a_out if update_types else None, x_out, l_out, self._status,
+                               None if then is None else (then[0], then[1], time_t, sigma_t))
         if self.record_atom_type_update and update_types:
             self._record_atom_type_update(sched, mode, index_i, logits, a_in, gumbel, u, a_out, batch)
         return AXL(A=a_out, X=x_out, L=l_out), predictions
@@ -490,12 +494,16 @@
     def _iteration_on_device_index(self, comp: AXL, forces: torch.Tensor, d_index: torch.Tensor,
                                    visits: Optional[int] = None):
         visits = 1 + self.resampling_steps if visits is None else visits
+        chained = self.fused_next_fill and type(self)._after_predictor is LangevinGenerator._after_predictor
+        correctors = self.number_of_corrector_steps
         for self._visit in range(visits):
-            comp, _ = self._step(MDX_PREDICTOR, comp, 1, forces, 0, d_index=d_index, in_place=True, predictions_unread=True)
+            comp, _ = self._step(MDX_PREDICTOR, comp, 1, forces, 0, d_index=d_index, in_place=True, predictions_unread=True,
+                                 then=(MDX_CORRECTOR, 0) if chained and correctors > 0 else None)
             comp = self._after_predictor(comp, 0, d_index=d_index)
-            for m in range(self.number_of_corrector_steps):
+            for m in range(correctors):
                 comp, _ = self._step(MDX_CORRECTOR, comp, 0, forces, 1 + m, d_index=d_index, in_place=True,
-                                     predictions_unread=True)
+                                     predictions_unread=True, filled=chained,
+                                     then=(MDX_CORRECTOR, 0) if chained and m + 1 < correctors else None)
             if self._visit < visits - 1:
                 comp = self._forward_step(comp, 0, d_index=d_index)
         self._visit = 0
@@ -527,7 +535,8 @@
     def _graph_key(self, start: AXL):
         settings = (self.number_of_corrector_steps, self.resampling_steps, self.atom_type_greedy_sampling,
                     self.one_atom_type_transition_per_step, self.atom_type_transition_in_corrector,
-                    self.use_fixed_lattice_parameters, self.small_epsilon, self.num_classes)
+                    self.use_fixed_lattice_parameters, self.small_epsilon, self.num_classes,
+                    self.fused_next_fill)
         words = tuple(None if w is None else w.data_ptr() for w in (self._call_word, self._status))
         net = self.axl_network
         return (tuple(start.X.shape), tuple(start.L.shape), str(start.X.device), hooks.capture_key(net), settings, words,
diff --git a/diffusion_for_multi_scale_molecular_dynamics_amd/kernels.py b/diffusion_for_multi_scale_molecular_dynamics_amd/kernels.py
--- a/diffusion_for_multi_scale_molecular_dynamics_amd/kernels.py
+++ b/diffusion_for_multi_scale_molecular_dynamics_amd/kernels.py
@@ -112,8 +112,15 @@
 
 def pc_step_update(sched: DeviceSchedule, mode: int, index_i: int, d_index: Optional[torch.Tensor], flags: PcFlags,
                    atom_types, x, l, logits, score_x, score_l, z_coordinates, gumbel, u, z_lattice, rng: Rng,
-                   atom_types_out, x_out, l_out, status: Optional[torch.Tensor]):
+                   atom_types_out, x_out, l_out, status: Optional[torch.Tensor], next_fill=None):
     B, N, d = x.shape
+    if next_fill is not None:
+        next_mode, next_index_i, time_out, sigma_out = next_fill
+        assert time_out.numel() == B and sigma_out.numel() == B
+        call("mdx_pc_step_update_fill", C.byref(sched.c_struct), int(mode), int(index_i), d_index, C.byref(flags), atom_types, x, l,
+             logits, score_x, score_l, z_coordinates, gumbel, u, z_lattice, rng, B, N, d, atom_types_out, x_out, l_out, status,
+             int(next_mode), int(next_index_i), time_out, sigma_out)
+        return
     call("mdx_pc_step_update", C.byref(sched.c_struct), int(mode), int(index_i), d_index, C.byref(flags), atom_types, x, l,
          logits, score_x, score_l, z_coordinates, gumbel, u, z_lattice, rng, B, N, d, atom_types_out, x_out, l_out, status)
 
@@ -1538,7 +1545,7 @@
         self.grid_z = torch.zeros(G, coord_dimension, dtype=F32, device=device)
         self.grid_h = torch.zeros(G, embedding_width, dtype=F32, device=device)
         self.grid_proj = torch.zeros(G, 2 * hidden, dtype=F32, device=device)
-        self.workspace = torch.zeros(n_classes ** 2 * (hidden + 2), dtype=I32, device=device)
+        self.workspace = torch.zeros(n_classes ** 2 * (hidden + 2) + 1, dtype=I32, device=device)
         self.worst = torch.zeros(1, dtype=F32, device=device)
         self.key = torch.tensor([TABLE_NO_KEY, 0], dtype=I32, device=device)
         self.stamp = None
@@ -1558,6 +1565,7 @@
     n_classes: int
     n_even: int
     memo: EgnnTableMemo
+    one_launch_check: bool = False
 
 
 def egnn_table_points(coord_dimension: int) -> int:
@@ -1584,11 +1592,13 @@
     return _TABLE_GRIDS[key]
 
 
-def egnn_table_check(table, table_scalar, n_classes: int, n_even: int, sigma, workspace, worst=None, status=None, key=None):
+def egnn_table_check(table, table_scalar, n_classes: int, n_even: int, sigma, workspace, worst=None, status=None, key=None,
+                     one_launch: bool = False):
     H = table.shape[1]
-    assert table.shape[0] == n_classes * n_classes * (2 * n_even - 1) and workspace.numel() >= n_classes ** 2 * (H + 2)
-    call("mdx_egnn_table_check_keyed", table, table_scalar, H, n_classes, n_even, sigma, sigma.numel(), TABLE_TOLERANCE, workspace,
-         worst, status, key)
+    assert table.shape[0] == n_classes * n_classes * (2 * n_even - 1)
+    assert workspace.numel() >= n_classes ** 2 * (H + 2) + int(bool(one_launch))
+    call("mdx_egnn_table_check_verdict" if one_launch else "mdx_egnn_table_check_keyed", table, table_scalar, H, n_classes, n_even,
+         sigma, sigma.numel(), TABLE_TOLERANCE, workspace, worst, status, key)
 
 
 def egnn_table_gather(table, table_scalar, n_classes: int, n_even: int, atom_types, offsets, degree, mean_messages: bool, left,
@@ -1604,14 +1614,27 @@
     return out, coord_out
 
 
+def node_inputs_rows_kernel_covers(emb_weight, second=None) -> bool:
+    H, F = emb_weight.shape
+    H2 = second[0].shape[0] if second is not None else 0
+    return H % 4 == 0 and H2 % 4 == 0 and 4 * (1 + F) * (H + H2) <= 48 * 1024
+
+
+class HeldNodeInputs:
+
+    def __init__(self):
+        self.args = None
+
+
 def egnn_node_inputs(x, k_vectors, sigma, atom_types, emb_weight, emb_bias, second=None, memo: Optional[EgnnTableMemo] = None,
-                     with_h: bool = True):
+                     with_h: bool = True, hold: Optional[HeldNodeInputs] = None, joins: Optional[HeldNodeInputs] = None):
     B, N, d = x.shape
     assert d == 3 and k_vectors.shape[1] == 3
     n_nodes, n_k, (H, F) = B * N, k_vectors.shape[0], emb_weight.shape
     w2, b2 = second if second is not None else (None, None)
     assert second is None or (w2.shape[1] == F and b2.shape[0] == w2.shape[0])
     H2 = w2.shape[0] if second is not None else 0
+    assert hold is None or (memo is None and joins is None)
     if memo is not None:
         z, h, h2 = memo.grid_z, memo.grid_h, memo.grid_proj
         assert second is not None and tuple(z.shape) == (n_nodes, 2 * n_k) and tuple(h.shape) == (n_nodes, H) and \
@@ -1620,15 +1643,30 @@
         z = torch.empty(n_nodes, 2 * n_k, dtype=F32, device=x.device)
         h = torch.empty(n_nodes, H, dtype=F32, device=x.device) if with_h else None
         h2 = torch.empty(n_nodes, H2, dtype=F32, device=x.device) if second is not None else None
-    call("mdx_egnn_node_inputs_keyed", x, k_vectors, n_k, sigma, N, atom_types, emb_weight, emb_bias, F, H, n_nodes, z, h, w2, b2,
-         H2, h2, memo.key if memo is not None else None)
+    if hold is not None:
+        hold.args = (x, k_vectors, sigma, N, atom_types, emb_weight, emb_bias, n_nodes, z, h, h2)
+    elif joins is not None:
+        held, joins.args = joins.args, None
+        assert memo is not None and held is not None, "a held launch rides with the grid's, once"
+        bx, bk, bsigma, bN, btypes, bw, bb, b_nodes, bz, bh, bh2 = held
+        assert bk.data_ptr() == k_vectors.data_ptr() and bw.data_ptr() == emb_weight.data_ptr() and \
+            bb.data_ptr() == emb_bias.data_ptr(), "one embedding and one set of wave vectors for both problems"
+        call("mdx_egnn_node_inputs_pair", k_vectors, n_k, emb_weight, emb_bias, F, H, w2, b2, H2, bx, bsigma, bN, btypes, b_nodes,
+             bz, bh, bh2, x, sigma, N, atom_types, n_nodes, z, h, h2, memo.key)
+    else:
+        call("mdx_egnn_node_inputs_keyed", x, k_vectors, n_k, sigma, N, atom_types, emb_weight, emb_bias, F, H, n_nodes, z, h, w2,
+             b2, H2, h2, memo.key if memo is not None else None)
     return (z, h) if second is None else (z, h, h2)
 
 
-def egnn_scores(z, x_hat, k_vectors):
+def egnn_scores(z, x_hat, k_vectors, n_zero: Optional[int] = None):
     n_nodes, n_k = z.shape[0], k_vectors.shape[0]
     assert z.shape == x_hat.shape == (n_nodes, 2 * n_k)
     out = torch.empty(n_nodes, 3, dtype=F32, device=z.device)
+    if n_zero is not None:
+        zeros = torch.empty(int(n_zero), dtype=F32, device=z.device)
+        call("mdx_egnn_scores_zeros", z, x_hat, k_vectors, n_k, n_nodes, out, zeros if n_zero else None, int(n_zero))
+        return out, zeros
     call("mdx_egnn_scores", z, x_hat, k_vectors, n_k, n_nodes, out)
     return out
 
diff --git a/diffusion_for_multi_scale_molecular_dynamics_amd/models/egnn.py b/diffusion_for_multi_scale_molecular_dynamics_amd/models/egnn.py
--- a/diffusion_for_multi_scale_molecular_dynamics_amd/models/egnn.py
+++ b/diffusion_for_multi_scale_molecular_dynamics_amd/models/egnn.py
@@ -343,7 +343,7 @@
                                                   memo=memo, sigma=table.sigma)
         self.device_state.table_worst = memo.worst
         kernels.egnn_table_check(values, scalars, table.n_classes, table.n_even, table.sigma, memo.workspace,
-                                 worst=memo.worst, status=self.status_word, key=memo.key)
+                                 worst=memo.worst, status=self.status_word, key=memo.key, one_launch=table.one_launch_check)
         return kernels.egnn_table_gather(values, scalars, table.n_classes, table.n_even, table.atom_types, offsets, degree,
                                          self.message_mean, left, coord, edge_index, self.coords_mean,
                                          flags=self._coord_flags(), status=self.status_word)
diff --git a/diffusion_for_multi_scale_molecular_dynamics_amd/models/score_networks/egnn_score_network.py b/diffusion_for_multi_scale_molecular_dynamics_amd/models/score_networks/egnn_score_network.py
--- a/diffusion_for_multi_scale_molecular_dynamics_amd/models/score_networks/egnn_score_network.py
+++ b/diffusion_for_multi_scale_molecular_dynamics_amd/models/score_networks/egnn_score_network.py
@@ -99,6 +99,7 @@
         self.skip_unread_logits = True
         self.logits_unread_hint = False
         self.first_layer_class_rows = True
+        self.one_launch_glue = True
         self.egnn = self._make_egnn(hp)
 
     def __getstate__(self):
@@ -181,7 +182,10 @@
     def _class_rows_serve_first_layer(self) -> bool:
         return self.first_layer_class_rows and self.sigma_uniform_hint
 
-    def _first_layer_table(self, edges, z, h, sigma, atom_types, k_vectors, second, route=None):
+    def _glue_in_one_launch(self) -> bool:
+        return self.one_launch_glue and self.sigma_uniform_hint
+
+    def _first_layer_table(self, edges, z, h, sigma, atom_types, k_vectors, second, route=None, held=None):
         from ... import kernels
         if route is None:
             route = self._routes(z.shape[0], z.shape[1], edges.shape[0],
@@ -204,9 +208,9 @@
             memo.reset()
         _, _, grid_proj = kernels.egnn_node_inputs(grid_x, k_vectors.contiguous(), sigma, classes.reshape(1, G),
                                                    emb.weight.detach().contiguous(), emb.bias.detach().contiguous(), second=second,
-                                                   memo=memo)
+                                                   memo=memo, joins=held)
         return kernels.EgnnTable(grid_proj=grid_proj, sigma=sigma, atom_types=atom_types.reshape(-1).long().contiguous(),
-                                 n_classes=n_classes, n_even=n_even, memo=memo)
+                                 n_classes=n_classes, n_even=n_even, memo=memo, one_launch_check=self._glue_in_one_launch())
 
     def _make_egnn(self, hp):
         return EGNN(
@@ -323,22 +327,28 @@
             first = routes[0] if routes else None
             second = self._first_projection_of_inputs(first.edge_pack) if first is not None else None
             class_rows = first is not None and first.path.class_rows
-            inputs = kernels.egnn_node_inputs(x.contiguous(), k_vectors.contiguous(),
+            on_table = first is not None and first.path.edge == "table"
+            k_vectors, emb_weight, emb_bias = k_vectors.contiguous(), emb.weight.detach().contiguous(), emb.bias.detach().contiguous()
+            held = kernels.HeldNodeInputs() if on_table and self._glue_in_one_launch() and \
+                kernels.node_inputs_rows_kernel_covers(emb_weight, second) else None
+            inputs = kernels.egnn_node_inputs(x.contiguous(), k_vectors,
                                               sigma_in.to(device=x.device, dtype=torch.float32).reshape(-1).contiguous(),
-                                              comp.A.reshape(bsz, n).long().contiguous(), emb.weight.detach().contiguous(),
-                                              emb.bias.detach().contiguous(), second=None if class_rows else second,
-                                              with_h=not class_rows)
+                                              comp.A.reshape(bsz, n).long().contiguous(), emb_weight, emb_bias,
+                                              second=None if class_rows else second, with_h=not class_rows, hold=held)
             z, h = inputs[:2]
             first_proj = inputs[2] if second is not None and not class_rows else None
             table = row_class = None
-            if first is not None and first.path.edge == "table":
-                table = self._first_layer_table(edges, z, h, sigma_in, comp.A, k_vectors, second, route=first)
+            if on_table:
+                table = self._first_layer_table(edges, z, h, sigma_in, comp.A, k_vectors, second, route=first, held=held)
             if class_rows:
                 h, row_class = table.memo.grid_h[:table.n_classes], table.atom_types
             out = self.egnn(h, edges, z, degree, routes=routes, first_proj=first_proj, first_table=table,
                             first_row_class=row_class)
             h, x_hat = out.A, out.X
             if routes and routes[-1].path.coords_only:
+                if self._glue_in_one_launch() and comp.L.dtype == torch.float32:
+                    scores, zeros = kernels.egnn_scores(z, x_hat.contiguous(), k_vectors.contiguous(), n_zero=comp.L.numel())
+                    return AXL(A=None, X=scores.reshape(bsz, n, d), L=zeros.reshape(comp.L.shape))
                 scores = kernels.egnn_scores(z, x_hat.contiguous(), k_vectors.contiguous())
                 return AXL(A=None, X=scores.reshape(bsz, n, d), L=torch.zeros_like(comp.L))
             if one_launch_head:
diff --git a/include/mdx_hip.h b/include/mdx_hip.h
--- a/include/mdx_hip.h
+++ b/include/mdx_hip.h
@@ -135,6 +135,14 @@
                        const float* gumbel, const float* u, const float* z_lattice, mdx_rng_t rng, int64_t batch,
                        int number_of_atoms, int spatial_dimension, int64_t* atom_types_out, float* x_out,
                        float* l_out, uint32_t* status, mdx_stream_t stream);
+
+MDX_API int mdx_pc_step_update_fill(const mdx_schedule_t* sched_host, int mode, int index_i, const int32_t* d_index,
+                            const mdx_pc_flags_t* flags_host, const int64_t* atom_types, const float* x, const float* l,
+                            const float* logits, const float* score_x, const float* score_l, const float* z_coordinates,
+                            const float* gumbel, const float* u, const float* z_lattice, mdx_rng_t rng, int64_t batch,
+                            int number_of_atoms, int spatial_dimension, int64_t* atom_types_out, float* x_out,
+                            float* l_out, uint32_t* status, int next_mode, int next_index_i, float* next_time_out,
+                            float* next_sigma_out, mdx_stream_t stream);
 
 MDX_API int mdx_adaptive_corrector_statistics(const mdx_schedule_t* sched_host, int index_i, const int32_t* d_index,
                                       const float* score_x, const float* score_l, const float* z_coordinates,
@@ -452,6 +460,16 @@
 MDX_API int mdx_egnn_table_check_keyed(const float* table, const float* table_scalar, int H, int n_classes, int n_even,
                                        const float* sigma, int64_t n_sigma, float tolerance, uint32_t* workspace,
                                        float* worst_out, uint32_t* status, uint32_t* table_key, mdx_stream_t stream);
+MDX_API int mdx_egnn_table_check_verdict(const float* table, const float* table_scalar, int H, int n_classes, int n_even,
+                                         const float* sigma, int64_t n_sigma, float tolerance, uint32_t* workspace,
+                                         float* worst_out, uint32_t* status, uint32_t* table_key, mdx_stream_t stream);
+MDX_API int mdx_egnn_node_inputs_pair(const float* k_vectors, int n_k, const float* emb_weight, const float* emb_bias,
+                                      int n_features, int H, const float* second_weight, const float* second_bias,
+                                      int second_width, const float* x, const float* sigma, int atoms_per_structure,
+                                      const int64_t* atom_types, int64_t n_nodes, float* z_out, float* h_out, float* second_out,
+                                      const float* grid_x, const float* grid_sigma, int grid_atoms_per_structure,
+                                      const int64_t* grid_atom_types, int64_t grid_nodes, float* grid_z_out, float* grid_h_out,
+                                      float* grid_second_out, const uint32_t* table_key, mdx_stream_t stream);
 MDX_API int mdx_egnn_table_gather(const float* table, const float* table_scalar, int H, int n_classes, int n_even,
                                   float inv_spacing, const int64_t* atom_types, const int64_t* offsets, const int64_t* degree,
                                   int64_t n_nodes, int mean_messages, const float* left, float* out, const float* coord,
@@ -464,6 +482,8 @@
                                  const float* second_bias, int second_width, float* second_out, mdx_stream_t stream);
 MDX_API int mdx_egnn_scores(const float* z, const float* x_hat, const float* k_vectors, int n_k, int64_t n_nodes,
                             float* scores_out, mdx_stream_t stream);
+MDX_API int mdx_egnn_scores_zeros(const float* z, const float* x_hat, const float* k_vectors, int n_k, int64_t n_nodes,
+                                  float* scores_out, float* zero_out, int64_t n_zero, mdx_stream_t stream);
 
 MDX_API int mdx_egnn_outputs(const float* z, const float* x_hat, const float* k_vectors, int n_k, const float* h,
                              const float* class_weight, const float* class_bias, int H, int num_classes, int mask_class,
```

Result: no change. 22.00 (-0.0%).
